# balcilar/gnn-matlang

Hardware: NVIDIA B200
Metric: GNNML3 train graphs/s (higher is better)
Workload: dtype f32

## Files before the change

### gnn_matlang_b200/_lib.py

```python
import ctypes
import os

import torch

_HERE = os.path.dirname(os.path.abspath(__file__))
LIB_PATH = os.environ.get("GNNML3_LIB", os.path.join(_HERE, "libgnnml3_b200.so"))

_p = ctypes.c_void_p
_i64 = ctypes.c_int64
_i = ctypes.c_int
_sz = ctypes.c_size_t

SIGNATURES = {
    "gnnml3_last_error": (ctypes.c_char_p, []),
    "gnnml3_version": (_i, []),
    "gnnml3_launch_count": (_i64, []),
    "gnnml3_csr_workspace_bytes": (_sz, [_i64, _i64]),
    "gnnml3_csr_build": (_i, [_p, _i64, _i64, _p, _p, _p, _p, _p, _p, _p, _p, _sz, _p]),
    "gnnml3_gather_rows": (_i, [_p, _p, _i64, _i, _p, _p]),
    "gnnml3_scatter_rows": (_i, [_p, _p, _i64, _i, _p, _p]),
    "gnnml3_spmm_k": (_i, [_p, _p, _p, _p, _p, _i64, _i64, _i, _i, _p, _i64, _p]),
    "gnnml3_spmm_projected": (_i, [_p, _p, _p, _p, _i, _p, _i64, _i64, _i, _p, _p, _i64, _p]),
    "gnnml3_sddmm_k": (_i, [_p, _p, _p, _p, _i64, _p, _i64, _i64, _i, _i, _p, _p]),
    "gnnml3_gemm_nn": (_i, [_p, _i64, _p, _i64, _p, _p, _i64, _i64, _i, _i, _i, _i, _p]),
    "gnnml3_gemm_tn_workspace_bytes": (_sz, [_i64, _i, _i]),
    "gnnml3_gemm_tn": (_i, [_p, _i64, _p, _i64, _p, _i64, _i64, _i, _i, _i, _p, _sz, _p]),
    "gnnml3_gemm_nn_tc_supported": (_i, [_i64, _i, _i]),
    "gnnml3_gemm_nn_tc_workspace_bytes": (_sz, [_i, _i]),
    "gnnml3_gemm_nn_tc": (_i, [_p, _i64, _p, _i64, _p, _p, _i64, _i64, _i, _i, _i, _i, _p, _sz, _p]),
    "gnnml3_colsum_workspace_bytes": (_sz, [_i64, _i]),
    "gnnml3_colsum": (_i, [_p, _i64, _i64, _i, _p, _p, _sz, _p]),
    "gnnml3_edge_mlp_supported": (_i, [_i, _i]),
    "gnnml3_collate_workspace_bytes": (_sz, [_i]),
    "gnnml3_collate": (_i, [_p, _p, _p, _p, _p, _p, _i, _p, _p, _i, _p, _i, _i64, _p, _i, _i, _i64, _i64, _p, _p, _p, _p, _p, _p, _sz, _p]),
    "gnnml3_collate_graphs_workspace_bytes": (_sz, [_i]),
    "gnnml3_collate_graphs": (_i, [_p, _p, _p, _p, _i, _p, _p, _i, _p, _p, _p, _i, _i64, _p, _i, _p, _p, _p, _i, _i64, _i, _i64, _i64, _i64,
                                   _p, _p, _p, _p, _p, _p, _p, _sz, _p]),
    "gnnml3_edge_mlp_set_tc": (_i, [_i]),
    "gnnml3_edge_mlp_path_counts": (_i, [_p, _i]),
    "gnnml3_edge_mlp_fwd": (_i, [_p, _p, _p, _p, _p, _p, _i64, _i, _i, _p, _p]),
    "gnnml3_edge_mlp_bwd_workspace_bytes": (_sz, [_i64, _i]),
    "gnnml3_edge_mlp_bwd": (_i, [_p, _p, _p, _p, _p, _p, _p, _i64, _i, _i, _p, _p, _p, _p, _p, _p, _sz, _p]),
    "gnnml3_ml3_act_fwd": (_i, [_p, _i64, _i64, _i, _i, _p, _i64, _p]),
    "gnnml3_ml3_act_bwd_workspace_bytes": (_sz, [_i64, _i, _i]),
    "gnnml3_ml3_act_bwd": (_i, [_p, _i64, _p, _i64, _i64, _i, _i, _p, _i64, _p, _i64, _p, _p, _sz, _p]),
    "gnnml3_ml3_act_bwd_y": (_i, [_p, _i64, _p, _i64, _p, _i64, _i64, _i, _i, _p, _i64, _p, _p, _sz, _p]),
    "gnnml3_fused_debug_counters": (_i, [_p, _i]),
    "gnnml3_fused_set_mode": (_i, [_i]),
    "gnnml3_fused_profile": (_i, [_i]),
    "gnnml3_fused_profile_fetch": (_i, [_p, _i]),
    "gnnml3_fused_supported": (_i, [_i, _i, _i, _i, _i, _i, _i]),
    "gnnml3_fused_workspace_bytes": (_sz, [_i, _i, _i, _i]),
    "gnnml3_fused_agg_proj": (_i, [_p, _p, _p, _p, _i, _i, _p, _i64, _i, _p, _i64, _i, _i, _p, _i64, _p, _i64, _i, _p, _p,
                                   _i64, _i, _p, _i64, _p, _i64, _i, _i, _p, _i64, _p, _p, _sz, _p]),
    "gnnml3_tile_rows": (_i, []),
    "gnnml3_tile_windows": (_i, [_p, _p, _i64, _p, _p]),
    "gnnml3_fused_ts_supported": (_i, [_i, _i, _i, _i, _i, _i, _i]),
    "gnnml3_fused_ts_workspace_bytes": (_sz, [_i, _i, _i]),
    "gnnml3_fused_set_ts": (_i, [_i]),
    "gnnml3_fused_path_counts": (_i, [_p, _i]),
    "gnnml3_fused_sddmm_supported": (_i, [_i, _i, _i]),
    "gnnml3_fused_sddmm_workspace_bytes": (_sz, [_i]),
    "gnnml3_fused_sddmm": (_i, [_p, _p, _p, _p, _i64, _i, _p, _i64, _i, _p, _i, _i64, _p, _p, _sz, _p]),
    "gnnml3_ml3layer_supported": (_i, [_i, _i, _i, _i, _i]),
    "gnnml3_ml3layer_workspace_bytes": (_sz, [_i64, _i64, _i, _i, _i, _i]),
    "gnnml3_ml3layer_forward": (_i, [_p, _p, _p, _i64, _i64, _p, _i64, _i, _p, _i, _p, _p, _p, _p, _p, _p, _i, _p, _p, _p, _p, _i, _p, _p,
                                     _i64, _p, _p, _i64, _p, _sz, _p]),
    "gnnml3_ml3layer_backward": (_i, [_p, _p, _p, _p, _p, _p, _p, _i64, _i64, _p, _i64, _i, _p, _p, _i, _p, _p, _p, _p, _p, _i, _p, _p, _i,
                                      _p, _i64, _p, _p, _i64, _i, _i, _p, _i64, _p, _p, _p, _p, _p, _p, _p, _p, _p, _p, _i64, _p, _sz, _p]),
    "gnnml3_ml1layer_supported": (_i, [_i, _i, _i]),
    "gnnml3_ml1layer_workspace_bytes": (_sz, [_i64, _i, _i, _i]),
    "gnnml3_ml1layer_forward": (_i, [_p, _p, _i64, _i64, _p, _i64, _i, _p, _p, _p, _p, _p, _p, _p, _p, _i, _i, _p, _i64, _p, _i64,
                                     _p, _i64, _p, _sz, _p]),
    "gnnml3_ml1layer_backward": (_i, [_p, _p, _i64, _i64, _p, _i64, _i, _p, _p, _p, _p, _i, _i, _p, _i64, _p, _i64, _p, _i64, _i,
                                      _p, _i64, _p, _p, _p, _p, _p, _p, _p, _p, _p, _sz, _p]),
    "gnnml3_ml1layer_forward_precision": (_i, [_p, _p, _i64, _i64, _p, _i64, _i, _p, _p, _p, _p, _p, _p, _p, _p, _i, _i, _p, _i64, _p,
                                               _i64, _p, _i64, _p, _sz, _p, _i]),
    "gnnml3_ml1layer_backward_precision": (_i, [_p, _p, _i64, _i64, _p, _i64, _i, _p, _p, _p, _p, _i, _i, _p, _i64, _p, _i64, _p, _i64,
                                                _i, _p, _i64, _p, _p, _p, _p, _p, _p, _p, _p, _p, _sz, _p, _i]),
    "gnnml3_segment_pool_fwd":(_i, [_p, _i64, _p, _i, _i, _i, _p, _p]),
    "gnnml3_segment_pool_bwd": (_i, [_p, _p, _i, _i, _i, _p, _i64, _p]),
    "gnnml3_segment_max_fwd": (_i, [_p, _i64, _p, _i, _i, _p, _p, _p]),
    "gnnml3_segment_max_bwd": (_i, [_p, _p, _p, _i, _i, _p, _i64, _p]),
    "gnnml3_spectral_max_nodes": (_i, [_i]),
    "gnnml3_spectral_count": (_i, [_p, _i64, _p, _p, _i, _i, _i, _p, _p]),
    "gnnml3_spectral_design": (_i, [_p, _i64, _p, _p, _i, _i, ctypes.c_double, _i, _i, _i, _i, ctypes.c_double, _i, _p, _i, _p,
                                    _i64, _p, _p, _p, _p]),
    "gnnml3_pairs_mark": (_i, [_p, _i64, _i64, _i, _p, _i64, ctypes.c_float, _p, _i64, _p]),
    "gnnml3_pairs_count": (_i, [_p, _i64, _i64, _i64, _p, _p]),
}

PREC_3XTF32 = 0
PREC_TF32 = 1
PREC_BF16 = 2
FUSED_FLAGS = {0: 0, 1: 0x100, 2: 0x200}
EPI_NONE = 0
EPI_RELU = 1

_lib = None


def load():
    global _lib
    if _lib is not None:
        return _lib
    if not os.path.exists(LIB_PATH):
        raise RuntimeError(
            "gnn_matlang_b200: %s not found -- build it with `python -c 'import __graft_entry__ as g; g.build()'` "
            "(or `make -C gnn_matlang_b200/csrc`).  There is no CPU / PyTorch fallback for the hot path." % LIB_PATH)
    lib = ctypes.CDLL(LIB_PATH)
    for name, (res, args) in SIGNATURES.items():
        fn = getattr(lib, name)
        fn.restype = res
        fn.argtypes = args
    _lib = lib
    return lib


def check(rc, what):
    if rc != 0:
        msg = load().gnnml3_last_error()
        raise RuntimeError("%s failed (code %d): %s" % (what, rc, msg.decode() if msg else "?"))


def stream_ptr():
    return torch._C._cuda_getCurrentRawStream(torch.cuda.current_device())


def ptr(t):
    if t is None:
        return None
    if not t.is_cuda:
        raise RuntimeError("gnn_matlang_b200: expected a CUDA tensor (the hot path has no CPU fallback)")
    return t.data_ptr()


def launch_count():
    return int(load().gnnml3_launch_count())
```

### gnn_matlang_b200/csrc/edge_mlp.cu

```cuda
#include "edge_mlp.cuh"

#include <stdlib.h>

#include <atomic>

namespace gnnml3 {

template <int K>
__global__ void __launch_bounds__(256)
k_edge_mlp_fwd(const float* __restrict__ ea, const int* __restrict__ eperm, const float* __restrict__ w1,
               const float* __restrict__ w2, const float* __restrict__ w3, const float* __restrict__ w4, int64_t E,
               float* __restrict__ out) {
    using C = EMC<K>;
    __shared__ __align__(16) float sw123[C::W123];
    __shared__ __align__(16) float sw4[C::W4];
    load_weights_smem<K>(sw123, sw4, w1, w2, w3, w4);
    __syncthreads();
    for (int64_t e = blockIdx.x * (int64_t)blockDim.x + threadIdx.x; e < E; e += (int64_t)gridDim.x * blockDim.x) {
        const int64_t src = eperm ? (int64_t)__ldg(eperm + e) : e;
        float in[C::KP];
        load_edge_row<K>(ea + src * K, in);
        float tmp[C::T];
#pragma unroll
        for (int j = 0; j < C::H; ++j) {
            const float a1 = dot_row<K>(sw123 + (0 * C::H + j) * C::KP, in);
            const float a2 = dot_row<K>(sw123 + (1 * C::H + j) * C::KP, in);
            const float a3 = dot_row<K>(sw123 + (2 * C::H + j) * C::KP, in);
            tmp[j] = fmaxf(a1, 0.f);
            tmp[C::H + j] = tanh_fast(a2) * tanh_fast(a3);
        }
        float o[K];
#pragma unroll
        for (int k = 0; k < K; ++k) {
            float a = 0.f;
#pragma unroll
            for (int j = 0; j < C::T; j += 4) {
                const float4 w = *reinterpret_cast<const float4*>(sw4 + k * C::T + j);
                a = fmaf(w.x, tmp[j], a);
                a = fmaf(w.y, tmp[j + 1], a);
                a = fmaf(w.z, tmp[j + 2], a);
                a = fmaf(w.w, tmp[j + 3], a);
            }
            o[k] = fmaxf(a, 0.f);
        }
        float* op = out + e * K;
#pragma unroll
        for (int k = 0; k < K; k += 2) *reinterpret_cast<float2*>(op + k) = make_float2(o[k], o[k + 1]);
    }
}

template <int K, bool DIN>
__global__ void __launch_bounds__(EMC<K>::THREADS)
k_edge_mlp_bwd(const float* __restrict__ ea, const int* __restrict__ eperm, const float* __restrict__ gout,
               const float* __restrict__ w1, const float* __restrict__ w2, const float* __restrict__ w3,
               const float* __restrict__ w4, int64_t E, float* __restrict__ dea, float* __restrict__ partial) {
    using C = EMC<K>;
    extern __shared__ __align__(16) float smem[];
    float* stage = smem;
    float* sw123 = smem + (size_t)C::TILE_E * C::S;
    float* sw4 = sw123 + C::W123;
    load_weights_smem<K>(sw123, sw4, w1, w2, w3, w4);

    const int tid = threadIdx.x;
    const int tile = tid % C::NT, group = tid / C::NT;
    const bool accum = group < C::GROUPS;
    int offA, offB;
    if (tile < C::NT1) {
        offA = C::OFF_D4 + 4 * (tile / (C::T / 4));
        offB = C::OFF_TMP + 4 * (tile % (C::T / 4));
    } else {
        const int t2 = tile - C::NT1;
        offA = C::OFF_D + 4 * (t2 / (C::KP / 4));
        offB = C::OFF_IN + 4 * (t2 % (C::KP / 4));
    }
    float acc[4][4];
#pragma unroll
    for (int r = 0; r < 4; ++r)
#pragma unroll
        for (int c = 0; c < 4; ++c) acc[r][c] = 0.f;
    __syncthreads();

    const int64_t ntiles = (E + C::TILE_E - 1) / C::TILE_E;
    for (int64_t tl = blockIdx.x; tl < ntiles; tl += gridDim.x) {
        const int64_t e = tl * C::TILE_E + tid;
        float* row = stage + (size_t)tid * C::S;
        if (e < E) {
            const int64_t src = eperm ? (int64_t)__ldg(eperm + e) : e;
            float in[C::KP];
            load_edge_row<K>(ea + src * K, in);
            float tmp[C::T];
            uint32_t mask1 = 0;
#pragma unroll
            for (int j0 = 0; j0 < C::H; j0 += 4) {
                float t2v[4], t3v[4];
#pragma unroll
                for (int jj = 0; jj < 4; ++jj) {
                    const int j = j0 + jj;
                    const float a1 = dot_row<K>(sw123 + (0 * C::H + j) * C::KP, in);
                    const float a2 = dot_row<K>(sw123 + (1 * C::H + j) * C::KP, in);
                    const float a3 = dot_row<K>(sw123 + (2 * C::H + j) * C::KP, in);
                    tmp[j] = fmaxf(a1, 0.f);
                    if (a1 > 0.f) mask1 |= (1u << j);
                    t2v[jj] = tanh_fast(a2);
                    t3v[jj] = tanh_fast(a3);
                    tmp[C::H + j] = t2v[jj] * t3v[jj];
                }
                *reinterpret_cast<float4*>(row + C::OFF_D + C::H + j0) = make_float4(t2v[0], t2v[1], t2v[2], t2v[3]);
                *reinterpret_cast<float4*>(row + C::OFF_D + 2 * C::H + j0) = make_float4(t3v[0], t3v[1], t3v[2], t3v[3]);
            }
#pragma unroll
            for (int j = 0; j < C::T; j += 4)
                *reinterpret_cast<float4*>(row + C::OFF_TMP + j) = make_float4(tmp[j], tmp[j + 1], tmp[j + 2], tmp[j + 3]);
#pragma unroll
            for (int i = 0; i < C::KP; i += 4)
                *reinterpret_cast<float4*>(row + C::OFF_IN + i) = make_float4(in[i], in[i + 1], in[i + 2], in[i + 3]);
            float d4[C::KP];
            {
                float go[C::KP];
                load_edge_row<K>(gout + e * K, go);
#pragma unroll
                for (int k = 0; k < K; ++k) {
                    float a = 0.f;
#pragma unroll
                    for (int j = 0; j < C::T; j += 4) {
                        const float4 w = *reinterpret_cast<const float4*>(sw4 + k * C::T + j);
                        a = fmaf(w.x, tmp[j], a);
                        a = fmaf(w.y, tmp[j + 1], a);
                        a = fmaf(w.z, tmp[j + 2], a);
                        a = fmaf(w.w, tmp[j + 3], a);
                    }
                    d4[k] = a > 0.f ? go[k] : 0.f;
                }
#pragma unroll
                for (int k = K; k < C::KP; ++k) d4[k] = 0.f;
            }
#pragma unroll
            for (int k = 0; k < C::KP; k += 4)
                *reinterpret_cast<float4*>(row + C::OFF_D4 + k) = make_float4(d4[k], d4[k + 1], d4[k + 2], d4[k + 3]);
            float din[DIN ? C::KP : 1];
#pragma unroll
            for (int i = 0; i < (DIN ? C::KP : 1); ++i) din[i] = 0.f;
#pragma unroll
            for (int j0 = 0; j0 < C::H; j0 += 4) {
                float dt1[4] = {0.f, 0.f, 0.f, 0.f}, dt2[4] = {0.f, 0.f, 0.f, 0.f};
#pragma unroll
                for (int k = 0; k < K; ++k) {
                    const float4 wa = *reinterpret_cast<const float4*>(sw4 + k * C::T + j0);
                    const float4 wb = *reinterpret_cast<const float4*>(sw4 + k * C::T + C::H + j0);
                    dt1[0] = fmaf(d4[k], wa.x, dt1[0]); dt1[1] = fmaf(d4[k], wa.y, dt1[1]);
                    dt1[2] = fmaf(d4[k], wa.z, dt1[2]); dt1[3] = fmaf(d4[k], wa.w, dt1[3]);
                    dt2[0] = fmaf(d4[k], wb.x, dt2[0]); dt2[1] = fmaf(d4[k], wb.y, dt2[1]);
                    dt2[2] = fmaf(d4[k], wb.z, dt2[2]); dt2[3] = fmaf(d4[k], wb.w, dt2[3]);
                }
                const float4 t2 = *reinterpret_cast<const float4*>(row + C::OFF_D + C::H + j0);
                const float4 t3 = *reinterpret_cast<const float4*>(row + C::OFF_D + 2 * C::H + j0);
                const float t2a[4] = {t2.x, t2.y, t2.z, t2.w}, t3a[4] = {t3.x, t3.y, t3.z, t3.w};
                float d1[4], d2[4], d3[4];
#pragma unroll
                for (int jj = 0; jj < 4; ++jj) {
                    d1[jj] = ((mask1 >> (j0 + jj)) & 1u) ? dt1[jj] : 0.f;
                    d2[jj] = dt2[jj] * t3a[jj] * (1.f - t2a[jj] * t2a[jj]);
                    d3[jj] = dt2[jj] * t2a[jj] * (1.f - t3a[jj] * t3a[jj]);
                }
                *reinterpret_cast<float4*>(row + C::OFF_D + j0) = make_float4(d1[0], d1[1], d1[2], d1[3]);
                *reinterpret_cast<float4*>(row + C::OFF_D + C::H + j0) = make_float4(d2[0], d2[1], d2[2], d2[3]);
                *reinterpret_cast<float4*>(row + C::OFF_D + 2 * C::H + j0) = make_float4(d3[0], d3[1], d3[2], d3[3]);
                if constexpr (DIN) {
#pragma unroll
                    for (int jj = 0; jj < 4; ++jj) {
                        const float* r1 = sw123 + (0 * C::H + j0 + jj) * C::KP;
                        const float* r2 = sw123 + (1 * C::H + j0 + jj) * C::KP;
                        const float* r3 = sw123 + (2 * C::H + j0 + jj) * C::KP;
#pragma unroll
                        for (int i = 0; i < C::KP; i += 4) {
                            const float4 a = *reinterpret_cast<const float4*>(r1 + i);
                            const float4 b = *reinterpret_cast<const float4*>(r2 + i);
                            const float4 c = *reinterpret_cast<const float4*>(r3 + i);
                            din[i] += d1[jj] * a.x + d2[jj] * b.x + d3[jj] * c.x;
                            din[i + 1] += d1[jj] * a.y + d2[jj] * b.y + d3[jj] * c.y;
                            din[i + 2] += d1[jj] * a.z + d2[jj] * b.z + d3[jj] * c.z;
                            din[i + 3] += d1[jj] * a.w + d2[jj] * b.w + d3[jj] * c.w;
                        }
                    }
                }
            }
            if constexpr (C::DP > C::D) {
#pragma unroll
                for (int i = C::D; i < C::DP; ++i) row[C::OFF_D + i] = 0.f;
            }
            if constexpr (DIN) {
                float* dp = dea + src * K;
#pragma unroll
                for (int i = 0; i < K; i += 2) *reinterpret_cast<float2*>(dp + i) = make_float2(din[i], din[i + 1]);
            }
        } else {
#pragma unroll
            for (int i = 0; i < C::ROW; i += 4) *reinterpret_cast<float4*>(row + i) = make_float4(0.f, 0.f, 0.f, 0.f);
        }
        __syncthreads();
        if (accum) {
#pragma unroll 4
            for (int r = group; r < C::TILE_E; r += C::GROUPS) {
                const float4 a = *reinterpret_cast<const float4*>(stage + (size_t)r * C::S + offA);
                const float4 b = *reinterpret_cast<const float4*>(stage + (size_t)r * C::S + offB);
                const float av[4] = {a.x, a.y, a.z, a.w}, bv[4] = {b.x, b.y, b.z, b.w};
#pragma unroll
                for (int i = 0; i < 4; ++i)
#pragma unroll
                    for (int j = 0; j < 4; ++j) acc[i][j] = fmaf(av[i], bv[j], acc[i][j]);
            }
        }
        __syncthreads();
    }
    float* red = stage;
    if (accum) {
#pragma unroll
        for (int i = 0; i < 4; ++i)
#pragma unroll
            for (int j = 0; j < 4; ++j) red[(size_t)group * C::NT * 16 + tile * 16 + i * 4 + j] = acc[i][j];
    }
    __syncthreads();
    for (int i = tid; i < C::NT * 16; i += blockDim.x) {
        float s = 0.f;
#pragma unroll
        for (int g = 0; g < C::GROUPS; ++g) s += red[(size_t)g * C::NT * 16 + i];
        partial[(size_t)blockIdx.x * C::NT * 16 + i] = s;
    }
}

static int bwd_blocks(int64_t E, int tile_e) {
    int64_t t = (E + tile_e - 1) / tile_e;
    int64_t cap = kNumSMs;
    return (int)(t < 1 ? 1 : (t > cap ? cap : t));
}

int edge_mlp_tc_fwd(const float* ea, const int32_t* eperm, const float* w1, const float* w2, const float* w3, const float* w4, int64_t E,
                    int K, float* out, cudaStream_t st);
size_t edge_mlp_tc_bwd_workspace_bytes(int K);
int edge_mlp_tc_bwd(const float* ea, const int32_t* eperm, const float* gout, const float* w1, const float* w2, const float* w3,
                    const float* w4, int64_t E, int K, float* dea, float* dw1, float* dw2, float* dw3, float* dw4, float* partial,
                    cudaStream_t st);

}

using namespace gnnml3;

static int g_edge_tc = [] {
    const char* e = getenv("GNNML3_EDGE_TC");
    return (e && e[0] == '0') ? 0 : 1;
}();
static std::atomic<long long> g_edge_paths[2];

extern "C" int gnnml3_edge_mlp_set_tc(int enable) {
    const int old = g_edge_tc;
    if (enable == 0 || enable == 1) g_edge_tc = enable;
    return old;
}
extern "C" int gnnml3_edge_mlp_path_counts(long long* out2_host, int reset) {
    out2_host[0] = reset ? g_edge_paths[0].exchange(0) : g_edge_paths[0].load();
    out2_host[1] = reset ? g_edge_paths[1].exchange(0) : g_edge_paths[1].load();
    return GNNML3_OK;
}

#define DISPATCH_EVEN_K(KV, ...)                                   \
    switch (KV) {                                                  \
        case 2: { constexpr int K_ = 2; __VA_ARGS__; } break;      \
        case 4: { constexpr int K_ = 4; __VA_ARGS__; } break;      \
        case 6: { constexpr int K_ = 6; __VA_ARGS__; } break;      \
        case 8: { constexpr int K_ = 8; __VA_ARGS__; } break;      \
        case 10: { constexpr int K_ = 10; __VA_ARGS__; } break;    \
        case 12: { constexpr int K_ = 12; __VA_ARGS__; } break;    \
        case 14: { constexpr int K_ = 14; __VA_ARGS__; } break;    \
        case 16: { constexpr int K_ = 16; __VA_ARGS__; } break;    \
        default: return set_err(GNNML3_ERR_INVALID, "edge_mlp: K=%d not instantiated (even K <= 16)", KV); \
    }

extern "C" int gnnml3_edge_mlp_supported(int K, int Kout) { return (K == Kout && K >= 2 && K <= 16 && K % 2 == 0) ? 1 : 0; }

extern "C" int gnnml3_edge_mlp_fwd(const float* ea, const int32_t* eperm, const float* w1, const float* w2, const float* w3,
                                   const float* w4, int64_t E, int K, int Kout, float* out, void* stream_) {
    GNNML3_REQUIRE(gnnml3_edge_mlp_supported(K, Kout), "edge_mlp_fwd: unsupported K=%d Kout=%d (even K <= 16, Kout == K)", K, Kout);
    GNNML3_REQUIRE(E >= 0, "edge_mlp_fwd: E < 0");
    if (E == 0) return GNNML3_OK;
    GNNML3_REQUIRE(ea && w1 && w2 && w3 && w4 && out, "edge_mlp_fwd: NULL pointer");
    GNNML3_REQUIRE((uintptr_t)ea % 16 == 0 && (uintptr_t)out % 16 == 0, "edge_mlp_fwd: ea/out must be 16-byte aligned");
    if (g_edge_tc) {
        ++g_edge_paths[0];
        return edge_mlp_tc_fwd(ea, eperm, w1, w2, w3, w4, E, K, out, (cudaStream_t)stream_);
    }
    ++g_edge_paths[1];
    int64_t nb = (E + 255) / 256;
    if (nb > (int64_t)kNumSMs * 8) nb = (int64_t)kNumSMs * 8;
    DISPATCH_EVEN_K(K, (k_edge_mlp_fwd<K_><<<(int)nb, 256, 0, (cudaStream_t)stream_>>>(ea, eperm, w1, w2, w3, w4, E, out)));
    GNNML3_LAUNCH_CHECK();
    return GNNML3_OK;
}

extern "C" size_t gnnml3_edge_mlp_bwd_workspace_bytes(int64_t E, int K) {
    const int KP = pad4(K), T = 4 * K, DP = pad4(6 * K);
    const size_t nt = (size_t)(KP / 4) * (T / 4) + (size_t)(DP / 4) * (KP / 4);
    const size_t cc = (size_t)bwd_blocks(E, 256) * nt * 16 * sizeof(float);
    const size_t tc = edge_mlp_tc_bwd_workspace_bytes(K);
    return align_up(cc > tc ? cc : tc, 256);
}

template <int K>
static int launch_edge_bwd(const float* ea, const int32_t* eperm, const float* gout, const float* w1, const float* w2,
                           const float* w3, const float* w4, int64_t E, float* dea, float* dw1, float* dw2, float* dw3,
                           float* dw4, float* partial, cudaStream_t st) {
    using C = EMC<K>;
    static bool configured[64] = {};
    if (auto once_ = first_use_on_device(configured)) {
        GNNML3_CUDA(cudaFuncSetAttribute(k_edge_mlp_bwd<K, true>, cudaFuncAttributeMaxDynamicSharedMemorySize, (int)C::bwd_smem));
        GNNML3_CUDA(cudaFuncSetAttribute(k_edge_mlp_bwd<K, false>, cudaFuncAttributeMaxDynamicSharedMemorySize, (int)C::bwd_smem));
    }
    const int nb = bwd_blocks(E, C::TILE_E);
    if (dea)
        k_edge_mlp_bwd<K, true><<<nb, C::THREADS, C::bwd_smem, st>>>(ea, eperm, gout, w1, w2, w3, w4, E, dea, partial);
    else
        k_edge_mlp_bwd<K, false><<<nb, C::THREADS, C::bwd_smem, st>>>(ea, eperm, gout, w1, w2, w3, w4, E, dea, partial);
    GNNML3_LAUNCH_CHECK();
    k_edge_mlp_bwd_reduce<K><<<cdiv(C::NOUT, 32), 256, 0, st>>>(partial, nb, dw1, dw2, dw3, dw4);
    GNNML3_LAUNCH_CHECK();
    return GNNML3_OK;
}

extern "C" int gnnml3_edge_mlp_bwd(const float* ea, const int32_t* eperm, const float* gout, const float* w1, const float* w2,
                                   const float* w3, const float* w4, int64_t E, int K, int Kout, float* dea, float* dw1,
                                   float* dw2, float* dw3, float* dw4, void* workspace, size_t workspace_bytes,
                                   void* stream_) {
    GNNML3_REQUIRE(gnnml3_edge_mlp_supported(K, Kout), "edge_mlp_bwd: unsupported K=%d Kout=%d", K, Kout);
    GNNML3_REQUIRE(E >= 0 && w1 && w2 && w3 && w4 && dw1 && dw2 && dw3 && dw4, "edge_mlp_bwd: bad arguments");
    cudaStream_t st = (cudaStream_t)stream_;
    if (E == 0) {
        GNNML3_CUDA(cudaMemsetAsync(dw1, 0, sizeof(float) * 2 * K * K, st));
        GNNML3_CUDA(cudaMemsetAsync(dw2, 0, sizeof(float) * 2 * K * K, st));
        GNNML3_CUDA(cudaMemsetAsync(dw3, 0, sizeof(float) * 2 * K * K, st));
        GNNML3_CUDA(cudaMemsetAsync(dw4, 0, sizeof(float) * 4 * K * K, st));
        return GNNML3_OK;
    }
    GNNML3_REQUIRE(ea && gout && workspace, "edge_mlp_bwd: NULL pointer");
    GNNML3_REQUIRE((uintptr_t)ea % 16 == 0 && (uintptr_t)gout % 16 == 0 && (dea == nullptr || (uintptr_t)dea % 16 == 0),
                   "edge_mlp_bwd: ea/gout/dea must be 16-byte aligned");
    if (workspace_bytes < gnnml3_edge_mlp_bwd_workspace_bytes(E, K))
        return set_err(GNNML3_ERR_WORKSPACE, "edge_mlp_bwd: workspace too small");
    if (g_edge_tc) {
        ++g_edge_paths[0];
        return edge_mlp_tc_bwd(ea, eperm, gout, w1, w2, w3, w4, E, K, dea, dw1, dw2, dw3, dw4, (float*)workspace, st);
    }
    ++g_edge_paths[1];
    DISPATCH_EVEN_K(K, return launch_edge_bwd<K_>(ea, eperm, gout, w1, w2, w3, w4, E, dea, dw1, dw2, dw3, dw4,
                                                   (float*)workspace, st));
    return GNNML3_OK;
}
```

### gnn_matlang_b200/csrc/edge_mlp.cuh

```cuda
#pragma once
#include "common.cuh"

namespace gnnml3 {

constexpr int pad4(int x) { return (x + 3) / 4 * 4; }

template <int K>
struct EMC {
    static constexpr int KP = pad4(K);
    static constexpr int H = 2 * K;
    static constexpr int T = 4 * K;
    static constexpr int D = 6 * K;
    static constexpr int DP = pad4(D);
    static constexpr int OFF_D4 = 0, OFF_TMP = KP, OFF_D = KP + T, OFF_IN = KP + T + DP, ROW = KP + T + DP + KP;
    static constexpr int S = ((ROW / 4) % 2 == 1) ? ROW : ROW + 4;
    static constexpr int NT1 = (KP / 4) * (T / 4);
    static constexpr int NT2 = (DP / 4) * (KP / 4);
    static constexpr int NT = NT1 + NT2;
    static constexpr int THREADS = 256;
    static constexpr int GROUPS = (THREADS / NT) < 1 ? 1 : (THREADS / NT);
    static constexpr int TILE_E = THREADS;
    static constexpr int W123 = 3 * H * KP;
    static constexpr int W4 = K * T;
    static constexpr int NOUT = K * T + 3 * H * K;
    static constexpr size_t bwd_smem = sizeof(float) * ((size_t)TILE_E * S + W123 + W4);
};

template <int K>
__device__ __forceinline__ void load_weights_smem(float* sw123, float* sw4, const float* __restrict__ w1,
                                                  const float* __restrict__ w2, const float* __restrict__ w3,
                                                  const float* __restrict__ w4) {
    using C = EMC<K>;
    for (int i = threadIdx.x; i < C::W123; i += blockDim.x) {
        const int m = i / (C::H * C::KP), r = (i / C::KP) % C::H, c = i % C::KP;
        const float* w = m == 0 ? w1 : (m == 1 ? w2 : w3);
        sw123[i] = (c < K) ? __ldg(w + r * K + c) : 0.f;
    }
    for (int i = threadIdx.x; i < C::W4; i += blockDim.x) sw4[i] = __ldg(w4 + i);
}

template <int K>
__device__ __forceinline__ void load_edge_row(const float* __restrict__ p, float (&in)[EMC<K>::KP]) {
    if constexpr (K % 4 == 0) {
#pragma unroll
        for (int i = 0; i < K; i += 4) {
            float4 v = ldg4(p + i);
            in[i] = v.x; in[i + 1] = v.y; in[i + 2] = v.z; in[i + 3] = v.w;
        }
    } else {
#pragma unroll
        for (int i = 0; i < K; i += 2) {
            float2 v = ldg2(p + i);
            in[i] = v.x; in[i + 1] = v.y;
        }
#pragma unroll
        for (int i = K; i < EMC<K>::KP; ++i) in[i] = 0.f;
    }
}

template <int K>
__device__ __forceinline__ float dot_row(const float* __restrict__ wrow, const float (&in)[EMC<K>::KP]) {
    float a = 0.f;
#pragma unroll
    for (int i = 0; i < EMC<K>::KP; i += 4) {
        const float4 w = *reinterpret_cast<const float4*>(wrow + i);
        a = fmaf(w.x, in[i], a);
        a = fmaf(w.y, in[i + 1], a);
        a = fmaf(w.z, in[i + 2], a);
        a = fmaf(w.w, in[i + 3], a);
    }
    return a;
}

template <int K>
__global__ void __launch_bounds__(256)
k_edge_mlp_bwd_reduce(const float* __restrict__ partial, int nblocks, float* __restrict__ dw1, float* __restrict__ dw2,
                      float* __restrict__ dw3, float* __restrict__ dw4) {
    using C = EMC<K>;
    __shared__ float red[8][33];
    const int tx = threadIdx.x & 31, ty = threadIdx.x >> 5;
    const int i = blockIdx.x * 32 + tx;
    int idx = 0;
    float* dst = nullptr;
    if (i < C::NOUT) {
        int r, c;
        if (i < K * C::T) {
            r = i / C::T;
            c = i % C::T;
            idx = ((r / 4) * (C::T / 4) + c / 4) * 16 + (r % 4) * 4 + (c % 4);
            dst = dw4 + i;
        } else {
            const int q = i - K * C::T;
            const int m = q / (C::H * K), jj = (q / K) % C::H;
            c = q % K;
            r = m * C::H + jj;
            idx = (C::NT1 + (r / 4) * (C::KP / 4) + c / 4) * 16 + (r % 4) * 4 + (c % 4);
            dst = (m == 0 ? dw1 : (m == 1 ? dw2 : dw3)) + jj * K + c;
        }
    }
    float s = 0.f;
    if (dst) {
        float s1 = 0.f, s2 = 0.f, s3 = 0.f;
        int b = ty;
        for (; b + 24 < nblocks; b += 32) {
            s += __ldg(partial + (size_t)b * C::NT * 16 + idx);
            s1 += __ldg(partial + (size_t)(b + 8) * C::NT * 16 + idx);
            s2 += __ldg(partial + (size_t)(b + 16) * C::NT * 16 + idx);
            s3 += __ldg(partial + (size_t)(b + 24) * C::NT * 16 + idx);
        }
        for (; b < nblocks; b += 8) s += __ldg(partial + (size_t)b * C::NT * 16 + idx);
        s = (s + s1) + (s2 + s3);
    }
    red[ty][tx] = s;
    __syncthreads();
    if (ty == 0 && dst) {
        float v = 0.f;
#pragma unroll
        for (int y = 0; y < 8; ++y) v += red[y][tx];
        *dst = v;
    }
}


}
```

### gnn_matlang_b200/csrc/edge_mlp_tc.cu

```cuda
#include "edge_mlp.cuh"
#include "tc_common.cuh"

namespace gnnml3 {

#ifndef EMT_MAXWG
#define EMT_MAXWG 4
#endif

template <int K>
struct EMT {
    using C = EMC<K>;
    static constexpr int P = (K + 7) / 8 * 8;
    static constexpr int HP = 2 * P, TP = 4 * P, DPP = 6 * P;
    static constexpr int N1 = 6 * P;
    static constexpr int N2 = 16;
    static constexpr int N3 = TP;
    static constexpr int TB = TP / 32;
    static constexpr int DB = (DPP + 31) / 32;
    static constexpr int B1_BYTES = 2 * N1 * 128, B2_BYTES = TB * 32 * 128, B3_BYTES = 2 * N3 * 128, B4_BYTES = DB * 32 * 128;
    __host__ __device__ static constexpr int xc(int mode) { return mode > 1 ? 12 * P : 8 * P; }
    static constexpr int YC = 2 * P;
    __host__ __device__ static constexpr int slot(int mode) { return xc(mode) + YC; }
    __host__ __device__ static constexpr int plane_bytes(int mode) { return B1_BYTES + B2_BYTES + (mode > 0 ? B3_BYTES : 0) + (mode > 1 ? B4_BYTES : 0); }
    static constexpr int stage_bytes = 128 * C::S * 4;
    static constexpr int SMEM_MAX = 227 * 1024 - 1024;
    __host__ __device__ static constexpr int nwg(int mode) {
        int n = 512 / slot(mode);
        if (mode > 0) {
            const int m = (SMEM_MAX - plane_bytes(mode) - 64) / stage_bytes;
            n = m < n ? m : n;
        }
        return n < 1 ? 1 : (n > EMT_MAXWG ? EMT_MAXWG : n);
    }
    __host__ __device__ static constexpr int smem_bytes(int mode) { return 1024 + plane_bytes(mode) + 64 + (mode > 0 ? nwg(mode) * stage_bytes : 0); }
    static constexpr int NT = C::NT;
    static constexpr int TPT = (NT + 127) / 128;
    static constexpr int GROUPS = NT >= 128 ? 1 : 128 / NT;
};

#ifdef EMT_PROFILE
__device__ unsigned long long g_emt_dbg[16];
#define EMT_T(i) do { if (prof) { const long long now_ = clock64(); tacc[i] += now_ - tlast; tlast = now_; } } while (0)
#else
#define EMT_T(i) do { } while (0)
#endif

struct EMTParams {
    const float* ea;
    const int* eperm;
    const float* gout;
    const float *w1, *w2, *w3, *w4;
    int64_t E;
    float* out;
    float* dea;
    float* partial;
};

__device__ __forceinline__ float emt_lo(float v) { return v - __uint_as_float(__float_as_uint(v) & 0xFFFFE000u); }

__device__ __forceinline__ void emt_st8(uint32_t ta, const float* v) {
    asm volatile("tcgen05.st.sync.aligned.32x32b.x8.b32 [%0], {%1,%2,%3,%4,%5,%6,%7,%8};" ::"r"(ta), "f"(v[0]), "f"(v[1]), "f"(v[2]),
                 "f"(v[3]), "f"(v[4]), "f"(v[5]), "f"(v[6]), "f"(v[7])
                 : "memory");
}
__device__ __forceinline__ void emt_st16(uint32_t ta, const float* v) {
    asm volatile("tcgen05.st.sync.aligned.32x32b.x16.b32 [%0], {%1,%2,%3,%4,%5,%6,%7,%8,%9,%10,%11,%12,%13,%14,%15,%16};" ::"r"(ta),
                 "f"(v[0]), "f"(v[1]), "f"(v[2]), "f"(v[3]), "f"(v[4]), "f"(v[5]), "f"(v[6]), "f"(v[7]), "f"(v[8]), "f"(v[9]), "f"(v[10]),
                 "f"(v[11]), "f"(v[12]), "f"(v[13]), "f"(v[14]), "f"(v[15])
                 : "memory");
}
__device__ __forceinline__ void emt_st_wait() { asm volatile("tcgen05.wait::st.sync.aligned;" ::: "memory"); }
__device__ __forceinline__ void emt_ld16(uint32_t ta, float (&v)[16]) {
    asm volatile(
        "tcgen05.ld.sync.aligned.32x32b.x16.b32 {%0,%1,%2,%3,%4,%5,%6,%7,%8,%9,%10,%11,%12,%13,%14,%15}, [%16];"
        : "=f"(v[0]), "=f"(v[1]), "=f"(v[2]), "=f"(v[3]), "=f"(v[4]), "=f"(v[5]), "=f"(v[6]), "=f"(v[7]), "=f"(v[8]), "=f"(v[9]), "=f"(v[10]),
          "=f"(v[11]), "=f"(v[12]), "=f"(v[13]), "=f"(v[14]), "=f"(v[15])
        : "r"(ta)
        : "memory");
}
__device__ __forceinline__ void emt_ld_wait() { asm volatile("tcgen05.wait::ld.sync.aligned;" ::: "memory"); }

__device__ __forceinline__ void emt_mma(uint32_t tmem_d, uint32_t tmem_a, uint64_t bdesc, uint32_t idesc, uint32_t accumulate) {
    asm volatile(
        "{\n\t"
        ".reg .pred p;\n\t"
        "setp.ne.b32 p, %4, 0;\n\t"
        "tcgen05.mma.cta_group::1.kind::tf32 [%0], [%1], %2, %3, p;\n\t"
        "}\n" ::"r"(tmem_d), "r"(tmem_a), "l"(bdesc), "r"(idesc), "r"(accumulate)
        : "memory");
}
__device__ __forceinline__ bool emt_elect() {
    uint32_t pred;
    asm volatile(
        "{\n\t"
        ".reg .pred p;\n\t"
        "elect.sync _|p, 0xffffffff;\n\t"
        "selp.u32 %0, 1, 0, p;\n\t"
        "}\n"
        : "=r"(pred));
    return pred != 0;
}
__device__ __forceinline__ void emt_group_sync(int id) { asm volatile("bar.sync %0, 128;" ::"r"(id) : "memory"); }

__device__ __forceinline__ uint32_t emt_sw128(int n, int c) { return (uint32_t)n * 128u + ((uint32_t)(((c >> 2) ^ (n & 7)) << 4) | (uint32_t)((c & 3) << 2)); }

__device__ __forceinline__ void emt_put(uint8_t* plane, int n, int c, float v, bool lo) {
    const float h = tf32_rn(v);
    *reinterpret_cast<float*>(plane + emt_sw128(n, c)) = lo ? v - h : h;
}

template <typename F>
__device__ __forceinline__ void emt_round(int barid, int warp_in_wg, uint64_t* bar, uint32_t& ph, F issue) {
    emt_st_wait();
    tc_fence_before();
    emt_group_sync(barid);
    if (warp_in_wg == 0) {
        if (emt_elect()) {
            tc_fence_after();
            issue();
            umma_commit(bar);
        }
        __syncwarp();
    }
    mbar_wait(bar, ph);
    ph ^= 1;
    tc_fence_after();
}

template <int K, int MODE>
__global__ void __launch_bounds__(EMT<K>::nwg(MODE) * 128, 1) k_edge_mlp_tc(const EMTParams p) {
    using T = EMT<K>;
    using C = EMC<K>;
    constexpr int P = T::P, HP = T::HP, TP = T::TP, H = C::H;
    constexpr int NWG = T::nwg(MODE);
    extern __shared__ uint8_t smem_raw[];
    uint8_t* smem = smem_raw + ((1024u - (smem_u32(smem_raw) & 1023u)) & 1023u);
    uint8_t* b1 = smem;
    uint8_t* b2 = b1 + T::B1_BYTES;
    uint8_t* b3 = b2 + T::B2_BYTES;
    uint8_t* b4 = b3 + T::B3_BYTES;
    uint8_t* tail = smem + T::plane_bytes(MODE);
    uint64_t* bars = reinterpret_cast<uint64_t*>(tail);
    uint32_t* tmem_slot = reinterpret_cast<uint32_t*>(tail + 48);
    float* stage_all = reinterpret_cast<float*>(tail + 64);

    const int wg = threadIdx.x >> 7, t = threadIdx.x & 127, warp_in_wg = t >> 5;

    for (int i = threadIdx.x; i < 2 * T::N1 * P; i += blockDim.x) {
        const int n = i / P, c = i % P;
        const bool lo = n >= T::N1;
        const int nn = lo ? n - T::N1 : n, b = nn / HP, j = nn % HP;
        const float* w = b == 0 ? p.w1 : (b == 1 ? p.w2 : p.w3);
        emt_put(b1, n, c, (j < H && c < K) ? __ldg(w + j * K + c) : 0.f, lo);
    }
    for (int i = threadIdx.x; i < T::TB * 32 * 32; i += blockDim.x) {
        const int tb = i / 1024, n = (i / 32) % 32, c = i % 32;
        const bool lo = n >= 16;
        const int k = n & 15, q = tb * 32 + c, part = q / HP, j = q % HP;
        emt_put(b2 + tb * 4096, n, c, (k < K && j < H) ? __ldg(p.w4 + k * C::T + part * H + j) : 0.f, lo);
    }
    if constexpr (MODE > 0) {
        for (int i = threadIdx.x; i < 2 * T::N3 * P; i += blockDim.x) {
            const int n = i / P, c = i % P;
            const bool lo = n >= T::N3;
            const int q = lo ? n - T::N3 : n, part = q / HP, j = q % HP;
            emt_put(b3, n, c, (c < K && j < H) ? __ldg(p.w4 + c * C::T + part * H + j) : 0.f, lo);
        }
    }
    if constexpr (MODE > 1) {
        for (int i = threadIdx.x; i < T::DB * 32 * 32; i += blockDim.x) {
            const int db = i / 1024, n = (i / 32) % 32, c = i % 32;
            const bool lo = n >= 16;
            const int ii = n & 15, q = db * 32 + c, b = q / HP, j = q % HP;
            const float* w = b == 0 ? p.w1 : (b == 1 ? p.w2 : p.w3);
            emt_put(b4 + db * 4096, n, c, (ii < K && q < T::DPP && j < H) ? __ldg(w + j * K + ii) : 0.f, lo);
        }
    }
    fence_proxy_async_smem();
    if (threadIdx.x == 0) {
        for (int g = 0; g < NWG; ++g) mbar_init(bars + g, 1);
        asm volatile("fence.mbarrier_init.release.cluster;" ::: "memory");
    }
    if (threadIdx.x < 32) tmem_alloc(tmem_slot, 512);
    tc_fence_before();
    __syncthreads();
    tc_fence_after();
    const uint32_t tmem_base = *tmem_slot;

    const uint32_t Xm = tmem_base + (uint32_t)wg * T::slot(MODE), Ym = Xm + T::xc(MODE);
    const uint32_t lane_sel = (uint32_t)(warp_in_wg * 32) << 16;
    const uint32_t X = Xm + lane_sel, Y = Ym + lane_sel;
    uint64_t* bar = bars + wg;
    uint32_t ph = 0;
    const int barid = 1 + wg;
    const uint64_t d1h = make_kmajor_sw128_desc(smem_u32(b1)), d1l = d1h + (uint64_t)((T::N1 * 128) >> 4);
    const uint64_t d2h = make_kmajor_sw128_desc(smem_u32(b2)), d2l = d2h + (uint64_t)((16 * 128) >> 4);
    const uint64_t d3h = make_kmajor_sw128_desc(smem_u32(b3)), d3l = d3h + (uint64_t)((T::N3 * 128) >> 4);
    const uint64_t d4h = make_kmajor_sw128_desc(smem_u32(b4)), d4l = d4h + (uint64_t)((16 * 128) >> 4);
    constexpr uint32_t ID1 = make_idesc_tf32_mn(128, T::N1), ID2 = make_idesc_tf32_mn(128, T::N2), ID3 = make_idesc_tf32_mn(128, T::N3);
    auto mma3 = [&](uint32_t d, uint32_t a_raw, uint32_t a_lo, uint64_t bh, uint64_t bl, uint32_t idesc, bool first) {
        emt_mma(d, a_raw, bh, idesc, first ? 0u : 1u);
        emt_mma(d, a_raw, bl, idesc, 1u);
        emt_mma(d, a_lo, bh, idesc, 1u);
    };

    float* stage = stage_all + (size_t)wg * 128 * C::S;
    float* row = stage + (size_t)t * C::S;

    int offA[T::TPT], offB[T::TPT];
    bool accum[T::TPT];
    float acc[T::TPT][4][4];
    const int group = T::TPT == 1 ? t / T::NT : 0;
    if constexpr (MODE > 0) {
#pragma unroll
        for (int u = 0; u < T::TPT; ++u) {
            const int tl = T::TPT == 1 ? t % T::NT : t + 128 * u;
            accum[u] = T::TPT == 1 ? group < T::GROUPS : tl < T::NT;
            if (tl < C::NT1) {
                offA[u] = C::OFF_D4 + 4 * (tl / (C::T / 4));
                offB[u] = C::OFF_TMP + 4 * (tl % (C::T / 4));
            } else {
                const int t2 = (tl < T::NT ? tl : C::NT1) - C::NT1;
                offA[u] = C::OFF_D + 4 * (t2 / (C::KP / 4));
                offB[u] = C::OFF_IN + 4 * (t2 % (C::KP / 4));
            }
#pragma unroll
            for (int r = 0; r < 4; ++r)
#pragma unroll
                for (int c = 0; c < 4; ++c) acc[u][r][c] = 0.f;
        }
    }

    const int64_t ntiles = (p.E + 127) / 128;
    const int64_t tstride = (int64_t)gridDim.x * NWG;
    float in_n[C::KP];
    int64_t src_n = 0;
    auto fetch = [&](int64_t tile) {
        const int64_t e = tile * 128 + t;
#pragma unroll
        for (int i = 0; i < C::KP; ++i) in_n[i] = 0.f;
        src_n = 0;
        if (tile < ntiles && e < p.E) {
            src_n = p.eperm ? (int64_t)__ldg(p.eperm + e) : e;
            load_edge_row<K>(p.ea + src_n * K, in_n);
        }
    };
    fetch((int64_t)blockIdx.x * NWG + wg);
#ifdef EMT_PROFILE
    const bool prof = t == 0;
    long long tacc[10] = {0, 0, 0, 0, 0, 0, 0, 0, 0, 0}, tlast = clock64();
    const long long tbegin = tlast;
#endif
    for (int64_t tile = (int64_t)blockIdx.x * NWG + wg; tile < ntiles; tile += tstride) {
        const int64_t e = tile * 128 + t;
        const bool live = e < p.E;
        const int64_t src = src_n;
        float in[P];
#pragma unroll
        for (int i = 0; i < P; ++i) in[i] = i < C::KP ? in_n[i < C::KP ? i : 0] : 0.f;
        {
            float lo[P];
#pragma unroll
            for (int i = 0; i < P; ++i) lo[i] = emt_lo(in[i]);
            if constexpr (P == 8) {
                emt_st8(Y, in);
                emt_st8(Y + 8, lo);
            } else {
                emt_st16(Y, in);
                emt_st16(Y + 16, lo);
            }
        }
        if constexpr (MODE > 0) {
#pragma unroll
            for (int i = 0; i < C::KP; i += 4) *reinterpret_cast<float4*>(row + C::OFF_IN + i) = make_float4(in[i], in[i + 1], in[i + 2], in[i + 3]);
        }
        float go[C::KP];
#pragma unroll
        for (int i = 0; i < C::KP; ++i) go[i] = 0.f;
        if constexpr (MODE > 0) {
            if (live) load_edge_row<K>(p.gout + e * K, go);
        }
        fetch(tile + tstride);
        EMT_T(0);
        emt_round(barid, warp_in_wg, bar, ph, [&] {
#pragma unroll
            for (int s = 0; s < P / 8; ++s) mma3(Xm, Ym + 8 * s, Ym + P + 8 * s, d1h + (uint64_t)(2 * s), d1l + (uint64_t)(2 * s), ID1, s == 0);
        });
        EMT_T(1);
        uint32_t mask1 = 0;
#pragma unroll
        for (int c = 0; c < HP / 16; ++c) {
            float r[16], a2[16], a3[16];
            emt_ld16(X + 16 * c, r);
            emt_ld16(X + 2 * P + 16 * c, a2);
            emt_ld16(X + 4 * P + 16 * c, a3);
            emt_ld_wait();
            float pr[16];
#pragma unroll
            for (int i = 0; i < 16; ++i) {
                if (MODE > 0 && r[i] > 0.f) mask1 |= 1u << (16 * c + i);
                r[i] = fmaxf(r[i], 0.f);
                a2[i] = tanh_fast5(a2[i]);
                a3[i] = tanh_fast5(a3[i]);
                pr[i] = a2[i] * a3[i];
            }
            emt_st16(X + 16 * c, r);
            emt_st16(X + 2 * P + 16 * c, pr);
            if constexpr (MODE > 0) {
#pragma unroll
                for (int i = 0; i < 16; i += 4) {
                    const int j0 = 16 * c + i;
                    if (j0 < H) {
                        *reinterpret_cast<float4*>(row + C::OFF_TMP + j0) = make_float4(r[i], r[i + 1], r[i + 2], r[i + 3]);
                        *reinterpret_cast<float4*>(row + C::OFF_TMP + H + j0) = make_float4(pr[i], pr[i + 1], pr[i + 2], pr[i + 3]);
                        *reinterpret_cast<float4*>(row + C::OFF_D + H + j0) = make_float4(a2[i], a2[i + 1], a2[i + 2], a2[i + 3]);
                        *reinterpret_cast<float4*>(row + C::OFF_D + 2 * H + j0) = make_float4(a3[i], a3[i + 1], a3[i + 2], a3[i + 3]);
                    }
                }
            }
#pragma unroll
            for (int i = 0; i < 16; ++i) {
                r[i] = emt_lo(r[i]);
                pr[i] = emt_lo(pr[i]);
            }
            emt_st16(X + 4 * P + 16 * c, r);
            emt_st16(X + 6 * P + 16 * c, pr);
        }
        EMT_T(2);
        emt_round(barid, warp_in_wg, bar, ph, [&] {
#pragma unroll
            for (int s = 0; s < TP / 8; ++s) {
                const uint64_t adv = (uint64_t)((s / 4) * (4096 >> 4) + 2 * (s % 4));
                mma3(Ym, Xm + 8 * s, Xm + TP + 8 * s, d2h + adv, d2l + adv, ID2, s == 0);
            }
        });
        EMT_T(3);
        float pre4[16];
        emt_ld16(Y, pre4);
        emt_ld_wait();
        if constexpr (MODE == 0) {
            if (live) {
                float* op = p.out + e * K;
#pragma unroll
                for (int k = 0; k < K; k += 2) *reinterpret_cast<float2*>(op + k) = make_float2(fmaxf(pre4[k], 0.f), fmaxf(pre4[k + 1], 0.f));
            }
        } else {
            float dp4[P];
#pragma unroll
            for (int k = 0; k < P; ++k) dp4[k] = (k < K && pre4[k] > 0.f) ? go[k < C::KP ? k : 0] : 0.f;
#pragma unroll
            for (int k = 0; k < C::KP; k += 4) *reinterpret_cast<float4*>(row + C::OFF_D4 + k) = make_float4(dp4[k], dp4[k + 1], dp4[k + 2], dp4[k + 3]);
            {
                float lo[P];
#pragma unroll
                for (int i = 0; i < P; ++i) lo[i] = emt_lo(dp4[i]);
                if constexpr (P == 8) {
                    emt_st8(Y, dp4);
                    emt_st8(Y + 8, lo);
                } else {
                    emt_st16(Y, dp4);
                    emt_st16(Y + 16, lo);
                }
            }
            emt_round(barid, warp_in_wg, bar, ph, [&] {
#pragma unroll
                for (int s = 0; s < P / 8; ++s) mma3(Xm, Ym + 8 * s, Ym + P + 8 * s, d3h + (uint64_t)(2 * s), d3l + (uint64_t)(2 * s), ID3, s == 0);
            });
            EMT_T(4);
#pragma unroll
            for (int c = 0; c < HP / 16; ++c) {
                float dt1[16], dt2[16];
                emt_ld16(X + 16 * c, dt1);
                emt_ld16(X + 2 * P + 16 * c, dt2);
                emt_ld_wait();
                float g1[16], g2[16], g3[16];
#pragma unroll
                for (int i = 0; i < 16; i += 4) {
                    const int j0 = 16 * c + i;
                    float4 t2 = make_float4(0.f, 0.f, 0.f, 0.f), t3 = t2;
                    if (j0 < H) {
                        t2 = *reinterpret_cast<const float4*>(row + C::OFF_D + H + j0);
                        t3 = *reinterpret_cast<const float4*>(row + C::OFF_D + 2 * H + j0);
                    }
                    const float t2a[4] = {t2.x, t2.y, t2.z, t2.w}, t3a[4] = {t3.x, t3.y, t3.z, t3.w};
#pragma unroll
                    for (int jj = 0; jj < 4; ++jj) {
                        g1[i + jj] = ((mask1 >> (j0 + jj)) & 1u) ? dt1[i + jj] : 0.f;
                        g2[i + jj] = dt2[i + jj] * t3a[jj] * (1.f - t2a[jj] * t2a[jj]);
                        g3[i + jj] = dt2[i + jj] * t2a[jj] * (1.f - t3a[jj] * t3a[jj]);
                    }
                    if (j0 < H) {
                        *reinterpret_cast<float4*>(row + C::OFF_D + j0) = make_float4(g1[i], g1[i + 1], g1[i + 2], g1[i + 3]);
                        *reinterpret_cast<float4*>(row + C::OFF_D + H + j0) = make_float4(g2[i], g2[i + 1], g2[i + 2], g2[i + 3]);
                        *reinterpret_cast<float4*>(row + C::OFF_D + 2 * H + j0) = make_float4(g3[i], g3[i + 1], g3[i + 2], g3[i + 3]);
                    }
                }
                if constexpr (MODE > 1) {
                    emt_st16(X + 16 * c, g1);
                    emt_st16(X + 2 * P + 16 * c, g2);
                    emt_st16(X + 4 * P + 16 * c, g3);
#pragma unroll
                    for (int i = 0; i < 16; ++i) {
                        g1[i] = emt_lo(g1[i]);
                        g2[i] = emt_lo(g2[i]);
                        g3[i] = emt_lo(g3[i]);
                    }
                    emt_st16(X + 6 * P + 16 * c, g1);
                    emt_st16(X + 8 * P + 16 * c, g2);
                    emt_st16(X + 10 * P + 16 * c, g3);
                }
            }
            if constexpr (C::DP > C::D) {
#pragma unroll
                for (int i = C::D; i < C::DP; ++i) row[C::OFF_D + i] = 0.f;
            }
            if constexpr (MODE > 1) {
                emt_round(barid, warp_in_wg, bar, ph, [&] {
#pragma unroll
                    for (int s = 0; s < T::DPP / 8; ++s) {
                        const uint64_t adv = (uint64_t)((s / 4) * (4096 >> 4) + 2 * (s % 4));
                        mma3(Ym, Xm + 8 * s, Xm + T::DPP + 8 * s, d4h + adv, d4l + adv, ID2, s == 0);
                    }
                });
                float din[16];
                emt_ld16(Y, din);
                emt_ld_wait();
                if (live) {
                    float* dp = p.dea + src * K;
#pragma unroll
                    for (int i = 0; i < K; i += 2) *reinterpret_cast<float2*>(dp + i) = make_float2(din[i], din[i + 1]);
                }
            }
            EMT_T(5);
            emt_group_sync(barid);
            EMT_T(6);
#pragma unroll
            for (int u = 0; u < T::TPT; ++u) {
                if (accum[u]) {
                    const float* pa = stage + (size_t)group * C::S + offA[u];
                    const float* pb = stage + (size_t)group * C::S + offB[u];
#pragma unroll 4
                    for (int r = group; r < 128; r += T::GROUPS) {
                        const float4 a = *reinterpret_cast<const float4*>(pa);
                        const float4 b = *reinterpret_cast<const float4*>(pb);
                        pa += T::GROUPS * C::S;
                        pb += T::GROUPS * C::S;
                        const float av[4] = {a.x, a.y, a.z, a.w}, bv[4] = {b.x, b.y, b.z, b.w};
#pragma unroll
                        for (int i = 0; i < 4; ++i)
#pragma unroll
                            for (int j = 0; j < 4; ++j) acc[u][i][j] = fmaf(av[i], bv[j], acc[u][i][j]);
                    }
                }
            }
            emt_group_sync(barid);
            EMT_T(7);
        }
        EMT_T(8);
    }
#ifdef EMT_PROFILE
    if (prof && wg == 0) {
        for (int i = 0; i < 9; ++i) atomicAdd(&g_emt_dbg[i], (unsigned long long)tacc[i]);
        atomicAdd(&g_emt_dbg[9], (unsigned long long)(clock64() - tbegin));
        atomicAdd(&g_emt_dbg[10], 1ull);
    }
#endif
    if constexpr (MODE > 0) {
        float* red = stage;
#pragma unroll
        for (int u = 0; u < T::TPT; ++u) {
            if (accum[u]) {
                const int tl = T::TPT == 1 ? t % T::NT : t + 128 * u;
#pragma unroll
                for (int i = 0; i < 4; ++i)
#pragma unroll
                    for (int j = 0; j < 4; ++j) red[(size_t)group * T::NT * 16 + tl * 16 + i * 4 + j] = acc[u][i][j];
            }
        }
        emt_group_sync(barid);
        for (int i = t; i < T::NT * 16; i += 128) {
            float s = 0.f;
#pragma unroll
            for (int g = 0; g < T::GROUPS; ++g) s += red[(size_t)g * T::NT * 16 + i];
            red[i] = s;
        }
        __syncthreads();
        float* dst = p.partial + (size_t)blockIdx.x * T::NT * 16;
        for (int i = threadIdx.x; i < T::NT * 16; i += NWG * 128) {
            float s = 0.f;
#pragma unroll
            for (int g = 0; g < NWG; ++g) s += stage_all[(size_t)g * 128 * C::S + i];
            dst[i] = s;
        }
    }
    tc_fence_before();
    __syncthreads();
    if (threadIdx.x < 32) tmem_dealloc(tmem_base, 512);
}

template <int K, int MODE>
static int emt_launch(const EMTParams& p, int* nparts, cudaStream_t st) {
    using T = EMT<K>;
    static bool configured[64] = {};
    if (auto once_ = first_use_on_device(configured))
        GNNML3_CUDA(cudaFuncSetAttribute(k_edge_mlp_tc<K, MODE>, cudaFuncAttributeMaxDynamicSharedMemorySize, T::smem_bytes(MODE)));
    constexpr int NWG = T::nwg(MODE);
    const int64_t ntiles = (p.E + 127) / 128;
    int64_t grid = (ntiles + NWG - 1) / NWG;
    if (grid > kNumSMs) grid = kNumSMs;
    k_edge_mlp_tc<K, MODE><<<(int)grid, NWG * 128, T::smem_bytes(MODE), st>>>(p);
    GNNML3_LAUNCH_CHECK();
    if (nparts) *nparts = (int)grid;
    return GNNML3_OK;
}

#define EMT_DISPATCH(KV, ...)                                      \
    switch (KV) {                                                  \
        case 2: { constexpr int K_ = 2; __VA_ARGS__; } break;      \
        case 4: { constexpr int K_ = 4; __VA_ARGS__; } break;      \
        case 6: { constexpr int K_ = 6; __VA_ARGS__; } break;      \
        case 8: { constexpr int K_ = 8; __VA_ARGS__; } break;      \
        case 10: { constexpr int K_ = 10; __VA_ARGS__; } break;    \
        case 12: { constexpr int K_ = 12; __VA_ARGS__; } break;    \
        case 14: { constexpr int K_ = 14; __VA_ARGS__; } break;    \
        case 16: { constexpr int K_ = 16; __VA_ARGS__; } break;    \
        default: return set_err(GNNML3_ERR_INVALID, "edge_mlp_tc: K=%d not instantiated (even K <= 16)", KV); \
    }

int edge_mlp_tc_fwd(const float* ea, const int32_t* eperm, const float* w1, const float* w2, const float* w3, const float* w4, int64_t E,
                    int K, float* out, cudaStream_t st) {
    EMTParams p;
    p.ea = ea; p.eperm = eperm; p.gout = nullptr; p.w1 = w1; p.w2 = w2; p.w3 = w3; p.w4 = w4; p.E = E; p.out = out; p.dea = nullptr;
    p.partial = nullptr;
    EMT_DISPATCH(K, return (emt_launch<K_, 0>(p, nullptr, st)));
    return GNNML3_OK;
}

size_t edge_mlp_tc_bwd_workspace_bytes(int K) {
    const int KP = pad4(K), T = 4 * K, DP = pad4(6 * K);
    const size_t nt = (size_t)(KP / 4) * (T / 4) + (size_t)(DP / 4) * (KP / 4);
    return (size_t)kNumSMs * nt * 16 * sizeof(float);
}

int edge_mlp_tc_bwd(const float* ea, const int32_t* eperm, const float* gout, const float* w1, const float* w2, const float* w3,
                    const float* w4, int64_t E, int K, float* dea, float* dw1, float* dw2, float* dw3, float* dw4, float* partial,
                    cudaStream_t st) {
    EMTParams p;
    p.ea = ea; p.eperm = eperm; p.gout = gout; p.w1 = w1; p.w2 = w2; p.w3 = w3; p.w4 = w4; p.E = E; p.out = nullptr; p.dea = dea;
    p.partial = partial;
    int nparts = 0, rc;
    if (dea) {
        EMT_DISPATCH(K, rc = (emt_launch<K_, 2>(p, &nparts, st)));
    } else {
        EMT_DISPATCH(K, rc = (emt_launch<K_, 1>(p, &nparts, st)));
    }
    if (rc) return rc;
    EMT_DISPATCH(K, (k_edge_mlp_bwd_reduce<K_><<<cdiv(EMC<K_>::NOUT, 32), 256, 0, st>>>(partial, nparts, dw1, dw2, dw3, dw4)));
    GNNML3_LAUNCH_CHECK();
    return GNNML3_OK;
}

}

#ifdef EMT_PROFILE
extern "C" __attribute__((visibility("default"))) int gnnml3_emt_debug_fetch(unsigned long long* host16, int reset) {
    cudaDeviceSynchronize();
    cudaMemcpyFromSymbol(host16, gnnml3::g_emt_dbg, sizeof(unsigned long long) * 16);
    if (reset) {
        unsigned long long z[16] = {};
        cudaMemcpyToSymbol(gnnml3::g_emt_dbg, z, sizeof(z));
    }
    return 0;
}
#endif
```

### gnn_matlang_b200/libs/spect_conv.py

```python
import math
import os

import torch
import torch.nn as nn
from torch.nn import Parameter

from .. import _lib, ops
from ..graph import get_plan, sorted_edge_attr

_PRECISIONS = {"fp32": _lib.PREC_3XTF32, "3xtf32": _lib.PREC_3XTF32, "tf32": _lib.PREC_TF32, "bf16": _lib.PREC_BF16}
USE_FUSED = os.environ.get("GNNML3_NO_FUSED", "0") != "1"
USE_LAYER_API = os.environ.get("GNNML3_NO_LAYER_API", "0") != "1"
KEEP_FIRST_LAYER_AGGREGATE = os.environ.get("GNNML3_KEEP_AGGREGATE", "1") != "0"


def _use_fused(precision):
    return USE_FUSED


def _fused_ok(precision, K, Kstride, F, Nc, Fs=0, self_mode=0, Ns=0):
    if precision == _lib.PREC_3XTF32:
        return ops.fused_supported(K, Kstride, F, Nc, Fs, self_mode, Ns)
    return ops.fused_ts_supported(K, Kstride, F, Nc, Fs, self_mode, Ns)


def glorot(tensor):
    if tensor is not None:
        stdv = math.sqrt(6.0 / (tensor.size(-2) + tensor.size(-1)))
        tensor.data.uniform_(-stdv, stdv)


def zeros(tensor):
    if tensor is not None:
        tensor.data.fill_(0)


def _aggregate(plan, ea_s, x, width_blocks, transposed=False):
    N, F = x.shape
    K = ea_s.size(1)
    out = torch.empty(N, width_blocks * F, dtype=torch.float32, device=x.device)
    if plan.E == 0:
        out[:, :K * F].zero_()
    elif transposed:
        ops.spmm_k(plan.rowptrT, plan.colT, plan.permT, ea_s, x, out=out)
    else:
        ops.spmm_k(plan.rowptr, plan.col, None, ea_s, x, out=out)
    return out


class _SpectConvFn(torch.autograd.Function):

    @staticmethod
    def forward(ctx, x, ea_s, weight, bias, plan, selfconn, precision):
        if x.stride(1) != 1:
            x = x.contiguous()
        ea_s = ea_s.contiguous()
        weight = weight.contiguous()
        N, Fi = x.shape
        Kw, _, Fo = weight.shape
        K = ea_s.size(1)
        fused = (_use_fused(precision) and N > 0 and plan.E > 0 and (not selfconn or Fi <= 32)
                 and _fused_ok(precision, K, K, Fi, Fo, Fi if selfconn else 0, 2 if selfconn else 0, 0))
        ctx.plan, ctx.selfconn, ctx.precision, ctx.has_bias = plan, selfconn, precision, bias is not None
        ctx.fused = fused
        if fused:
            x = ops.aligned_rows(x)
            out, _ = ops.fused_agg_proj(plan.rowptr, plan.col, None, ea_s, x, weight[:K].reshape(K * Fi, Fo), bias=bias,
                                        S=x if selfconn else None, self_mode=2 if selfconn else 0,
                                        Bself=weight[K] if selfconn else None, epilogue=0, win=plan.win, precision=precision)
        else:
            H = _aggregate(plan, ea_s, x, Kw)
            if selfconn:
                H[:, K * Fi:] = x
            out = ops.gemm_nn(H, weight.view(Kw * Fi, Fo), bias, precision=precision)
        ctx.save_for_backward(x, ea_s, weight)
        return out

    @staticmethod
    def backward(ctx, gout):
        x, ea_s, weight = ctx.saved_tensors
        plan, prec = ctx.plan, ctx.precision
        N, Fi = x.shape
        Kw, _, Fo = weight.shape
        K = ea_s.size(1)
        need_x, need_ea, need_w, need_b = ctx.needs_input_grad[:4]
        dx = dea = dw = db = None
        if N == 0:
            return (torch.zeros_like(x) if need_x else None, torch.zeros_like(ea_s) if need_ea else None,
                    torch.zeros_like(weight) if need_w else None,
                    torch.zeros(Fo, device=x.device) if (need_b and ctx.has_bias) else None, None, None, None)
        gout = ops.aligned_rows(gout) if ctx.fused else gout.contiguous()
        fused_dx = (ctx.fused and need_x and (not ctx.selfconn or Fo <= 32)
                    and _fused_ok(prec, K, K, Fo, Fi, Fo if ctx.selfconn else 0, 2 if ctx.selfconn else 0, 0))
        G = None
        if fused_dx:
            Fp = (Fo + 31) // 32 * 32
            side = need_w and ops.fused_side_output_ok()
            if side:
                G = torch.empty(N, (K + (1 if ctx.selfconn else 0)) * Fp, dtype=torch.float32, device=x.device)
            dx, _ = ops.fused_agg_proj(plan.rowptrT, plan.colT, plan.permT, ea_s, gout,
                                       weight[:K].transpose(1, 2).reshape(K * Fo, Fi).contiguous(),
                                       S=gout if ctx.selfconn else None, self_mode=2 if ctx.selfconn else 0,
                                       Bself=weight[K].t().contiguous() if ctx.selfconn else None, epilogue=0, hout=G,
                                       win=plan.winT, precision=prec)
            if side:
                dcat = ops.gemm_tn(x, G, precision=prec)
                dw = dcat.view(Fi, Kw, Fp)[:, :, :Fo].permute(1, 0, 2).contiguous()
                need_w = False
        if need_w or (need_x and not fused_dx):
            G = _aggregate(plan, ea_s, gout, Kw, transposed=True)
            if ctx.selfconn:
                G[:, K * Fo:] = gout
            if need_x and not fused_dx:
                dx = ops.gemm_nn(G, weight.transpose(1, 2).contiguous().view(Kw * Fo, Fi), precision=prec)
            if need_w:
                dw = ops.gemm_tn(x, G, precision=prec).view(Fi, Kw, Fo).permute(1, 0, 2).contiguous()
        if need_b and ctx.has_bias:
            db = ops.colsum(gout)
        if need_ea:
            if plan.E == 0:
                dea = torch.zeros_like(ea_s)
            elif ctx.fused and ops.fused_sddmm_supported(K, Fi, Fo):
                dea = ops.fused_sddmm(plan.rowptr, plan.col, x, gout, weight[:K].contiguous(), plan.E, win=plan.win)
            else:
                wp = weight[:K].permute(2, 0, 1).reshape(Fo, K * Fi).contiguous()
                dH = ops.gemm_nn(gout, wp, precision=prec)
                dea = ops.sddmm_k(plan.rowptr, plan.col, None, x, dH, K, plan.E)
        return dx, dea, dw, db, None, None, None


class _SpectConvProjectFirstFn(torch.autograd.Function):

    @staticmethod
    def forward(ctx, x, ea_s, weight, bias, plan, precision):
        x, ea_s = x.contiguous(), ea_s.contiguous()
        K, Fi, Fo = weight.shape
        wcat = weight.permute(1, 0, 2).reshape(Fi, K * Fo).contiguous()
        Y = ops.gemm_nn(x, wcat, precision=precision)
        if plan.E == 0:
            out = torch.zeros(x.size(0), Fo, device=x.device) + (bias if bias is not None else 0)
        else:
            out = ops.spmm_projected(plan.rowptr, plan.col, None, ea_s, Y, Fo, bias)
        ctx.save_for_backward(x, ea_s, wcat, Y)
        ctx.plan, ctx.precision, ctx.has_bias, ctx.shape = plan, precision, bias is not None, (K, Fi, Fo)
        return out

    @staticmethod
    def backward(ctx, gout):
        x, ea_s, wcat, Y = ctx.saved_tensors
        plan, prec = ctx.plan, ctx.precision
        K, Fi, Fo = ctx.shape
        gout = gout.contiguous()
        dY = _aggregate(plan, ea_s, gout, K, transposed=True)
        dx = ops.gemm_nn(dY, wcat.t().contiguous(), precision=prec) if ctx.needs_input_grad[0] else None
        dw = None
        if ctx.needs_input_grad[2]:
            dw = ops.gemm_tn(x, dY, precision=prec).view(Fi, K, Fo).permute(1, 0, 2).contiguous()
        dea = None
        if ctx.needs_input_grad[1]:
            dea = (torch.zeros_like(ea_s) if plan.E == 0 else
                   ops.sddmm_k(plan.rowptrT, plan.colT, plan.permT, gout, Y, K, plan.E))
        db = ops.colsum(gout) if (ctx.has_bias and ctx.needs_input_grad[3]) else None
        return dx, dea, dw, db, None, None


def project_first_pays(N, E, K, Fi, Fo):
    return K * Fo * (E + 2 * N) < Fi * (E + 2 * N * K)


class _AggregateFn(torch.autograd.Function):

    @staticmethod
    def forward(ctx, x, ea_s, plan):
        x, ea_s = x.contiguous(), ea_s.contiguous()
        ctx.save_for_backward(x, ea_s)
        ctx.plan = plan
        return _aggregate(plan, ea_s, x, ea_s.size(1))

    @staticmethod
    def backward(ctx, dH):
        x, ea_s = ctx.saved_tensors
        plan = ctx.plan
        dH = dH.contiguous()
        K, F = ea_s.size(1), x.size(1)
        if plan.E == 0:
            return torch.zeros_like(x), torch.zeros_like(ea_s), None
        dx = ops.spmm_projected(plan.rowptrT, plan.colT, plan.permT, ea_s, dH, F) if ctx.needs_input_grad[0] else None
        dea = ops.sddmm_k(plan.rowptr, plan.col, None, x, dH, K, plan.E) if ctx.needs_input_grad[1] else None
        return dx, dea, None


class _DepthwiseAggFn(torch.autograd.Function):

    @staticmethod
    def forward(ctx, x, ea_s, scale, plan):
        x, ea_s, scale = x.contiguous(), ea_s.contiguous(), scale.contiguous()
        N, F = x.shape
        K = ea_s.size(1)
        H = _aggregate(plan, ea_s, x, K)
        ctx.save_for_backward(x, ea_s, scale, H)
        ctx.plan = plan
        return (H.view(N, K, F) * scale.unsqueeze(0)).sum(1)

    @staticmethod
    def backward(ctx, dZ):
        x, ea_s, scale, H = ctx.saved_tensors
        plan = ctx.plan
        dZ = dZ.contiguous()
        N, F = x.shape
        K = ea_s.size(1)
        G = _aggregate(plan, ea_s, dZ, K, transposed=True)
        dx = (G.view(N, K, F) * scale.unsqueeze(0)).sum(1)
        dscale = (H.view(N, K, F) * dZ.unsqueeze(1)).sum(0)
        if plan.E == 0:
            dea = torch.zeros_like(ea_s)
        else:
            g = (dZ.unsqueeze(1) * scale.unsqueeze(0)).reshape(N, K * F).contiguous()
            dea = ops.sddmm_k(plan.rowptr, plan.col, None, x, g, K, plan.E)
        return dx, dea, dscale, None


class _LinearFn(torch.autograd.Function):

    @staticmethod
    def forward(ctx, x, wt, bias, precision):
        x, wt = x.contiguous(), wt.contiguous()
        ctx.save_for_backward(x, wt)
        ctx.precision, ctx.has_bias = precision, bias is not None
        return ops.gemm_nn(x, wt, bias, precision=precision)

    @staticmethod
    def backward(ctx, g):
        x, wt = ctx.saved_tensors
        g = g.contiguous()
        dx = dw = db = None
        if x.size(0) == 0:
            return torch.zeros_like(x), torch.zeros_like(wt), (torch.zeros(wt.size(1), device=x.device) if ctx.has_bias else None), None
        if ctx.needs_input_grad[0]:
            dx = ops.gemm_nn(g, wt.t().contiguous(), precision=ctx.precision)
        if ctx.needs_input_grad[1]:
            dw = ops.gemm_tn(x, g, precision=ctx.precision)
        if ctx.has_bias and ctx.needs_input_grad[2]:
            db = ops.colsum(g)
        return dx, dw, db, None


class _ML3LayerFn(torch.autograd.Function):

    @staticmethod
    def forward(ctx, x, ea_s, w1, w2, w3, w4, wconv, bconv, w11, b11, w12, b12, plan, fused_edge, precision, save=True):
        if x.stride(1) != 1:
            x = x.contiguous()
        ea_s = ea_s.contiguous()
        wconv = wconv.contiguous()
        N, Fi = x.shape
        K, _, Fo = wconv.shape
        G = 0 if w11 is None else w11.size(0)
        ctx.composite = False
        if (_use_fused(precision) and precision == _lib.PREC_3XTF32 and USE_LAYER_API and N > 0 and plan.E > 0
                and (fused_edge or w1 is None) and ops.ml3layer_supported(K, Fi, Fo, G, fused_edge)):
            xa = ops.aligned_rows(x)
            ws4 = tuple(w.contiguous() for w in (w1, w2, w3, w4)) if fused_edge else None
            gates = (w11.contiguous(), b11.contiguous(), w12.contiguous(), b12.contiguous()) if G > 0 else None
            keep = (not ctx.needs_input_grad[0]) and ctx.needs_input_grad[6] and Fi <= 32 and KEEP_FIRST_LAYER_AGGREGATE
            if save:
                y, aux, ea2, hside = ops.ml3layer_forward(plan, xa, ea_s, ws4, wconv, bconv.contiguous() if bconv is not None else None,
                                                          gates, keep_aggregate=keep)
            else:
                y, aux, ea2, hside = ops.ml3layer_forward(plan, xa, ea_s, ws4, wconv, bconv.contiguous() if bconv is not None else None,
                                                          gates, keep_aggregate=False, aux=False)
            ctx.plan, ctx.fused_edge, ctx.precision, ctx.G = plan, fused_edge, precision, G
            ctx.has_bias, ctx.fused, ctx.composite = bconv is not None, True, True
            if save:
                ctx.save_for_backward(xa, ea_s, ea2, y, aux, w1, w2, w3, w4, wconv, w11, w12, hside)
            return y
        if fused_edge:
            w1, w2, w3, w4 = w1.contiguous(), w2.contiguous(), w3.contiguous(), w4.contiguous()
            ea2 = ops.edge_mlp_fwd(ea_s, None, w1, w2, w3, w4)
        else:
            ea2 = ea_s
        fused = (_use_fused(precision) and N > 0 and plan.E > 0 and (G == 0 or Fi <= 32)
                 and _fused_ok(precision, K, K, Fi, Fo, Fi if G else 0, 1 if G else 0, 2 * G)
                 and _fused_ok(precision, K, K, Fo, Fi, 2 * G, 2 if G else 0, 0))
        ctx.plan, ctx.fused_edge, ctx.precision, ctx.G = plan, fused_edge, precision, G
        ctx.has_bias = bconv is not None
        ctx.fused = fused
        if fused:
            xa = ops.aligned_rows(x)
            wg = torch.cat([w11.t(), w12.t()], 1).contiguous() if G > 0 else None
            bg = torch.cat([b11, b12]) if G > 0 else None
            if save:
                y, aux = ops.fused_agg_proj(plan.rowptr, plan.col, None, ea2, xa, wconv.view(K * Fi, Fo), bias=bconv,
                                            S=xa if G > 0 else None, self_mode=1 if G > 0 else 0, Bself=wg, bias_s=bg, G=G,
                                            epilogue=1, win=plan.win, precision=precision)
                ctx.save_for_backward(xa, ea_s, ea2 if fused_edge else None, y, aux, w1, w2, w3, w4, wconv, w11, w12, None)
            else:
                y, _ = ops.fused_agg_proj(plan.rowptr, plan.col, None, ea2, xa, wconv.view(K * Fi, Fo), bias=bconv,
                                          S=xa if G > 0 else None, self_mode=1 if G > 0 else 0, Bself=wg, bias_s=bg, G=G,
                                          epilogue=1, win=plan.win, precision=precision, aux=False)
            return y
        H = _aggregate(plan, ea2, x, K)
        pre = torch.empty(N, (Fo + 2 * G + 3) // 4 * 4, dtype=torch.float32, device=x.device)[:, :Fo + 2 * G]
        if N > 0:
            ops.gemm_nn(H, wconv.view(K * Fi, Fo), bconv, precision=precision, out=pre[:, :Fo])
            if G > 0:
                wg = torch.cat([w11.t(), w12.t()], 1).contiguous()
                ops.gemm_nn(x, wg, torch.cat([b11, b12]), precision=precision, out=pre[:, Fo:])
        y = ops.ml3_act_fwd(pre, Fo, G)
        if save:
            ctx.save_for_backward(x, ea_s, ea2 if fused_edge else None, pre, None, w1, w2, w3, w4, wconv, w11, w12, None)
        return y

    @staticmethod
    def backward(ctx, gy):
        x, ea_s, ea2, pre, aux, w1, w2, w3, w4, wconv, w11, w12, hside = ctx.saved_tensors
        plan, prec, G = ctx.plan, ctx.precision, ctx.G
        if ea2 is None:
            ea2 = ea_s
        N, Fi = x.shape
        K, _, Fo = wconv.shape
        need = ctx.needs_input_grad
        if ctx.composite and N > 0:
            gy = gy if gy.stride(1) == 1 else gy.contiguous()
            ws4 = (w1, w2, w3, w4) if ctx.fused_edge else None
            dx, dea, dws, dwc, dbc, dw11, db11, dw12, db12 = ops.ml3layer_backward(
                plan, x, ea_s, ea2, ws4, wconv, (w11, w12) if G > 0 else None, pre, aux, gy, need[0], need[1], ctx.has_bias, hside=hside)
            return (dx, dea, dws[0], dws[1], dws[2], dws[3], dwc, dbc, dw11, db11, dw12, db12, None, None, None, None)
        gy = gy.contiguous()
        Gp = torch.empty(N, K * Fo + 2 * G, dtype=torch.float32, device=x.device)
        if ctx.fused:
            Fo4 = (Fo + 3) // 4 * 4
            gpre, dball = ops.ml3_act_bwd_y(pre, aux, gy, Fo, G)
            if G > 0:
                Gp[:, K * Fo:] = gpre[:, Fo4:Fo4 + 2 * G]
        else:
            gpre, dball = ops.ml3_act_bwd(pre, gy, Fo, G, gate_out=Gp[:, K * Fo:] if G > 0 else None)
        gc = gpre[:, :Fo]
        dx = dea = None
        dws = [None, None, None, None]
        dwc = dbc = dw11 = db11 = dw12 = db12 = None
        if N == 0:
            z = torch.zeros_like
            return (z(x), z(ea_s), *(z(w) if w is not None else None for w in (w1, w2, w3, w4)), z(wconv),
                    torch.zeros(Fo, device=x.device) if ctx.has_bias else None,
                    z(w11) if G else None, torch.zeros(G, device=x.device) if G else None,
                    z(w12) if G else None, torch.zeros(G, device=x.device) if G else None, None, None, None, None)
        if plan.E == 0:
            Gp[:, :K * Fo].zero_()
        else:
            ops.spmm_k(plan.rowptrT, plan.colT, plan.permT, ea2, gc, out=Gp)
        if need[0] and ctx.fused:
            dx, _ = ops.fused_agg_proj(plan.rowptrT, plan.colT, plan.permT, ea2, gpre[:, :Fo],
                                       wconv.transpose(1, 2).reshape(K * Fo, Fi).contiguous(),
                                       S=gpre[:, Fo4:Fo4 + 2 * G] if G > 0 else None, self_mode=2 if G > 0 else 0,
                                       Bself=torch.cat([w11, w12], 0).contiguous() if G > 0 else None, epilogue=0,
                                       win=plan.winT, precision=prec)
        elif need[0]:
            blocks = [wconv.transpose(1, 2).reshape(K * Fo, Fi)]
            if G > 0:
                blocks += [w11, w12]
            dx = ops.gemm_nn(Gp, torch.cat(blocks, 0).contiguous(), precision=prec)
        dcat = ops.gemm_tn(x, Gp, precision=prec)
        dwc = dcat[:, :K * Fo].reshape(Fi, K, Fo).permute(1, 0, 2).contiguous()
        if ctx.has_bias:
            dbc = dball[:Fo].contiguous()
        if G > 0:
            dw11 = dcat[:, K * Fo:K * Fo + G].t().contiguous()
            dw12 = dcat[:, K * Fo + G:].t().contiguous()
            db11 = dball[Fo:Fo + G].contiguous()
            db12 = dball[Fo + G:].contiguous()
        if ctx.fused_edge or need[1]:
            if plan.E == 0:
                dea2 = torch.zeros_like(ea2)
            elif ctx.fused and ops.fused_sddmm_supported(K, Fi, Fo):
                dea2 = ops.fused_sddmm(plan.rowptr, plan.col, x, gc, wconv, plan.E, win=plan.win)
            else:
                wp = wconv.permute(2, 0, 1).reshape(Fo, K * Fi).contiguous()
                dH = ops.gemm_nn(gc, wp, precision=prec)
                dea2 = ops.sddmm_k(plan.rowptr, plan.col, None, x, dH, K, plan.E)
            if ctx.fused_edge:
                dea, dws = ops.edge_mlp_bwd(ea_s, None, dea2, w1, w2, w3, w4, need_dea=need[1])
            else:
                dea = dea2
        return (dx, dea, dws[0], dws[1], dws[2], dws[3], dwc, dbc, dw11, db11, dw12, db12, None, None, None, None)


def _needs_save(*tensors):
    return torch.is_grad_enabled() and any(t is not None and t.requires_grad for t in tensors)


def _check_inputs(x, edge_index, edge_attr):
    if not (x.is_cuda and edge_index.is_cuda and edge_attr.is_cuda):
        raise RuntimeError("gnn_matlang_b200: x, edge_index and edge_attr must be CUDA tensors "
                           "(the B200 hot path has no CPU fallback)")
    if x.dim() != 2 or x.dtype != torch.float32 or edge_attr.dtype != torch.float32:
        raise RuntimeError("gnn_matlang_b200: x [N,F] and edge_attr [E,K] must be float32")


class SpectConv(nn.Module):

    def __init__(self, in_channels, out_channels, K=1, selfconn=True, depthwise=False, bias=True, **kwargs):
        kwargs.setdefault('aggr', 'add')
        if kwargs.pop('aggr') != 'add':
            raise ValueError("SpectConv only implements aggr='add' (the reference's default, :27)")
        self.precision = kwargs.pop('precision', 'fp32')
        if self.precision not in _PRECISIONS:
            raise ValueError("precision must be one of %s" % sorted(_PRECISIONS))
        self.order = kwargs.pop('order', 'auto')
        if self.order not in ('auto', 'aggregate_first', 'project_first'):
            raise ValueError("order must be 'auto', 'aggregate_first' or 'project_first'")
        super(SpectConv, self).__init__()
        assert K > 0
        self.in_channels = in_channels
        self.out_channels = out_channels
        self.depthwise = depthwise
        self.selfconn = selfconn
        if self.selfconn:
            K = K + 1
        if self.depthwise:
            self.DSweight = Parameter(torch.Tensor(K, in_channels))
            self.nsup = K
            K = 1
        self.weight = Parameter(torch.Tensor(K, in_channels, out_channels))
        if bias:
            self.bias = Parameter(torch.Tensor(out_channels))
        else:
            self.register_parameter('bias', None)
        self.reset_parameters()

    def reset_parameters(self):
        glorot(self.weight)
        zeros(self.bias)
        if self.depthwise:
            zeros(self.DSweight)

    def forward(self, x, edge_index, edge_attr, edge_weight=None, batch=None, lambda_max=None):
        _check_inputs(x, edge_index, edge_attr)
        plan = get_plan(edge_index, x.size(0))
        return self.forward_sorted(x, plan, sorted_edge_attr(edge_attr, plan))

    def forward_sorted(self, x, plan, ea_s):
        prec = _PRECISIONS[self.precision]
        if not self.depthwise:
            nk = self.weight.size(0) - (1 if self.selfconn else 0)
            if ea_s.size(1) < nk:
                raise RuntimeError("SpectConv: edge_attr has %d channels but the layer was built with K=%d"
                                   % (ea_s.size(1), nk))
            if ea_s.size(1) > nk:
                ea_s = ea_s[:, :nk]
            order = self.order
            if order == 'auto':
                Fi, Fo = self.in_channels, self.out_channels
                fused = _use_fused(prec) and _fused_ok(prec, nk, nk, Fi, Fo, Fi if self.selfconn else 0, 2 if self.selfconn else 0, 0)
                order = 'project_first' if (not fused and Fo <= 256 and project_first_pays(plan.N, plan.E, nk, Fi, Fo)) else 'aggregate_first'
            if order == 'project_first' and self.out_channels <= 256:
                out = _SpectConvProjectFirstFn.apply(x, ea_s, self.weight[:nk], None if self.selfconn else self.bias, plan, prec)
                if self.selfconn:
                    out = out + _LinearFn.apply(x, self.weight[nk], self.bias, prec)
                return out
            return _SpectConvFn.apply(x, ea_s, self.weight, self.bias, plan, self.selfconn, prec)
        nk = self.nsup - (1 if self.selfconn else 0)
        if ea_s.size(1) < nk:
            raise RuntimeError("SpectConv(depthwise): edge_attr has %d channels, need %d" % (ea_s.size(1), nk))
        scale = self.DSweight[:nk] + torch.cat([torch.ones(1, self.in_channels, device=x.device),
                                                torch.zeros(nk - 1, self.in_channels, device=x.device)], 0)
        z = _DepthwiseAggFn.apply(x, ea_s[:, :nk], scale, plan)
        if self.selfconn:
            z = z + x * self.DSweight[-1]
        return _LinearFn.apply(z, self.weight[0], self.bias, prec)

    def __repr__(self):
        return '{}({}, {}, K={})'.format(self.__class__.__name__, self.in_channels, self.out_channels,
                                         self.weight.size(0))


class SpectConCatConv(nn.Module):

    def __init__(self, in_channels, out_channels, K, selfconn=True, bias=True, **kwargs):
        kwargs.setdefault('aggr', 'add')
        if kwargs.pop('aggr') != 'add':
            raise ValueError("SpectConCatConv only implements aggr='add' (the reference's default, :109)")
        self.precision = kwargs.pop('precision', 'fp32')
        if self.precision not in _PRECISIONS:
            raise ValueError("precision must be one of %s" % sorted(_PRECISIONS))
        super(SpectConCatConv, self).__init__()
        assert K > 0
        self.in_channels = in_channels
        self.out_channels = out_channels
        self.selfconn = selfconn
        if self.selfconn:
            K = K + 1
        self.weight = Parameter(torch.Tensor(K, in_channels, out_channels))
        if bias:
            self.bias = Parameter(torch.Tensor(K * out_channels))
        else:
            self.register_parameter('bias', None)
        self.reset_parameters()

    def reset_parameters(self):
        glorot(self.weight)
        zeros(self.bias)

    def forward(self, x, edge_index, edge_attr, edge_weight=None, batch=None, lambda_max=None):
        _check_inputs(x, edge_index, edge_attr)
        plan = get_plan(edge_index, x.size(0))
        ea_s = sorted_edge_attr(edge_attr, plan)
        prec = _PRECISIONS[self.precision]
        nk = self.weight.size(0) - (1 if self.selfconn else 0)
        if ea_s.size(1) < nk:
            raise RuntimeError("SpectConCatConv: edge_attr has %d channels but the layer was built with K=%d" % (ea_s.size(1), nk))
        Fi = self.in_channels
        out = []
        if self.selfconn:
            out.append(_LinearFn.apply(x, self.weight[-1], None, prec))
        H = _AggregateFn.apply(x, ea_s[:, :nk], plan)
        for i in range(nk):
            out.append(_LinearFn.apply(H[:, i * Fi:(i + 1) * Fi], self.weight[i], None, prec))
        out = torch.cat(out, 1)
        if self.bias is not None:
            out = out + self.bias
        return out

    def __repr__(self):
        return '{}({}, {}, K={})'.format(self.__class__.__name__, self.in_channels, self.out_channels, self.weight.size(0))


class EdgeEncoder(torch.nn.Module):

    def __init__(self, emb_dim):
        super(EdgeEncoder, self).__init__()
        self.fc1 = torch.nn.Linear(emb_dim[0], emb_dim[1])
        self.fc2 = torch.nn.Linear(emb_dim[1], emb_dim[2])

    def forward(self, edge_attr):
        h = torch.relu(_LinearFn.apply(edge_attr, self.fc1.weight.t(), self.fc1.bias, _lib.PREC_3XTF32))
        return torch.relu(_LinearFn.apply(h, self.fc2.weight.t(), self.fc2.bias, _lib.PREC_3XTF32))


class ML3Layer(torch.nn.Module):

    def __init__(self, learnedge, nedgeinput, nedgeoutput, ninp, nout1, nout2, precision='fp32'):
        super(ML3Layer, self).__init__()
        self.learnedge = learnedge
        self.nout2 = nout2
        self.precision = precision
        if self.learnedge:
            self.fc1_1 = torch.nn.Linear(nedgeinput, 2 * nedgeinput, bias=False)
            self.fc1_2 = torch.nn.Linear(nedgeinput, 2 * nedgeinput, bias=False)
            self.fc1_3 = torch.nn.Linear(nedgeinput, 2 * nedgeinput, bias=False)
            self.fc1_4 = torch.nn.Linear(4 * nedgeinput, nedgeoutput, bias=False)
        else:
            nedgeoutput = nedgeinput
        self.conv1 = SpectConv(ninp, nout1, nedgeoutput, selfconn=False, precision=precision)
        if nout2 > 0:
            self.fc11 = torch.nn.Linear(ninp, nout2)
            self.fc12 = torch.nn.Linear(ninp, nout2)

    def forward(self, x, edge_index, edge_attr):
        _check_inputs(x, edge_index, edge_attr)
        plan = get_plan(edge_index, x.size(0))
        ea = sorted_edge_attr(edge_attr, plan)
        prec = _PRECISIONS[self.precision]
        c = self.conv1
        if not self.learnedge and ea.size(1) > c.weight.size(0):
            ea = ea[:, :c.weight.size(0)].contiguous()
        if ea.size(1) != (self.fc1_1.in_features if self.learnedge else c.weight.size(0)):
            raise RuntimeError("ML3Layer: edge_attr has %d channels, expected %d"
                               % (ea.size(1), self.fc1_1.in_features if self.learnedge else c.weight.size(0)))
        fused_edge = self.learnedge and ops.edge_mlp_supported(self.fc1_1.in_features, self.fc1_4.out_features)
        if self.learnedge and not fused_edge:
            tmp = torch.cat([torch.relu(_LinearFn.apply(ea, self.fc1_1.weight.t(), None, prec)),
                             torch.tanh(_LinearFn.apply(ea, self.fc1_2.weight.t(), None, prec)) *
                             torch.tanh(_LinearFn.apply(ea, self.fc1_3.weight.t(), None, prec))], 1)
            ea = torch.relu(_LinearFn.apply(tmp, self.fc1_4.weight.t(), None, prec))
        w = (self.fc1_1.weight, self.fc1_2.weight, self.fc1_3.weight, self.fc1_4.weight) if fused_edge else (None,) * 4
        g = (self.fc11.weight, self.fc11.bias, self.fc12.weight, self.fc12.bias) if self.nout2 > 0 else (None,) * 4
        return _ML3LayerFn.apply(x, ea, *w, c.weight, c.bias, *g, plan, fused_edge, prec, _needs_save(x, ea, *w, c.weight, c.bias, *g))


ML1_PATH_COUNTS = {"fused": 0, "composed": 0}


class _ML1LayerFn(torch.autograd.Function):

    @staticmethod
    def forward(ctx, x, wconv, bconv, wA, bA, wB, bB, wC, bC, plan, concat, precision=_lib.PREC_3XTF32, save=True):
        xa = ops.aligned_rows(x)
        ws = [w.contiguous() for w in (wconv, wA, wB, wC)]
        bs = [b.contiguous() if b is not None else None for b in (bconv, bA, bB, bC)]
        if save:
            y, aux, _ = ops.ml1layer_forward(plan, xa, ws[0], bs[0], ws[1], bs[1], ws[2], bs[2], ws[3], bs[3], concat=concat,
                                             precision=precision)
        else:
            y, aux, _ = ops.ml1layer_forward(plan, xa, ws[0], bs[0], ws[1], bs[1], ws[2], bs[2], ws[3], bs[3], concat=concat, aux=False,
                                             precision=precision)
        ctx.plan, ctx.concat, ctx.precision = plan, concat, precision
        ctx.has_bias = tuple(b is not None for b in (bconv, bA, bB, bC))
        if save:
            ctx.save_for_backward(xa, *ws, y, aux)
        return y

    @staticmethod
    def backward(ctx, gy):
        xa, wconv, wA, wB, wC, y, aux = ctx.saved_tensors
        need = ctx.needs_input_grad
        N, Fi = xa.shape
        if N == 0:
            z = torch.zeros_like
            bz = [torch.zeros(wconv.size(2), device=xa.device) if h else None for h in ctx.has_bias]
            return z(xa), z(wconv), bz[0], z(wA), bz[1], z(wB), bz[2], z(wC), bz[3], None, None, None, None
        gy = gy if gy.stride(1) == 1 else gy.contiguous()
        dx, dwc, dbc, dwA, dbA, dwB, dbB, dwC, dbC = ops.ml1layer_backward(ctx.plan, xa, wconv, wA, wB, wC, y, aux, gy, need[0],
                                                                          concat=ctx.concat, precision=ctx.precision)
        hb = ctx.has_bias
        return (dx, dwc, dbc if hb[0] else None, dwA, dbA if hb[1] else None, dwB, dbB if hb[2] else None, dwC,
                dbC if hb[3] else None, None, None, None, None)


class ML1Layer(torch.nn.Module):

    def __init__(self, ninp, nout, concat=False, precision="fp32"):
        super(ML1Layer, self).__init__()
        _check_precision(precision)
        self.concat = bool(concat)
        self.precision = precision
        self.conv1 = SpectConv(ninp, nout, 1, selfconn=False)
        self.fc11 = torch.nn.Linear(ninp, nout)
        self.fc12 = torch.nn.Linear(ninp, nout)
        self.fc13 = torch.nn.Linear(ninp, nout)

    @property
    def out_features(self):
        return self.conv1.out_channels * (3 if self.concat else 1)

    def forward(self, x, edge_index):
        return ml1_layer(x, edge_index, self.conv1, self.fc11, self.fc12, self.fc13, self.concat, self.precision)


def _check_precision(precision):
    if precision not in _PRECISIONS:
        raise ValueError("precision must be one of %s" % sorted(_PRECISIONS))


def ml1_layer(x, edge_index, conv, fcA, fcB, fcC, concat=False, precision="fp32"):
    _check_precision(precision)
    if not (x.is_cuda and edge_index.is_cuda):
        raise RuntimeError("gnn_matlang_b200: x and edge_index must be CUDA tensors (the B200 hot path has no CPU fallback)")
    if x.dim() != 2 or x.dtype != torch.float32:
        raise RuntimeError("gnn_matlang_b200: x [N, F] must be float32")
    plan = get_plan(edge_index, x.size(0))
    Fi, Fo = conv.in_channels, conv.out_channels
    prec = _PRECISIONS[precision]
    if ops.ml1layer_supported(Fi, Fo, concat):
        ML1_PATH_COUNTS["fused"] += 1
        ps = (conv.weight, conv.bias, fcA.weight, fcA.bias, fcB.weight, fcB.bias, fcC.weight, fcC.bias)
        return _ML1LayerFn.apply(x, *ps, plan, bool(concat), prec, _needs_save(x, *ps))
    ML1_PATH_COUNTS["composed"] += 1
    ones = torch.ones(plan.E, 1, dtype=torch.float32, device=x.device)
    ax = _AggregateFn.apply(x, ones, plan)
    pa = _LinearFn.apply(x, fcA.weight.t(), fcA.bias, prec)
    pc = _LinearFn.apply(ax, conv.weight[0], conv.bias, prec)
    pp = _LinearFn.apply(x, fcB.weight.t(), fcB.bias, prec) * _LinearFn.apply(x, fcC.weight.t(), fcC.bias, prec)
    if concat:
        return torch.cat([torch.relu(pa), torch.relu(pc), torch.relu(pp)], 1)
    return torch.relu(pa + pc + pp)
```

### gnn_matlang_b200/models.py

```python
import torch
import torch.nn as nn

from .libs.spect_conv import ML3Layer, SpectConv, _LinearFn, _PRECISIONS, _check_precision, ml1_layer
import torch.nn.functional as F

from .pool import global_add_pool, global_max_pool, global_mean_pool

MODEL_CONFIGS = {
    "graph8c": dict(nlayer=3, nout1=32, nout2=16, head=(10,), pool="add", final="tanh"),
    "zinc": dict(nlayer=4, nout1=30, nout2=2, head=(32, 1), pool="add", final=None),
    "exp": dict(nlayer=3, nout1=32, nout2=16, head=(10, 1), pool="mean", final=None),
    "counting": dict(nlayer=5, nout1=16, nout2=16, head=(32, 1), pool="add", final=None),
    "enzymes": dict(nlayer=4, nout1=64, nout2=0, head=(6,), pool="add_max", final="log_softmax", learnedge=False, dropout=0.1,
                    bn="readout", fc_name="fc2"),
    "mutag": dict(nlayer=3, nout1=24, nout2=24, head=(32, 1), pool="mean", final=None, learnedge=False, bn="layers"),
    "filtering": dict(nlayer=3, nout1=32, nout2=16, head=(1,), pool="none", final=None, learnedge=False, fc_name="fc2"),
}


class GNNML3(nn.Module):
    def __init__(self, config, ne, ninp, precision="fp32"):
        super().__init__()
        c = dict(MODEL_CONFIGS[config]) if isinstance(config, str) else dict(config)
        self.cfg = c
        self.precision = precision
        nin = c["nout1"] + c["nout2"]
        for l in range(c["nlayer"]):
            setattr(self, "conv%d" % (l + 1),
                    ML3Layer(learnedge=c.get("learnedge", True), nedgeinput=ne, nedgeoutput=ne, ninp=ninp if l == 0 else nin,
                             nout1=c["nout1"], nout2=c["nout2"], precision=precision))
        if c.get("bn") == "layers":
            for l in range(c["nlayer"]):
                setattr(self, "bn%d" % (l + 1), nn.BatchNorm1d(nin))
        npool = nin * (2 if "_" in c["pool"] else 1)
        if c.get("bn") == "readout":
            setattr(self, "bn%d" % c["nlayer"], nn.BatchNorm1d(npool))
        if len(c["head"]) == 1 and c.get("fc_name") == "fc2":
            self.fc2 = nn.Linear(npool, c["head"][0])
        else:
            self.fc1 = nn.Linear(npool, c["head"][0])
            if len(c["head"]) > 1:
                self.fc2 = nn.Linear(c["head"][0], c["head"][1])

    def forward(self, data):
        x = data.x
        edge_index = data.edge_index2
        edge_attr = data.edge_attr2
        c = self.cfg
        for l in range(c["nlayer"]):
            if c.get("dropout"):
                x = F.dropout(x, p=c["dropout"], training=self.training)
            x = getattr(self, "conv%d" % (l + 1))(x, edge_index, edge_attr)
            if c.get("bn") == "layers":
                x = getattr(self, "bn%d" % (l + 1))(x)
        B = getattr(data, "num_graphs", None)
        pools = {"add": global_add_pool, "mean": global_mean_pool, "max": global_max_pool}
        if c["pool"] != "none":
            x = torch.cat([pools[k](x, data.batch, B) for k in c["pool"].split("_")], 1)
        if c.get("bn") == "readout":
            x = getattr(self, "bn%d" % c["nlayer"])(x)
        prec = _PRECISIONS[self.precision]
        if len(c["head"]) == 1:
            fc = self.fc2 if c.get("fc_name") == "fc2" else self.fc1
            x = _LinearFn.apply(x, fc.weight.t(), fc.bias, prec)
            if c["final"] == "tanh":
                return torch.tanh(x)
            return F.log_softmax(x, dim=1) if c["final"] == "log_softmax" else x
        x = _LinearFn.apply(x, self.fc1.weight.t(), self.fc1.bias, prec)
        return _LinearFn.apply(torch.relu(x), self.fc2.weight.t(), self.fc2.bias, prec)


GNNML1_PRESETS = ("graph8c", "zinc", "exp", "counting")


class GNNML1(nn.Module):

    def __init__(self, config, ninp, nlayer=3, nout=64, concat=False, precision="fp32"):
        super().__init__()
        if isinstance(config, str) and config not in GNNML1_PRESETS:
            raise ValueError("GNNML1 presets: %s" % (GNNML1_PRESETS,))
        _check_precision(precision)
        c = dict(MODEL_CONFIGS[config]) if isinstance(config, str) else dict(config)
        self.cfg = c
        self.precision = precision
        self.nlayer, self.concat = int(nlayer), bool(concat)
        width = nout * (3 if concat else 1)
        for l in range(1, self.nlayer + 1):
            nin = ninp if l == 1 else width
            setattr(self, "conv%d1" % l, SpectConv(nin, nout, 1, selfconn=False))
            setattr(self, "fc%d1" % l, nn.Linear(nin, nout))
            setattr(self, "fc%d2" % l, nn.Linear(nin, nout))
            setattr(self, "fc%d3" % l, nn.Linear(nin, nout))
        self.fc1 = nn.Linear(width, c["head"][0])
        if len(c["head"]) > 1:
            self.fc2 = nn.Linear(c["head"][0], c["head"][1])

    def forward(self, data):
        x = data.x
        edge_index = data.edge_index
        for l in range(1, self.nlayer + 1):
            x = ml1_layer(x, edge_index, getattr(self, "conv%d1" % l), getattr(self, "fc%d1" % l), getattr(self, "fc%d2" % l),
                          getattr(self, "fc%d3" % l), self.concat, self.precision)
        c = self.cfg
        B = getattr(data, "num_graphs", None)
        pool = {"add": global_add_pool, "mean": global_mean_pool}[c["pool"]]
        x = pool(x, data.batch, B)
        prec = _PRECISIONS[self.precision]
        x = _LinearFn.apply(x, self.fc1.weight.t(), self.fc1.bias, prec)
        if len(c["head"]) == 1:
            return torch.tanh(x) if c["final"] == "tanh" else x
        return _LinearFn.apply(torch.relu(x), self.fc2.weight.t(), self.fc2.bias, prec)
```

### gnn_matlang_b200/ops.py

```python
import os

import torch

from . import _lib

_workspaces = {}


class _NullCtx(object):
    def __enter__(self):
        return None

    def __exit__(self, *a):
        return False


_NULL = _NullCtx()


def _on(device):
    idx = device.index
    if idx is None or idx == torch.cuda.current_device():
        return _NULL
    return torch.cuda.device(device)


def _ws(device, nbytes, tag="main"):
    idx = device.index if device.index is not None else torch.cuda.current_device()
    key = (idx, torch._C._cuda_getCurrentRawStream(idx), tag)
    buf = _workspaces.get(key)
    if buf is None or buf.numel() < nbytes:
        buf = torch.empty(max(int(nbytes), 1 << 20), dtype=torch.uint8, device=device)
        _workspaces[key] = buf
    return buf


def _f32c(t, name):
    if t.dtype != torch.float32:
        raise RuntimeError("%s must be float32 (got %s)" % (name, t.dtype))
    if not t.is_cuda:
        raise RuntimeError("%s must be a CUDA tensor: gnn_matlang_b200 has no CPU fallback" % name)
    return t if t.is_contiguous() else t.contiguous()


def _rows(t, name):
    if t.dtype != torch.float32:
        raise RuntimeError("%s must be float32 (got %s)" % (name, t.dtype))
    if not t.is_cuda:
        raise RuntimeError("%s must be a CUDA tensor: gnn_matlang_b200 has no CPU fallback" % name)
    if t.dim() == 2 and (t.size(1) == 1 or t.stride(1) == 1) and (t.size(0) <= 1 or t.stride(0) >= t.size(1)):
        return t
    return t if t.is_contiguous() else t.contiguous()


def _ld(t):
    return t.stride(0) if t.size(0) > 1 else max(t.size(1), 1)


def csr_build(edge_index, num_nodes, check_range=True):
    lib = _lib.load()
    if edge_index.dtype != torch.int64 or edge_index.dim() != 2 or edge_index.size(0) != 2:
        raise RuntimeError("edge_index must be an int64 tensor of shape [2, E]")
    if not edge_index.is_cuda:
        raise RuntimeError("edge_index must be a CUDA tensor: gnn_matlang_b200 has no CPU fallback")
    ei = edge_index.contiguous()
    E, N = ei.size(1), int(num_nodes)
    dev = ei.device
    i32 = dict(dtype=torch.int32, device=dev)
    out = dict(rowptr=torch.empty(N + 1, **i32), col=torch.empty(E, **i32), perm=torch.empty(E, **i32),
               rowptrT=torch.empty(N + 1, **i32), colT=torch.empty(E, **i32), permT=torch.empty(E, **i32))
    flag = torch.zeros(1, **i32)
    nbytes = lib.gnnml3_csr_workspace_bytes(E, N)
    ws = _ws(dev, nbytes)
    with _on(dev):
        rc = lib.gnnml3_csr_build(_lib.ptr(ei), E, N, _lib.ptr(out["rowptr"]), _lib.ptr(out["col"]), _lib.ptr(out["perm"]),
                                  _lib.ptr(out["rowptrT"]), _lib.ptr(out["colT"]), _lib.ptr(out["permT"]),
                                  _lib.ptr(flag), _lib.ptr(ws), ws.numel(), _lib.stream_ptr())
    _lib.check(rc, "gnnml3_csr_build")
    if check_range and int(flag.item()) != 0:
        raise RuntimeError("edge_index contains node ids outside [0, %d)" % N)
    if E > 0:
        nt = (N + lib.gnnml3_tile_rows() - 1) // lib.gnnml3_tile_rows()
        out["win"] = torch.empty(nt, 2, **i32)
        out["winT"] = torch.empty(nt, 2, **i32)
        with _on(dev):
            _lib.check(lib.gnnml3_tile_windows(_lib.ptr(out["rowptr"]), _lib.ptr(out["col"]), N, _lib.ptr(out["win"]),
                                               _lib.stream_ptr()), "gnnml3_tile_windows")
            _lib.check(lib.gnnml3_tile_windows(_lib.ptr(out["rowptrT"]), _lib.ptr(out["colT"]), N, _lib.ptr(out["winT"]),
                                               _lib.stream_ptr()), "gnnml3_tile_windows")
    else:
        out["win"] = out["winT"] = None
    return out


def tile_windows(rowptr, col):
    lib = _lib.load()
    N = rowptr.numel() - 1
    nt = (N + lib.gnnml3_tile_rows() - 1) // lib.gnnml3_tile_rows()
    win = torch.empty(nt, 2, dtype=torch.int32, device=rowptr.device)
    with _on(rowptr.device):
        _lib.check(lib.gnnml3_tile_windows(_lib.ptr(rowptr), _lib.ptr(col), N, _lib.ptr(win), _lib.stream_ptr()),
                   "gnnml3_tile_windows")
    return win


def gather_rows(src, perm):
    lib = _lib.load()
    src = _f32c(src, "src")
    rows, width = perm.numel(), src.size(1)
    out = torch.empty(rows, width, dtype=torch.float32, device=src.device)
    with _on(src.device):
        _lib.check(lib.gnnml3_gather_rows(_lib.ptr(src), _lib.ptr(perm), rows, width, _lib.ptr(out), _lib.stream_ptr()),
                   "gnnml3_gather_rows")
    return out


def scatter_rows(src, perm):
    lib = _lib.load()
    src = _f32c(src, "src")
    rows, width = perm.numel(), src.size(1)
    out = torch.empty(rows, width, dtype=torch.float32, device=src.device)
    with _on(src.device):
        _lib.check(lib.gnnml3_scatter_rows(_lib.ptr(src), _lib.ptr(perm), rows, width, _lib.ptr(out), _lib.stream_ptr()),
                   "gnnml3_scatter_rows")
    return out


def spmm_k(rowptr, col, eperm, ea, x, out=None):
    lib = _lib.load()
    x = _rows(x, "x")
    ea = _f32c(ea, "edge_attr")
    N, F = x.shape
    K = ea.size(1)
    if out is None:
        out = torch.empty(N, K * F, dtype=torch.float32, device=x.device)
    if N == 0:
        return out
    with _on(x.device):
        _lib.check(lib.gnnml3_spmm_k(_lib.ptr(rowptr), _lib.ptr(col), _lib.ptr(eperm), _lib.ptr(ea), _lib.ptr(x), _ld(x),
                                     N, K, F, _lib.ptr(out), _ld(out), _lib.stream_ptr()), "gnnml3_spmm_k")
    return out


def spmm_projected(rowptr, col, eperm, ea, Y, Fo, bias=None):
    lib = _lib.load()
    Y = _rows(Y, "Y")
    ea = _f32c(ea, "edge_attr")
    N, K = Y.size(0), ea.size(1)
    out = torch.empty(N, Fo, dtype=torch.float32, device=Y.device)
    if N == 0:
        return out
    if bias is not None:
        bias = _f32c(bias, "bias")
    with _on(Y.device):
        _lib.check(lib.gnnml3_spmm_projected(_lib.ptr(rowptr), _lib.ptr(col), _lib.ptr(eperm), _lib.ptr(ea), K, _lib.ptr(Y), _ld(Y), N, Fo,
                                             _lib.ptr(bias), _lib.ptr(out), _ld(out), _lib.stream_ptr()), "gnnml3_spmm_projected")
    return out


def sddmm_k(rowptr, col, eperm, x, g, K, E):
    lib = _lib.load()
    x = _rows(x, "x")
    g = _rows(g, "g")
    N, F = x.shape
    dea = torch.empty(E, K, dtype=torch.float32, device=x.device)
    if N == 0 or E == 0:
        return dea
    with _on(x.device):
        _lib.check(lib.gnnml3_sddmm_k(_lib.ptr(rowptr), _lib.ptr(col), _lib.ptr(eperm), _lib.ptr(x), _ld(x), _lib.ptr(g),
                                      _ld(g), N, K, F, _lib.ptr(dea), _lib.stream_ptr()), "gnnml3_sddmm_k")
    return dea


USE_TCGEN05 = os.environ.get("GNNML3_NO_TCGEN05", "0") != "1"
TC_MIN_ROWS = 1024


def gemm_nn_tc(A, B, bias=None, epilogue=_lib.EPI_NONE, out=None, chunk_kblocks=0):
    lib = _lib.load()
    A = _rows(A, "A")
    B = _f32c(B, "B")
    M, Kc = A.shape
    Nc = B.size(1)
    if B.size(0) != Kc:
        raise RuntimeError("gemm_nn_tc: inner dimensions differ (%d vs %d)" % (Kc, B.size(0)))
    if out is None:
        out = torch.empty(M, Nc, dtype=torch.float32, device=A.device)
    if M == 0:
        return out
    if bias is not None:
        bias = _f32c(bias, "bias")
    ws = _ws(A.device, lib.gnnml3_gemm_nn_tc_workspace_bytes(Nc, Kc), tag="tc")
    with _on(A.device):
        _lib.check(lib.gnnml3_gemm_nn_tc(_lib.ptr(A), _ld(A), _lib.ptr(B), _ld(B), _lib.ptr(bias), _lib.ptr(out), _ld(out),
                                         M, Nc, Kc, epilogue, chunk_kblocks, _lib.ptr(ws), ws.numel(), _lib.stream_ptr()),
                   "gnnml3_gemm_nn_tc")
    return out


def gemm_nn(A, B, bias=None, precision=_lib.PREC_3XTF32, epilogue=_lib.EPI_NONE, out=None):
    lib = _lib.load()
    precision = min(int(precision), _lib.PREC_TF32)
    A = _rows(A, "A")
    B = _f32c(B, "B")
    M, Kc = A.shape
    Nc = B.size(1)
    if B.size(0) != Kc:
        raise RuntimeError("gemm_nn: inner dimensions differ (%d vs %d)" % (Kc, B.size(0)))
    if (USE_TCGEN05 and precision == _lib.PREC_3XTF32 and M >= TC_MIN_ROWS and _ld(A) % 4 == 0 and A.data_ptr() % 16 == 0
            and lib.gnnml3_gemm_nn_tc_supported(_ld(A), Nc, Kc)):
        return gemm_nn_tc(A, B, bias, epilogue, out)
    if out is None:
        out = torch.empty(M, Nc, dtype=torch.float32, device=A.device)
    if M == 0:
        return out
    if bias is not None:
        bias = _f32c(bias, "bias")
    with _on(A.device):
        _lib.check(lib.gnnml3_gemm_nn(_lib.ptr(A), _ld(A), _lib.ptr(B), _ld(B), _lib.ptr(bias), _lib.ptr(out),
                                      _ld(out), M, Nc, Kc, precision, epilogue, _lib.stream_ptr()), "gnnml3_gemm_nn")
    return out


def gemm_tn(A, B, precision=_lib.PREC_3XTF32):
    lib = _lib.load()
    precision = min(int(precision), _lib.PREC_TF32)
    A = _rows(A, "A")
    B = _rows(B, "B")
    M, Ka = A.shape
    Nb = B.size(1)
    out = torch.empty(Ka, Nb, dtype=torch.float32, device=A.device)
    if M == 0:
        return out.zero_()
    nbytes = lib.gnnml3_gemm_tn_workspace_bytes(M, Ka, Nb)
    ws = _ws(A.device, nbytes)
    with _on(A.device):
        _lib.check(lib.gnnml3_gemm_tn(_lib.ptr(A), _ld(A), _lib.ptr(B), _ld(B), _lib.ptr(out), _ld(out), M, Ka,
                                      Nb, precision, _lib.ptr(ws), ws.numel(), _lib.stream_ptr()), "gnnml3_gemm_tn")
    return out


def colsum(A):
    lib = _lib.load()
    A = _rows(A, "A")
    M, Nc = A.shape
    out = torch.empty(Nc, dtype=torch.float32, device=A.device)
    if M == 0:
        return out.zero_()
    nbytes = lib.gnnml3_colsum_workspace_bytes(M, Nc)
    ws = _ws(A.device, nbytes)
    with _on(A.device):
        _lib.check(lib.gnnml3_colsum(_lib.ptr(A), _ld(A), M, Nc, _lib.ptr(out), _lib.ptr(ws), ws.numel(),
                                     _lib.stream_ptr()), "gnnml3_colsum")
    return out


def edge_mlp_supported(K, Kout):
    return bool(_lib.load().gnnml3_edge_mlp_supported(int(K), int(Kout)))


def edge_mlp_fwd(ea, eperm, w1, w2, w3, w4):
    lib = _lib.load()
    ea = _f32c(ea, "edge_attr")
    w1, w2, w3, w4 = (_f32c(w, "w") for w in (w1, w2, w3, w4))
    E, K = ea.shape
    Kout = w4.size(0)
    out = torch.empty(E, Kout, dtype=torch.float32, device=ea.device)
    with _on(ea.device):
        _lib.check(lib.gnnml3_edge_mlp_fwd(_lib.ptr(ea), _lib.ptr(eperm), _lib.ptr(w1), _lib.ptr(w2), _lib.ptr(w3), _lib.ptr(w4),
                                           E, K, Kout, _lib.ptr(out), _lib.stream_ptr()), "gnnml3_edge_mlp_fwd")
    return out


def edge_mlp_bwd(ea, eperm, gout, w1, w2, w3, w4, need_dea):
    lib = _lib.load()
    ea = _f32c(ea, "edge_attr")
    gout = _f32c(gout, "gout")
    w1, w2, w3, w4 = (_f32c(w, "w") for w in (w1, w2, w3, w4))
    E, K = ea.shape
    Kout = w4.size(0)
    dev = ea.device
    dea = torch.empty_like(ea) if need_dea else None
    dw = [torch.empty_like(w) for w in (w1, w2, w3, w4)]
    nbytes = lib.gnnml3_edge_mlp_bwd_workspace_bytes(E, K)
    ws = _ws(dev, nbytes)
    with _on(dev):
        _lib.check(lib.gnnml3_edge_mlp_bwd(_lib.ptr(ea), _lib.ptr(eperm), _lib.ptr(gout), _lib.ptr(w1), _lib.ptr(w2), _lib.ptr(w3),
                                           _lib.ptr(w4), E, K, Kout, _lib.ptr(dea), _lib.ptr(dw[0]), _lib.ptr(dw[1]),
                                           _lib.ptr(dw[2]), _lib.ptr(dw[3]), _lib.ptr(ws), ws.numel(), _lib.stream_ptr()),
                   "gnnml3_edge_mlp_bwd")
    return dea, dw


def ml3_act_fwd(pre, Fo, G):
    lib = _lib.load()
    N = pre.size(0)
    y = torch.empty(N, Fo + G, dtype=torch.float32, device=pre.device)
    with _on(pre.device):
        _lib.check(lib.gnnml3_ml3_act_fwd(_lib.ptr(pre), _ld(pre), N, Fo, G, _lib.ptr(y), _ld(y), _lib.stream_ptr()),
                   "gnnml3_ml3_act_fwd")
    return y


def ml3_act_bwd(pre, gy, Fo, G, gate_out=None):
    lib = _lib.load()
    gy = _f32c(gy, "gy")
    N = pre.size(0)
    ld4 = (Fo + 2 * G + 3) // 4 * 4
    gpre = torch.empty(N, ld4, dtype=torch.float32, device=pre.device)[:, :Fo + 2 * G]
    csum = torch.empty(Fo + 2 * G, dtype=torch.float32, device=pre.device)
    ws = _ws(pre.device, lib.gnnml3_ml3_act_bwd_workspace_bytes(N, Fo, G))
    with _on(pre.device):
        _lib.check(lib.gnnml3_ml3_act_bwd(_lib.ptr(pre), _ld(pre), _lib.ptr(gy), _ld(gy), N, Fo, G, _lib.ptr(gpre),
                                          _ld(gpre), _lib.ptr(gate_out) if gate_out is not None else None,
                                          _ld(gate_out) if gate_out is not None else 0, _lib.ptr(csum), _lib.ptr(ws),
                                          ws.numel(), _lib.stream_ptr()),
                   "gnnml3_ml3_act_bwd")
    return gpre, csum


def _padded_rows(N, W, device):
    ld = (W + 3) // 4 * 4
    buf = torch.empty(N, ld, dtype=torch.float32, device=device)
    if ld != W:
        buf[:, W:].zero_()
        buf._gnnml3_zero_pad = True
        return buf[:, :W]
    return buf


def aligned_rows(t):
    if t.dtype != torch.float32 or not t.is_cuda:
        raise RuntimeError("expected a float32 CUDA tensor: gnn_matlang_b200 has no CPU fallback")
    if t.dim() == 2 and t.stride(1) == 1 and t.stride(0) % 4 == 0 and t.data_ptr() % 16 == 0 and t.stride(0) >= t.size(1):
        if t.size(1) % 4 == 0 or getattr(t._base, "_gnnml3_zero_pad", False):
            return t
    N, F = t.shape
    buf = torch.zeros(N, (F + 3) // 4 * 4, dtype=torch.float32, device=t.device)
    buf[:, :F] = t
    return buf[:, :F]


def fused_supported(K, Kstride, F, Nc, Fs=0, self_mode=0, Ns=0):
    return bool(_lib.load().gnnml3_fused_supported(int(K), int(Kstride), int(F), int(Nc), int(Fs), int(self_mode), int(Ns)))


def fused_ts_supported(K, Kstride, F, Nc, Fs=0, self_mode=0, Ns=0):
    return bool(_lib.load().gnnml3_fused_ts_supported(int(K), int(Kstride), int(F), int(Nc), int(Fs), int(self_mode), int(Ns)))


def fused_agg_proj(rowptr, col, eperm, ea, x, Bmain, bias=None, S=None, self_mode=0, Bself=None, bias_s=None, G=0,
                   epilogue=0, hout=None, win=None, precision=_lib.PREC_3XTF32, aux=True):
    lib = _lib.load()
    ea = _f32c(ea, "edge_attr")
    Bmain = _f32c(Bmain, "Bmain")
    N = rowptr.numel() - 1
    F, K = x.size(1), ea.size(1)
    Nc = Bmain.size(1)
    if Bmain.size(0) != K * F:
        raise RuntimeError("fused_agg_proj: Bmain must be [K*F, Nc] = [%d, %d], got %s" % (K * F, Nc, tuple(Bmain.shape)))
    Fs = Ns = 0
    if self_mode:
        Bself = _f32c(Bself, "Bself")
        Fs, Ns = S.size(1), Bself.size(1)
        if Bself.size(0) != Fs:
            raise RuntimeError("fused_agg_proj: Bself must have %d rows" % Fs)
    dev = x.device
    W = Nc + (G if self_mode == 1 else 0)
    out = _padded_rows(N, W, dev)
    save_aux = self_mode == 1 and aux
    aux = torch.empty(N, 2 * G, dtype=torch.float32, device=dev) if save_aux else None
    if bias is not None:
        bias = _f32c(bias, "bias")
    if bias_s is not None:
        bias_s = _f32c(bias_s, "bias_s")
    E = ea.size(0)
    _prof["last_bytes"] = 4.0 * (N * F + (N * Fs if (self_mode and S.data_ptr() != x.data_ptr()) else 0) + E * K + E * (2 if eperm is not None else 1)
                                 + (N + 1) + K * F * Nc + Fs * Ns + Nc + N * W + (N * 2 * G if save_aux else 0))
    ws = _ws(dev, lib.gnnml3_fused_workspace_bytes(K, F, Nc, self_mode), tag="fused")
    with _on(dev):
        _lib.check(lib.gnnml3_fused_agg_proj(
            _lib.ptr(rowptr), _lib.ptr(col), _lib.ptr(eperm), _lib.ptr(ea), K, K, _lib.ptr(x), _ld(x), F,
            _lib.ptr(S) if self_mode else None, _ld(S) if self_mode else 0, Fs, self_mode, _lib.ptr(Bmain), _ld(Bmain),
            _lib.ptr(Bself) if self_mode else None, _ld(Bself) if self_mode else 0, Ns, _lib.ptr(bias), _lib.ptr(bias_s),
            N, Nc, _lib.ptr(out), (W + 3) // 4 * 4, _lib.ptr(aux), 2 * G, G, epilogue | _lib.FUSED_FLAGS[precision], _lib.ptr(hout), _ld(hout) if hout is not None else 0,
            _lib.ptr(win), _lib.ptr(ws), ws.numel(), _lib.stream_ptr()),
            "gnnml3_fused_agg_proj")
    return out, aux


def ml3_act_bwd_y(y, aux, gy, Fo, G):
    lib = _lib.load()
    gy = _rows(gy, "gy")
    N = y.size(0)
    Fo4 = (Fo + 3) // 4 * 4
    ldg = (Fo4 + 2 * G + 3) // 4 * 4
    gpre = torch.empty(N, ldg, dtype=torch.float32, device=y.device)
    csum = torch.empty(Fo + 2 * G, dtype=torch.float32, device=y.device)
    ws = _ws(y.device, lib.gnnml3_ml3_act_bwd_workspace_bytes(N, Fo, G))
    with _on(y.device):
        _lib.check(lib.gnnml3_ml3_act_bwd_y(_lib.ptr(y), _ld(y), _lib.ptr(aux), 2 * G, _lib.ptr(gy), _ld(gy), N, Fo, G,
                                            _lib.ptr(gpre), ldg, _lib.ptr(csum), _lib.ptr(ws), ws.numel(), _lib.stream_ptr()),
                   "gnnml3_ml3_act_bwd_y")
    return gpre, csum


def fused_path_counts(reset=False):
    import ctypes
    buf = (ctypes.c_longlong * 2)()
    _lib.load().gnnml3_fused_path_counts(buf, int(bool(reset)))
    return int(buf[0]), int(buf[1])


def edge_mlp_path_counts(reset=False):
    import ctypes
    buf = (ctypes.c_longlong * 2)()
    _lib.load().gnnml3_edge_mlp_path_counts(buf, int(bool(reset)))
    return int(buf[0]), int(buf[1])


def edge_mlp_set_tc(enable):
    return bool(_lib.load().gnnml3_edge_mlp_set_tc(int(bool(enable))))


def fused_side_output_ok():
    return _lib.load().gnnml3_fused_set_mode(-1) == 0


def fused_sddmm_supported(K, Fi, Fo):
    return bool(_lib.load().gnnml3_fused_sddmm_supported(int(K), int(Fi), int(Fo)))


def fused_sddmm(rowptr, col, x, gc, W, E, win=None):
    lib = _lib.load()
    W = _f32c(W, "W")
    K, Fi, Fo = W.shape
    N = rowptr.numel() - 1
    dea = torch.empty(E, K, dtype=torch.float32, device=x.device)
    ws = _ws(x.device, lib.gnnml3_fused_sddmm_workspace_bytes(K), tag="fused_sddmm")
    with _on(x.device):
        _lib.check(lib.gnnml3_fused_sddmm(_lib.ptr(rowptr), _lib.ptr(col), _lib.ptr(win), _lib.ptr(x), _ld(x), Fi, _lib.ptr(gc), _ld(gc), Fo,
                                          _lib.ptr(W), K, N, _lib.ptr(dea), _lib.ptr(ws), ws.numel(), _lib.stream_ptr()),
                   "gnnml3_fused_sddmm")
    return dea


def ml3layer_supported(K, Fi, Fo, G, learnedge):
    return bool(_lib.load().gnnml3_ml3layer_supported(int(K), int(Fi), int(Fo), int(G), int(bool(learnedge))))


def ml3layer_forward(plan, x, ea_s, ws4, wconv, bconv, gates, keep_aggregate=False, aux=True):
    lib = _lib.load()
    N, Fi = x.shape
    E, K = ea_s.shape
    Fo = wconv.size(2)
    G = gates[0].size(0) if gates is not None else 0
    dev = x.device
    W = Fo + G
    y = _padded_rows(N, W, dev)
    ldy = (W + 3) // 4 * 4
    aux = torch.empty(N, 2 * G, dtype=torch.float32, device=dev) if (G > 0 and aux) else None
    ea2 = torch.empty(E, K, dtype=torch.float32, device=dev) if ws4 is not None else None
    ldh = (K + (1 if G > 0 else 0)) * 32
    hside = torch.empty(N, ldh, dtype=torch.float32, device=dev) if (keep_aggregate and Fi <= 32) else None
    ws = _ws(dev, lib.gnnml3_ml3layer_workspace_bytes(N, E, K, Fi, Fo, G), tag="layer")
    p = _lib.ptr
    w = ws4 if ws4 is not None else (None,) * 4
    g = gates if gates is not None else (None,) * 4
    with _on(dev):
        _lib.check(lib.gnnml3_ml3layer_forward(p(plan.rowptr), p(plan.col), p(plan.win), N, E, p(x), _ld(x), Fi, p(ea_s), K, p(w[0]), p(w[1]), p(w[2]),
                                               p(w[3]), p(wconv), p(bconv), Fo, p(g[0]), p(g[1]), p(g[2]), p(g[3]), G, p(ea2), p(y), ldy,
                                               p(aux), p(hside), ldh, p(ws), ws.numel(), _lib.stream_ptr()), "gnnml3_ml3layer_forward")
    return y, aux, ea2, hside


def ml3layer_backward(plan, x, ea_s, ea2, ws4, wconv, gates_w, y, aux, gy, need_dx, need_dea, has_bias, hside=None):
    lib = _lib.load()
    N, Fi = x.shape
    E, K = ea_s.shape
    Fo = wconv.size(2)
    G = gates_w[0].size(0) if gates_w is not None else 0
    dev = x.device
    f32 = dict(dtype=torch.float32, device=dev)
    lddx = (Fi + 3) // 4 * 4
    dx = torch.empty(N, lddx, **f32) if need_dx else None
    dea = torch.empty(E, K, **f32) if need_dea else None
    dws = [torch.empty_like(t) for t in ws4] if ws4 is not None else [None] * 4
    dwc = torch.empty_like(wconv)
    dbias = torch.empty(Fo + 2 * G, **f32)
    dw11 = torch.empty(G, Fi, **f32) if G > 0 else None
    dw12 = torch.empty(G, Fi, **f32) if G > 0 else None
    ws = _ws(dev, lib.gnnml3_ml3layer_workspace_bytes(N, E, K, Fi, Fo, G), tag="layer")
    p = _lib.ptr
    w = ws4 if ws4 is not None else (None,) * 4
    gw = gates_w if gates_w is not None else (None, None)
    with _on(dev):
        _lib.check(lib.gnnml3_ml3layer_backward(
            p(plan.rowptr), p(plan.col), p(plan.win), p(plan.rowptrT), p(plan.colT), p(plan.permT), p(plan.winT), N, E, p(x), _ld(x), Fi, p(ea_s), p(ea2), K,
            p(w[0]), p(w[1]), p(w[2]), p(w[3]), p(wconv), Fo, p(gw[0]), p(gw[1]), G, p(y), _ld(y), p(aux), p(gy), _ld(gy),
            int(need_dx), int(need_dea), p(dx), lddx, p(dea), p(dws[0]), p(dws[1]), p(dws[2]), p(dws[3]), p(dwc), p(dbias), p(dw11),
            p(dw12), p(hside), _ld(hside) if hside is not None else 0, p(ws), ws.numel(), _lib.stream_ptr()), "gnnml3_ml3layer_backward")
    dbc = dbias[:Fo] if has_bias else None
    db11 = dbias[Fo:Fo + G] if G > 0 else None
    db12 = dbias[Fo + G:] if G > 0 else None
    return (dx[:, :Fi] if need_dx else None), dea, dws, dwc, dbc, dw11, db11, dw12, db12


def ml1layer_supported(Fi, Fo, concat=False):
    return bool(_lib.load().gnnml3_ml1layer_supported(int(Fi), int(Fo), int(bool(concat))))


def ml1layer_forward(plan, x, wconv, bconv, wA, bA, wB, bB, wC, bC, concat=False, keep_aggregate=False, aux=True,
                     precision=_lib.PREC_3XTF32):
    lib = _lib.load()
    N, Fi = x.shape
    Fo = wconv.size(2)
    dev = x.device
    W = 3 * Fo if concat else Fo
    y = _padded_rows(N, W, dev)
    aux = torch.empty(N, 2 * Fo, dtype=torch.float32, device=dev) if aux else None
    hside = _padded_rows(N, Fi, dev) if keep_aggregate else None
    ws = _ws(dev, lib.gnnml3_ml1layer_workspace_bytes(N, Fi, Fo, int(bool(concat))), tag="ml1")
    p = _lib.ptr
    args = (p(plan.rowptr), p(plan.col), N, plan.E, p(x), _ld(x), Fi, p(wconv), p(bconv), p(wA), p(bA), p(wB), p(bB), p(wC), p(bC), Fo,
            int(bool(concat)), p(y), _ld(y) if N > 1 else (W + 3) // 4 * 4, p(aux), 2 * Fo, p(hside), (Fi + 3) // 4 * 4, p(ws), ws.numel(),
            _lib.stream_ptr())
    with _on(dev):
        if precision == _lib.PREC_3XTF32:
            _lib.check(lib.gnnml3_ml1layer_forward(*args), "gnnml3_ml1layer_forward")
        else:
            _lib.check(lib.gnnml3_ml1layer_forward_precision(*args, int(precision)), "gnnml3_ml1layer_forward_precision")
    return y, aux, hside


def ml1layer_backward(plan, x, wconv, wA, wB, wC, y, aux, gy, need_dx, concat=False, precision=_lib.PREC_3XTF32):
    lib = _lib.load()
    N, Fi = x.shape
    Fo = wconv.size(2)
    dev = x.device
    f32 = dict(dtype=torch.float32, device=dev)
    lddx = (Fi + 3) // 4 * 4
    dx = torch.empty(N, lddx, **f32) if need_dx else None
    dwc = torch.empty_like(wconv)
    dwA, dwB, dwC = torch.empty_like(wA), torch.empty_like(wB), torch.empty_like(wC)
    dbs = torch.empty(4, Fo, **f32)
    ws = _ws(dev, lib.gnnml3_ml1layer_workspace_bytes(N, Fi, Fo, int(bool(concat))), tag="ml1")
    p = _lib.ptr
    args = (p(plan.rowptrT), p(plan.colT), N, plan.E, p(x), _ld(x), Fi, p(wconv), p(wA), p(wB), p(wC), Fo, int(bool(concat)),
            p(y), _ld(y) if N > 1 else y.size(1), p(aux), 2 * Fo, p(gy), _ld(gy), int(bool(need_dx)), p(dx), lddx, p(dwc), p(dbs[0]),
            p(dwA), p(dbs[1]), p(dwB), p(dbs[2]), p(dwC), p(dbs[3]), p(ws), ws.numel(), _lib.stream_ptr())
    with _on(dev):
        if precision == _lib.PREC_3XTF32:
            _lib.check(lib.gnnml3_ml1layer_backward(*args), "gnnml3_ml1layer_backward")
        else:
            _lib.check(lib.gnnml3_ml1layer_backward_precision(*args, int(precision)), "gnnml3_ml1layer_backward_precision")
    return (dx[:, :Fi] if need_dx else None), dwc, dbs[0], dwA, dbs[1], dwB, dbs[2], dwC, dbs[3]


def collate_device(n, e, el, ea, B, out, idx=None, node_off=None, edge_off=None, xc=None, widths=None, x=None, m=None, al=None,
                   adj_off=None):
    import ctypes
    lib = _lib.load()
    sup, adj = ea is not None, m is not None
    if not sup and not adj:
        raise RuntimeError("collate_device: the records carry neither supports (ea) nor a plain edge list (m, al)")
    dev = n.device
    if sup and el.is_cuda and not el.is_contiguous():
        el = el.contiguous()
    if adj and al is not None and al.is_cuda and not al.is_contiguous():
        al = al.contiguous()
    checks = [("n", n), ("out.x", out.x), ("out.batch", out.batch), ("out.graph_ptr", out.graph_ptr)]
    if sup:
        checks += [("e", e), ("el", el), ("ea", ea), ("out.edge_index2", out.edge_index2), ("out.edge_attr2", out.edge_attr2)]
    if adj:
        if al is None or getattr(out, "edge_index", None) is None:
            raise RuntimeError("collate_device: the plain edge list needs m, al and out.edge_index")
        checks += [("m", m), ("al", al), ("out.edge_index", out.edge_index)]
    for name, t in checks:
        if not t.is_cuda or not t.is_contiguous():
            raise RuntimeError("collate_device: %s must be a contiguous CUDA tensor (no CPU fallback)" % name)
    if n.dtype != torch.int32 or out.batch.dtype != torch.int64 or out.graph_ptr.dtype != torch.int32 or out.x.dtype != torch.float32 \
            or (sup and (e.dtype != torch.int32 or out.edge_index2.dtype != torch.int64 or ea.dtype != torch.float32)) \
            or (adj and (m.dtype != torch.int32 or out.edge_index.dtype != torch.int64)):
        raise RuntimeError("collate_device: unexpected dtype")
    for t in ((el,) if sup else ()) + ((al,) if adj else ()):
        if t.dtype not in (torch.uint8, torch.int16, torch.int32, torch.int64) or t.dim() != 2 or t.size(0) != 2:
            raise RuntimeError("collate_device: el / al must be [2, *] uint8 / int16 / int32 / int64")
    Np, F = out.x.shape
    Ep, K = out.edge_attr2.shape if sup else (0, 0)
    Mp = out.edge_index.size(1) if adj else 0
    if (sup and (out.edge_index2.size(1) != Ep or ea.size(1) != K)) or (adj and out.edge_index.size(0) != 2) \
            or out.batch.numel() != Np or out.graph_ptr.numel() < B + 1:
        raise RuntimeError("collate_device: output shapes do not match")
    wh = None
    C = 0
    if xc is not None:
        C = xc.size(1)
        wh = (ctypes.c_int32 * C)(*[int(w) for w in widths])
        if xc.dtype != torch.uint8 or not xc.is_contiguous():
            raise RuntimeError("collate_device: xc must be a contiguous uint8 tensor")
    elif x is None or x.dtype != torch.float32 or not x.is_contiguous() or x.size(1) != F:
        raise RuntimeError("collate_device: x [*, F] float32 or xc + widths must be given")
    for t in (idx, node_off, edge_off, adj_off):
        if t is not None and (t.dtype != torch.int64 or not t.is_cuda or not t.is_contiguous()):
            raise RuntimeError("collate_device: idx / node_off / edge_off / adj_off must be contiguous int64 CUDA tensors")
    P = _lib.ptr
    if sup and not adj:
        ws = _ws(dev, lib.gnnml3_collate_workspace_bytes(int(B)), tag="collate")
        with _on(dev):
            _lib.check(lib.gnnml3_collate(P(idx), P(n), P(e), P(node_off), P(edge_off), P(xc), C, wh, P(x), F, P(el),
                                          el.element_size(), el.size(1), P(ea), K, int(B), Np, Ep, P(out.x), P(out.edge_index2),
                                          P(out.edge_attr2), P(out.batch), P(out.graph_ptr), P(ws), ws.numel(), _lib.stream_ptr()),
                       "gnnml3_collate")
        return out
    ws = _ws(dev, lib.gnnml3_collate_graphs_workspace_bytes(int(B)), tag="collate")
    with _on(dev):
        _lib.check(lib.gnnml3_collate_graphs(
            P(idx), P(n), P(node_off), P(xc), C, wh, P(x), F, P(e) if sup else None, P(edge_off) if sup else None,
            P(el) if sup else None, el.element_size() if sup else 0, el.size(1) if sup else 0, P(ea), K, P(m),
            P(adj_off) if adj else None, P(al) if adj else None, al.element_size() if adj else 0, al.size(1) if adj else 0, int(B),
            Np, Ep, Mp, P(out.x), P(out.edge_index2) if sup else None, P(out.edge_attr2) if sup else None,
            P(out.edge_index) if adj else None, P(out.batch), P(out.graph_ptr), P(ws), ws.numel(), _lib.stream_ptr()),
            "gnnml3_collate_graphs")
    return out


def segment_pool_fwd(x, graph_ptr, mean):
    lib = _lib.load()
    x = _f32c(x, "x")
    B, F = graph_ptr.numel() - 1, x.size(1)
    out = torch.empty(B, F, dtype=torch.float32, device=x.device)
    with _on(x.device):
        _lib.check(lib.gnnml3_segment_pool_fwd(_lib.ptr(x), _ld(x), _lib.ptr(graph_ptr), B, F, int(mean), _lib.ptr(out),
                                               _lib.stream_ptr()), "gnnml3_segment_pool_fwd")
    return out


def segment_pool_bwd(gout, graph_ptr, mean, N):
    lib = _lib.load()
    gout = _f32c(gout, "gout")
    B, F = gout.shape
    gx = torch.empty(N, F, dtype=torch.float32, device=gout.device)
    with _on(gout.device):
        _lib.check(lib.gnnml3_segment_pool_bwd(_lib.ptr(gout), _lib.ptr(graph_ptr), B, F, int(mean), _lib.ptr(gx), _ld(gx),
                                               _lib.stream_ptr()), "gnnml3_segment_pool_bwd")
    return gx


def segment_max_fwd(x, graph_ptr):
    lib = _lib.load()
    x = _f32c(x, "x")
    B, F = graph_ptr.numel() - 1, x.size(1)
    out = torch.empty(B, F, dtype=torch.float32, device=x.device)
    arg = torch.empty(B, F, dtype=torch.int32, device=x.device)
    with _on(x.device):
        _lib.check(lib.gnnml3_segment_max_fwd(_lib.ptr(x), _ld(x), _lib.ptr(graph_ptr), B, F, _lib.ptr(out), _lib.ptr(arg),
                                              _lib.stream_ptr()), "gnnml3_segment_max_fwd")
    return out, arg


def segment_max_bwd(gout, arg, graph_ptr, N):
    lib = _lib.load()
    gout = _f32c(gout, "gout")
    B, F = gout.shape
    gx = torch.empty(N, F, dtype=torch.float32, device=gout.device)
    with _on(gout.device):
        _lib.check(lib.gnnml3_segment_max_bwd(_lib.ptr(gout), _lib.ptr(arg), _lib.ptr(graph_ptr), B, F, _lib.ptr(gx), _ld(gx),
                                              _lib.stream_ptr()), "gnnml3_segment_max_bwd")
    return gx


def pairs_mark(emb, bits, wpr, threshold, pairs=None):
    lib = _lib.load()
    emb = _rows(emb, "emb")
    n, d = emb.shape
    P = 0 if pairs is None else pairs.size(0)
    with _on(emb.device):
        _lib.check(lib.gnnml3_pairs_mark(_lib.ptr(emb), _ld(emb), n, d, _lib.ptr(pairs), P, float(threshold), _lib.ptr(bits), wpr,
                                         _lib.stream_ptr()), "gnnml3_pairs_mark")


def pairs_count(bits, n, wpr, P, out):
    lib = _lib.load()
    with _on(bits.device):
        _lib.check(lib.gnnml3_pairs_count(_lib.ptr(bits), n, wpr, P, _lib.ptr(out), _lib.stream_ptr()), "gnnml3_pairs_count")
    return out


_prof = {"enabled": False, "names": None, "records": [], "last_bytes": None}


def profile_start(names=None):
    _prof["enabled"], _prof["names"], _prof["records"] = True, (set(names) if names else None), []


def profile_stop():
    _prof["enabled"] = False
    torch.cuda.synchronize()
    out = [(n, s.elapsed_time(e), shp) for n, s, e, shp in _prof["records"]]
    _prof["records"] = []
    return out


def _instrument(name, fn):
    def wrapped(*a, **k):
        if not _prof["enabled"] or (_prof["names"] is not None and name not in _prof["names"]):
            return fn(*a, **k)
        s, e = torch.cuda.Event(enable_timing=True), torch.cuda.Event(enable_timing=True)
        s.record()
        out = fn(*a, **k)
        e.record()
        shapes = tuple(tuple(t.shape) for t in a if isinstance(t, torch.Tensor))
        if name == "fused_agg_proj":
            shapes = ("algorithmic_bytes", _prof["last_bytes"])
        _prof["records"].append((name, s, e, shapes))
        return out
    wrapped.__name__ = fn.__name__
    wrapped.__doc__ = fn.__doc__
    return wrapped


for _n in ("csr_build", "gather_rows", "scatter_rows", "spmm_k", "spmm_projected", "sddmm_k", "gemm_nn_tc", "gemm_nn", "gemm_tn", "colsum", "edge_mlp_fwd",
           "edge_mlp_bwd", "ml3_act_fwd", "ml3_act_bwd", "ml3_act_bwd_y", "fused_agg_proj", "fused_sddmm", "ml3layer_forward", "ml3layer_backward", "segment_pool_fwd",
           "segment_pool_bwd"):
    globals()[_n] = _instrument(_n, globals()[_n])
```

### include/gnnml3_b200.h

```cpp
#ifndef GNNML3_B200_H_
#define GNNML3_B200_H_

#include <stddef.h>
#include <stdint.h>

#ifdef __cplusplus
extern "C" {
#endif

#if defined(__GNUC__)
#define GNNML3_API __attribute__((visibility("default")))
#else
#define GNNML3_API
#endif

#define GNNML3_OK 0
#define GNNML3_ERR_INVALID 1
#define GNNML3_ERR_CUDA 2
#define GNNML3_ERR_WORKSPACE 3

#define GNNML3_PREC_3XTF32 0
#define GNNML3_PREC_TF32 1
#define GNNML3_PREC_BF16 2

#define GNNML3_FUSED_TF32 0x100
#define GNNML3_FUSED_BF16 0x200

#define GNNML3_EPI_NONE 0
#define GNNML3_EPI_RELU 1

GNNML3_API const char* gnnml3_last_error(void);
GNNML3_API int gnnml3_version(void);
GNNML3_API int64_t gnnml3_launch_count(void);

GNNML3_API size_t gnnml3_csr_workspace_bytes(int64_t E, int64_t N);
GNNML3_API int gnnml3_csr_build(const int64_t* edge_index, int64_t E, int64_t N,
                     int32_t* rowptr, int32_t* col, int32_t* perm,
                     int32_t* rowptrT, int32_t* colT, int32_t* permT,
                     int32_t* err_flag, void* workspace, size_t workspace_bytes, void* stream);

GNNML3_API int gnnml3_gather_rows(const float* in, const int32_t* perm, int64_t rows, int width, float* out, void* stream);
GNNML3_API int gnnml3_scatter_rows(const float* in, const int32_t* perm, int64_t rows, int width, float* out, void* stream);

GNNML3_API int gnnml3_spmm_k(const int32_t* rowptr, const int32_t* col, const int32_t* eperm, const float* ea,
                  const float* x, int64_t ldx, int64_t N, int K, int F, float* out, int64_t ldo, void* stream);

GNNML3_API int gnnml3_spmm_projected(const int32_t* rowptr, const int32_t* col, const int32_t* eperm, const float* ea, int K,
                          const float* Y, int64_t ldy, int64_t N, int Fo, const float* bias, float* out, int64_t ldo, void* stream);

GNNML3_API int gnnml3_sddmm_k(const int32_t* rowptr, const int32_t* col, const int32_t* eperm, const float* x, int64_t ldx,
                   const float* g, int64_t ldg, int64_t N, int K, int F, float* dea, void* stream);

GNNML3_API int gnnml3_gemm_nn(const float* A, int64_t lda, const float* B, int64_t ldb, const float* bias,
                   float* C, int64_t ldc, int64_t M, int Nc, int Kc, int precision, int epilogue, void* stream);
GNNML3_API size_t gnnml3_gemm_tn_workspace_bytes(int64_t M, int Ka, int Nb);
GNNML3_API int gnnml3_gemm_tn(const float* A, int64_t lda, const float* B, int64_t ldb, float* C, int64_t ldc,
                   int64_t M, int Ka, int Nb, int precision, void* workspace, size_t workspace_bytes, void* stream);
GNNML3_API size_t gnnml3_colsum_workspace_bytes(int64_t M, int Nc);
GNNML3_API int gnnml3_colsum(const float* A, int64_t lda, int64_t M, int Nc, float* out, void* workspace,
                  size_t workspace_bytes, void* stream);

GNNML3_API int gnnml3_edge_mlp_supported(int K, int Kout);
GNNML3_API int gnnml3_edge_mlp_set_tc(int enable);
GNNML3_API int gnnml3_edge_mlp_path_counts(long long* out2_host, int reset);
GNNML3_API int gnnml3_edge_mlp_fwd(const float* ea, const int32_t* eperm, const float* w1, const float* w2, const float* w3,
                        const float* w4, int64_t E, int K, int Kout, float* out, void* stream);
GNNML3_API size_t gnnml3_edge_mlp_bwd_workspace_bytes(int64_t E, int K);
GNNML3_API int gnnml3_edge_mlp_bwd(const float* ea, const int32_t* eperm, const float* gout, const float* w1, const float* w2,
                        const float* w3, const float* w4, int64_t E, int K, int Kout, float* dea, float* dw1,
                        float* dw2, float* dw3, float* dw4, void* workspace, size_t workspace_bytes, void* stream);

GNNML3_API int gnnml3_ml3_act_fwd(const float* pre, int64_t ldp, int64_t N, int Fo, int G, float* y, int64_t ldy, void* stream);
GNNML3_API size_t gnnml3_ml3_act_bwd_workspace_bytes(int64_t N, int Fo, int G);
GNNML3_API int gnnml3_ml3_act_bwd(const float* pre, int64_t ldp, const float* gy, int64_t ldy, int64_t N, int Fo, int G,
                       float* gpre, int64_t ldg, float* gate_out, int64_t ldgate, float* colsum,
                       void* workspace, size_t workspace_bytes, void* stream);

GNNML3_API int gnnml3_ml3_act_bwd_y(const float* y, int64_t ldy, const float* aux, int64_t ldaux, const float* gy, int64_t ldgy,
                         int64_t N, int Fo, int G, float* gpre, int64_t ldg, float* colsum,
                         void* workspace, size_t workspace_bytes, void* stream);

GNNML3_API int gnnml3_fused_debug_counters(unsigned long long* out8_host, int reset);
GNNML3_API int gnnml3_fused_set_mode(int slot_mode);
GNNML3_API int gnnml3_fused_profile(int enable);
GNNML3_API int gnnml3_fused_profile_fetch(double* out, int max_records);
GNNML3_API int gnnml3_fused_supported(int K, int Kstride, int F, int Nc, int Fs, int self_mode, int Ns);
GNNML3_API size_t gnnml3_fused_workspace_bytes(int K, int F, int Nc, int self_mode);
GNNML3_API int gnnml3_fused_agg_proj(const int32_t* rowptr, const int32_t* col, const int32_t* eperm, const float* ea,
                          int Kstride, int K, const float* X, int64_t ldx, int F, const float* S, int64_t lds,
                          int Fs, int self_mode, const float* Bmain, int64_t ldb, const float* Bself,
                          int64_t ldbs, int Ns, const float* bias, const float* bias_s, int64_t N, int Nc,
                          float* out, int64_t ldo, float* aux, int64_t ldaux, int G, int epilogue,
                          float* hout, int64_t ldh, const int32_t* tilewin, void* workspace, size_t workspace_bytes,
                          void* stream);
GNNML3_API int gnnml3_tile_rows(void);
GNNML3_API int gnnml3_tile_windows(const int32_t* rowptr, const int32_t* col, int64_t N, int32_t* win, void* stream);
GNNML3_API int gnnml3_fused_ts_supported(int K, int Kstride, int F, int Nc, int Fs, int self_mode, int Ns);
GNNML3_API size_t gnnml3_fused_ts_workspace_bytes(int K, int Nc, int self_mode);
GNNML3_API int gnnml3_fused_set_ts(int enable);
GNNML3_API int gnnml3_fused_path_counts(long long* out2_host, int reset);

GNNML3_API int gnnml3_fused_sddmm_supported(int K, int Fi, int Fo);
GNNML3_API size_t gnnml3_fused_sddmm_workspace_bytes(int K);
GNNML3_API int gnnml3_fused_sddmm(const int32_t* rowptr, const int32_t* col, const int32_t* win, const float* X, int64_t ldx, int Fi,
                       const float* GC, int64_t ldg, int Fo, const float* W, int K, int64_t N, float* dea, void* workspace,
                       size_t workspace_bytes, void* stream);

GNNML3_API int gnnml3_ml3layer_supported(int K, int Fi, int Fo, int G, int learnedge);
GNNML3_API size_t gnnml3_ml3layer_workspace_bytes(int64_t N, int64_t E, int K, int Fi, int Fo, int G);
GNNML3_API int gnnml3_ml3layer_forward(const int32_t* rowptr, const int32_t* col, const int32_t* win, int64_t N, int64_t E, const float* x, int64_t ldx,
                            int Fi, const float* ea_s, int K, const float* w1, const float* w2, const float* w3,
                            const float* w4, const float* wconv, const float* bconv, int Fo, const float* w11,
                            const float* b11, const float* w12, const float* b12, int G, float* ea2, float* y,
                            int64_t ldy, float* aux, float* hside, int64_t ldh, void* workspace, size_t workspace_bytes, void* stream);
GNNML3_API int gnnml3_ml3layer_backward(const int32_t* rowptr, const int32_t* col, const int32_t* win, const int32_t* rowptrT,
                             const int32_t* colT, const int32_t* permT, const int32_t* winT, int64_t N, int64_t E, const float* x, int64_t ldx, int Fi,
                             const float* ea_s, const float* ea2, int K, const float* w1, const float* w2, const float* w3,
                             const float* w4, const float* wconv, int Fo, const float* w11, const float* w12, int G,
                             const float* y, int64_t ldy, const float* aux, const float* gy, int64_t ldgy, int need_dx,
                             int need_dea, float* dx, int64_t lddx, float* dea, float* dw1, float* dw2, float* dw3,
                             float* dw4, float* dwconv, float* dbias, float* dw11, float* dw12, const float* hside, int64_t ldh,
                             void* workspace, size_t workspace_bytes, void* stream);

GNNML3_API int gnnml3_ml1layer_supported(int Fi, int Fo, int concat);
GNNML3_API size_t gnnml3_ml1layer_workspace_bytes(int64_t N, int Fi, int Fo, int concat);
GNNML3_API int gnnml3_ml1layer_forward(const int32_t* rowptr, const int32_t* col, int64_t N, int64_t E, const float* x, int64_t ldx,
                            int Fi, const float* wconv, const float* bconv, const float* wA, const float* bA, const float* wB,
                            const float* bB, const float* wC, const float* bC, int Fo, int concat, float* y, int64_t ldy,
                            float* aux, int64_t ldaux, float* hside, int64_t ldh, void* workspace, size_t workspace_bytes,
                            void* stream);
GNNML3_API int gnnml3_ml1layer_backward(const int32_t* rowptrT, const int32_t* colT, int64_t N, int64_t E, const float* x, int64_t ldx,
                             int Fi, const float* wconv, const float* wA, const float* wB, const float* wC, int Fo, int concat,
                             const float* y, int64_t ldy, const float* aux, int64_t ldaux, const float* gy, int64_t ldgy,
                             int need_dx, float* dx, int64_t lddx, float* dwconv, float* dbconv, float* dwA, float* dbA,
                             float* dwB, float* dbB, float* dwC, float* dbC, void* workspace, size_t workspace_bytes,
                             void* stream);
GNNML3_API int gnnml3_ml1layer_forward_precision(const int32_t* rowptr, const int32_t* col, int64_t N, int64_t E, const float* x,
                            int64_t ldx, int Fi, const float* wconv, const float* bconv, const float* wA, const float* bA,
                            const float* wB, const float* bB, const float* wC, const float* bC, int Fo, int concat, float* y,
                            int64_t ldy, float* aux, int64_t ldaux, float* hside, int64_t ldh, void* workspace,
                            size_t workspace_bytes, void* stream, int precision);
GNNML3_API int gnnml3_ml1layer_backward_precision(const int32_t* rowptrT, const int32_t* colT, int64_t N, int64_t E, const float* x,
                             int64_t ldx, int Fi, const float* wconv, const float* wA, const float* wB, const float* wC, int Fo,
                             int concat, const float* y, int64_t ldy, const float* aux, int64_t ldaux, const float* gy,
                             int64_t ldgy, int need_dx, float* dx, int64_t lddx, float* dwconv, float* dbconv, float* dwA,
                             float* dbA, float* dwB, float* dbB, float* dwC, float* dbC, void* workspace, size_t workspace_bytes,
                             void* stream, int precision);

GNNML3_API int gnnml3_segment_pool_fwd(const float* x, int64_t ldx, const int32_t* graph_ptr, int B, int F, int mean,
                            float* out, void* stream);
GNNML3_API int gnnml3_segment_pool_bwd(const float* gout, const int32_t* graph_ptr, int B, int F, int mean, float* gx,
                            int64_t ldx, void* stream);
GNNML3_API int gnnml3_segment_max_fwd(const float* x, int64_t ldx, const int32_t* graph_ptr, int B, int F, float* out, int32_t* arg,
                           void* stream);
GNNML3_API int gnnml3_segment_max_bwd(const float* gout, const int32_t* arg, const int32_t* graph_ptr, int B, int F, float* gx,
                           int64_t ldx, void* stream);

GNNML3_API int gnnml3_spectral_max_nodes(int nfreq);
GNNML3_API int gnnml3_spectral_count(const int64_t* edge_index, int64_t Etot, const int32_t* edge_ptr, const int32_t* node_ptr,
                          int B, int recfield, int nmax, int32_t* counts, void* stream);
GNNML3_API int gnnml3_spectral_design(const int64_t* edge_index, int64_t Etot, const int32_t* edge_ptr, const int32_t* node_ptr,
                           int B, int recfield, double dv, int nfreq, int laplacien, int addadj, int has_vmax,
                           double vmax, int nmax, const int64_t* out_ptr, int global_ids, int64_t* edge_index2,
                           int64_t E2, float* edge_attr2, float* lmax, float* degree, void* stream);

GNNML3_API int gnnml3_gemm_nn_tc_supported(int64_t lda, int Nc, int Kc);
GNNML3_API size_t gnnml3_gemm_nn_tc_workspace_bytes(int Nc, int Kc);
GNNML3_API int gnnml3_gemm_nn_tc(const float* A, int64_t lda, const float* B, int64_t ldb, const float* bias, float* C,
                      int64_t ldc, int64_t M, int Nc, int Kc, int epilogue, int chunk_kblocks, void* workspace,
                      size_t workspace_bytes, void* stream);

GNNML3_API size_t gnnml3_collate_workspace_bytes(int B);
GNNML3_API int gnnml3_collate(const int64_t* idx, const int32_t* n, const int32_t* e, const int64_t* node_off, const int64_t* edge_off,
                   const uint8_t* xc, int C, const int32_t* widths_host, const float* x, int F, const void* el, int el_bytes,
                   int64_t el_stride, const float* ea, int K, int B, int64_t Np, int64_t Ep, float* out_x,
                   int64_t* out_edge_index, float* out_edge_attr, int64_t* out_batch, int32_t* out_graph_ptr,
                   void* workspace, size_t workspace_bytes, void* stream);

GNNML3_API size_t gnnml3_collate_graphs_workspace_bytes(int B);
GNNML3_API int gnnml3_collate_graphs(const int64_t* idx, const int32_t* n, const int64_t* node_off, const uint8_t* xc, int C,
                   const int32_t* widths_host, const float* x, int F, const int32_t* e, const int64_t* edge_off, const void* el,
                   int el_bytes, int64_t el_stride, const float* ea, int K, const int32_t* m, const int64_t* adj_off, const void* al,
                   int al_bytes, int64_t al_stride, int B, int64_t Np, int64_t Ep, int64_t Mp, float* out_x,
                   int64_t* out_edge_index2, float* out_edge_attr2, int64_t* out_edge_index, int64_t* out_batch,
                   int32_t* out_graph_ptr, void* workspace, size_t workspace_bytes, void* stream);

GNNML3_API int gnnml3_pairs_mark(const float* emb, int64_t ld, int64_t n, int d, const int64_t* pairs, int64_t P,
                                 float threshold, uint32_t* bits, int64_t wpr, void* stream);
GNNML3_API int gnnml3_pairs_count(const uint32_t* bits, int64_t n, int64_t wpr, int64_t P, int64_t* out, void* stream);

#ifdef __cplusplus
}
#endif
#endif
```

Before: 3.651 million.

## Batch edge MLP across all layers into single multi-layer TC kernels

Adds multi-layer variants of the tensor-core edge MLP forward and backward that compute every layer's edge-attribute transform in one launch. They reuse the shared edge-attribute loads and keep one set of weight planes per layer in shared memory, or loop passes over the edges in backward modes. The model precomputes all layers' edge outputs up front when inputs permit, and each layer consumes its precomputed edge features instead of running its own fused edge path. This cuts launch count and repeated edge-attribute reads, at the cost of losing the per-layer fusion of the edge MLP into the aggregation kernel and more shared memory per block.

```diff
diff --git a/gnn_matlang_b200/_lib.py b/gnn_matlang_b200/_lib.py
--- a/gnn_matlang_b200/_lib.py
+++ b/gnn_matlang_b200/_lib.py
@@ -41,6 +41,9 @@
     "gnnml3_edge_mlp_fwd": (_i, [_p, _p, _p, _p, _p, _p, _i64, _i, _i, _p, _p]),
     "gnnml3_edge_mlp_bwd_workspace_bytes": (_sz, [_i64, _i]),
     "gnnml3_edge_mlp_bwd": (_i, [_p, _p, _p, _p, _p, _p, _p, _i64, _i, _i, _p, _p, _p, _p, _p, _p, _sz, _p]),
+    "gnnml3_edge_mlp_fwd_layers": (_i, [_p, _p, _p, _p, _p, _p, _i, _i64, _i, _i, _p, _p]),
+    "gnnml3_edge_mlp_bwd_layers_workspace_bytes": (_sz, [_i64, _i, _i]),
+    "gnnml3_edge_mlp_bwd_layers": (_i, [_p, _p, _p, _p, _p, _p, _p, _i, _i64, _i, _i, _p, _p, _p, _p, _p, _sz, _p]),
     "gnnml3_ml3_act_fwd": (_i, [_p, _i64, _i64, _i, _i, _p, _i64, _p]),
     "gnnml3_ml3_act_bwd_workspace_bytes": (_sz, [_i64, _i, _i]),
     "gnnml3_ml3_act_bwd": (_i, [_p, _i64, _p, _i64, _i64, _i, _i, _p, _i64, _p, _i64, _p, _p, _sz, _p]),
diff --git a/gnn_matlang_b200/csrc/edge_mlp.cu b/gnn_matlang_b200/csrc/edge_mlp.cu
--- a/gnn_matlang_b200/csrc/edge_mlp.cu
+++ b/gnn_matlang_b200/csrc/edge_mlp.cu
@@ -234,12 +234,12 @@
     return (int)(t < 1 ? 1 : (t > cap ? cap : t));
 }
 
-int edge_mlp_tc_fwd(const float* ea, const int32_t* eperm, const float* w1, const float* w2, const float* w3, const float* w4, int64_t E,
-                    int K, float* out, cudaStream_t st);
+int edge_mlp_tc_fwd(const float* ea, const int32_t* eperm, const float* const* w1, const float* const* w2, const float* const* w3,
+                    const float* const* w4, int L, int64_t E, int K, float* const* out, cudaStream_t st);
 size_t edge_mlp_tc_bwd_workspace_bytes(int K);
-int edge_mlp_tc_bwd(const float* ea, const int32_t* eperm, const float* gout, const float* w1, const float* w2, const float* w3,
-                    const float* w4, int64_t E, int K, float* dea, float* dw1, float* dw2, float* dw3, float* dw4, float* partial,
-                    cudaStream_t st);
+int edge_mlp_tc_bwd(const float* ea, const int32_t* eperm, const float* const* gout, const float* const* w1, const float* const* w2,
+                    const float* const* w3, const float* const* w4, int L, int64_t E, int K, float* dea, float* const* dw1,
+                    float* const* dw2, float* const* dw3, float* const* dw4, float* partial, cudaStream_t st);
 
 }
 
@@ -286,7 +286,7 @@
     GNNML3_REQUIRE((uintptr_t)ea % 16 == 0 && (uintptr_t)out % 16 == 0, "edge_mlp_fwd: ea/out must be 16-byte aligned");
     if (g_edge_tc) {
         ++g_edge_paths[0];
-        return edge_mlp_tc_fwd(ea, eperm, w1, w2, w3, w4, E, K, out, (cudaStream_t)stream_);
+        return edge_mlp_tc_fwd(ea, eperm, &w1, &w2, &w3, &w4, 1, E, K, &out, (cudaStream_t)stream_);
     }
     ++g_edge_paths[1];
     int64_t nb = (E + 255) / 256;
@@ -320,7 +320,9 @@
     else
         k_edge_mlp_bwd<K, false><<<nb, C::THREADS, C::bwd_smem, st>>>(ea, eperm, gout, w1, w2, w3, w4, E, dea, partial);
     GNNML3_LAUNCH_CHECK();
-    k_edge_mlp_bwd_reduce<K><<<cdiv(C::NOUT, 32), 256, 0, st>>>(partial, nb, dw1, dw2, dw3, dw4);
+    EMReduceOut d = {};
+    d.dw1[0] = dw1; d.dw2[0] = dw2; d.dw3[0] = dw3; d.dw4[0] = dw4;
+    k_edge_mlp_bwd_reduce<K><<<cdiv(C::NOUT, 32), 256, 0, st>>>(partial, nb, d);
     GNNML3_LAUNCH_CHECK();
     return GNNML3_OK;
 }
@@ -346,10 +348,80 @@
         return set_err(GNNML3_ERR_WORKSPACE, "edge_mlp_bwd: workspace too small");
     if (g_edge_tc) {
         ++g_edge_paths[0];
-        return edge_mlp_tc_bwd(ea, eperm, gout, w1, w2, w3, w4, E, K, dea, dw1, dw2, dw3, dw4, (float*)workspace, st);
+        return edge_mlp_tc_bwd(ea, eperm, &gout, &w1, &w2, &w3, &w4, 1, E, K, dea, &dw1, &dw2, &dw3, &dw4, (float*)workspace, st);
     }
     ++g_edge_paths[1];
     DISPATCH_EVEN_K(K, return launch_edge_bwd<K_>(ea, eperm, gout, w1, w2, w3, w4, E, dea, dw1, dw2, dw3, dw4,
                                                    (float*)workspace, st));
     return GNNML3_OK;
 }
+
+
+static int check_layers(const char* who, int L, const float* const* a, const float* const* b, const float* const* c,
+                        const float* const* d) {
+    GNNML3_REQUIRE(L >= 1, "%s: L=%d < 1", who, L);
+    GNNML3_REQUIRE(a && b && c && d, "%s: NULL pointer array", who);
+    for (int l = 0; l < L; ++l) GNNML3_REQUIRE(a[l] && b[l] && c[l] && d[l], "%s: NULL pointer for layer %d", who, l);
+    return GNNML3_OK;
+}
+
+extern "C" int gnnml3_edge_mlp_fwd_layers(const float* ea, const int32_t* eperm, const float* const* w1, const float* const* w2,
+                                          const float* const* w3, const float* const* w4, int L, int64_t E, int K, int Kout,
+                                          float* const* out, void* stream_) {
+    GNNML3_REQUIRE(gnnml3_edge_mlp_supported(K, Kout), "edge_mlp_fwd_layers: unsupported K=%d Kout=%d (even K <= 16, Kout == K)", K, Kout);
+    GNNML3_REQUIRE(E >= 0, "edge_mlp_fwd_layers: E < 0");
+    int rc;
+    if ((rc = check_layers("edge_mlp_fwd_layers", L, w1, w2, w3, w4))) return rc;
+    GNNML3_REQUIRE(out, "edge_mlp_fwd_layers: NULL output array");
+    for (int l = 0; l < L; ++l) {
+        GNNML3_REQUIRE(out[l], "edge_mlp_fwd_layers: NULL output for layer %d", l);
+        GNNML3_REQUIRE((uintptr_t)out[l] % 16 == 0, "edge_mlp_fwd_layers: outputs must be 16-byte aligned");
+    }
+    if (E == 0) return GNNML3_OK;
+    GNNML3_REQUIRE(ea && (uintptr_t)ea % 16 == 0, "edge_mlp_fwd_layers: ea must be a 16-byte aligned pointer");
+    if (g_edge_tc) {
+        ++g_edge_paths[0];
+        return edge_mlp_tc_fwd(ea, eperm, w1, w2, w3, w4, L, E, K, out, (cudaStream_t)stream_);
+    }
+    for (int l = 0; l < L; ++l)
+        if ((rc = gnnml3_edge_mlp_fwd(ea, eperm, w1[l], w2[l], w3[l], w4[l], E, K, Kout, out[l], stream_))) return rc;
+    return GNNML3_OK;
+}
+
+extern "C" size_t gnnml3_edge_mlp_bwd_layers_workspace_bytes(int64_t E, int K, int L) {
+    const size_t one = gnnml3_edge_mlp_bwd_workspace_bytes(E, K);
+    return one * (size_t)(L < 1 ? 1 : (L < EM_MAXL ? L : EM_MAXL));
+}
+
+extern "C" int gnnml3_edge_mlp_bwd_layers(const float* ea, const int32_t* eperm, const float* const* gout, const float* const* w1,
+                                          const float* const* w2, const float* const* w3, const float* const* w4, int L, int64_t E,
+                                          int K, int Kout, float* const* dw1, float* const* dw2, float* const* dw3,
+                                          float* const* dw4, void* workspace, size_t workspace_bytes, void* stream_) {
+    GNNML3_REQUIRE(gnnml3_edge_mlp_supported(K, Kout), "edge_mlp_bwd_layers: unsupported K=%d Kout=%d", K, Kout);
+    GNNML3_REQUIRE(E >= 0, "edge_mlp_bwd_layers: E < 0");
+    int rc;
+    if ((rc = check_layers("edge_mlp_bwd_layers", L, w1, w2, w3, w4))) return rc;
+    if ((rc = check_layers("edge_mlp_bwd_layers (weight gradients)", L, dw1, dw2, dw3, dw4))) return rc;
+    GNNML3_REQUIRE(gout, "edge_mlp_bwd_layers: NULL gradient array");
+    for (int l = 0; l < L; ++l) GNNML3_REQUIRE(gout[l], "edge_mlp_bwd_layers: NULL gradient for layer %d", l);
+    if (E == 0) {
+        for (int l = 0; l < L; ++l)
+            if ((rc = gnnml3_edge_mlp_bwd(ea, eperm, gout[l], w1[l], w2[l], w3[l], w4[l], 0, K, Kout, nullptr, dw1[l], dw2[l], dw3[l],
+                                          dw4[l], workspace, workspace_bytes, stream_))) return rc;
+        return GNNML3_OK;
+    }
+    GNNML3_REQUIRE(ea && workspace, "edge_mlp_bwd_layers: NULL pointer");
+    GNNML3_REQUIRE((uintptr_t)ea % 16 == 0, "edge_mlp_bwd_layers: ea must be 16-byte aligned");
+    for (int l = 0; l < L; ++l) GNNML3_REQUIRE((uintptr_t)gout[l] % 16 == 0, "edge_mlp_bwd_layers: gradients must be 16-byte aligned");
+    if (workspace_bytes < gnnml3_edge_mlp_bwd_layers_workspace_bytes(E, K, L))
+        return set_err(GNNML3_ERR_WORKSPACE, "edge_mlp_bwd_layers: workspace too small");
+    if (g_edge_tc) {
+        ++g_edge_paths[0];
+        return edge_mlp_tc_bwd(ea, eperm, gout, w1, w2, w3, w4, L, E, K, nullptr, dw1, dw2, dw3, dw4, (float*)workspace,
+                               (cudaStream_t)stream_);
+    }
+    for (int l = 0; l < L; ++l)
+        if ((rc = gnnml3_edge_mlp_bwd(ea, eperm, gout[l], w1[l], w2[l], w3[l], w4[l], E, K, Kout, nullptr, dw1[l], dw2[l], dw3[l],
+                                      dw4[l], workspace, workspace_bytes, stream_))) return rc;
+    return GNNML3_OK;
+}
diff --git a/gnn_matlang_b200/csrc/edge_mlp.cuh b/gnn_matlang_b200/csrc/edge_mlp.cuh
--- a/gnn_matlang_b200/csrc/edge_mlp.cuh
+++ b/gnn_matlang_b200/csrc/edge_mlp.cuh
@@ -72,11 +72,22 @@
     return a;
 }
 
+constexpr int EM_MAXL = 8;
+
+struct EMReduceOut {
+    float *dw1[EM_MAXL], *dw2[EM_MAXL], *dw3[EM_MAXL], *dw4[EM_MAXL];
+};
+
 template <int K>
 __global__ void __launch_bounds__(256)
-k_edge_mlp_bwd_reduce(const float* __restrict__ partial, int nblocks, float* __restrict__ dw1, float* __restrict__ dw2,
-                      float* __restrict__ dw3, float* __restrict__ dw4) {
+k_edge_mlp_bwd_reduce(const float* __restrict__ partial, int nblocks, const EMReduceOut out) {
     using C = EMC<K>;
+    const int layer = blockIdx.y;
+    partial += (size_t)layer * nblocks * C::NT * 16;
+    float* __restrict__ dw1 = out.dw1[layer];
+    float* __restrict__ dw2 = out.dw2[layer];
+    float* __restrict__ dw3 = out.dw3[layer];
+    float* __restrict__ dw4 = out.dw4[layer];
     __shared__ float red[8][33];
     const int tx = threadIdx.x & 31, ty = threadIdx.x >> 5;
     const int i = blockIdx.x * 32 + tx;
diff --git a/gnn_matlang_b200/csrc/edge_mlp_tc.cu b/gnn_matlang_b200/csrc/edge_mlp_tc.cu
--- a/gnn_matlang_b200/csrc/edge_mlp_tc.cu
+++ b/gnn_matlang_b200/csrc/edge_mlp_tc.cu
@@ -32,7 +32,10 @@
         }
         return n < 1 ? 1 : (n > EMT_MAXWG ? EMT_MAXWG : n);
     }
-    __host__ __device__ static constexpr int smem_bytes(int mode) { return 1024 + plane_bytes(mode) + 64 + (mode > 0 ? nwg(mode) * stage_bytes : 0); }
+    static constexpr int LC_FWD = (SMEM_MAX - 64) / plane_bytes(0) < EM_MAXL ? (SMEM_MAX - 64) / plane_bytes(0) : EM_MAXL;
+    __host__ __device__ static constexpr int smem_bytes(int mode, int L = 1) {
+        return 1024 + plane_bytes(mode) * (mode > 0 ? 1 : L) + 64 + (mode > 0 ? nwg(mode) * stage_bytes : 0);
+    }
     static constexpr int NT = C::NT;
     static constexpr int TPT = (NT + 127) / 128;
     static constexpr int GROUPS = NT >= 128 ? 1 : 128 / NT;
@@ -48,10 +51,11 @@
 struct EMTParams {
     const float* ea;
     const int* eperm;
-    const float* gout;
-    const float *w1, *w2, *w3, *w4;
+    const float* gout[EM_MAXL];
+    const float *w1[EM_MAXL], *w2[EM_MAXL], *w3[EM_MAXL], *w4[EM_MAXL];
     int64_t E;
-    float* out;
+    int L;
+    float* out[EM_MAXL];
     float* dea;
     float* partial;
 };
@@ -135,48 +139,58 @@
     constexpr int NWG = T::nwg(MODE);
     extern __shared__ uint8_t smem_raw[];
     uint8_t* smem = smem_raw + ((1024u - (smem_u32(smem_raw) & 1023u)) & 1023u);
+    constexpr int PB = T::plane_bytes(MODE);
     uint8_t* b1 = smem;
     uint8_t* b2 = b1 + T::B1_BYTES;
     uint8_t* b3 = b2 + T::B2_BYTES;
     uint8_t* b4 = b3 + T::B3_BYTES;
-    uint8_t* tail = smem + T::plane_bytes(MODE);
+    uint8_t* tail = smem + (MODE > 0 ? 1 : p.L) * PB;
     uint64_t* bars = reinterpret_cast<uint64_t*>(tail);
     uint32_t* tmem_slot = reinterpret_cast<uint32_t*>(tail + 48);
     float* stage_all = reinterpret_cast<float*>(tail + 64);
 
     const int wg = threadIdx.x >> 7, t = threadIdx.x & 127, warp_in_wg = t >> 5;
 
-    for (int i = threadIdx.x; i < 2 * T::N1 * P; i += blockDim.x) {
-        const int n = i / P, c = i % P;
-        const bool lo = n >= T::N1;
-        const int nn = lo ? n - T::N1 : n, b = nn / HP, j = nn % HP;
-        const float* w = b == 0 ? p.w1 : (b == 1 ? p.w2 : p.w3);
-        emt_put(b1, n, c, (j < H && c < K) ? __ldg(w + j * K + c) : 0.f, lo);
-    }
-    for (int i = threadIdx.x; i < T::TB * 32 * 32; i += blockDim.x) {
-        const int tb = i / 1024, n = (i / 32) % 32, c = i % 32;
-        const bool lo = n >= 16;
-        const int k = n & 15, q = tb * 32 + c, part = q / HP, j = q % HP;
-        emt_put(b2 + tb * 4096, n, c, (k < K && j < H) ? __ldg(p.w4 + k * C::T + part * H + j) : 0.f, lo);
-    }
-    if constexpr (MODE > 0) {
-        for (int i = threadIdx.x; i < 2 * T::N3 * P; i += blockDim.x) {
+    auto build_planes = [&](int l, uint8_t* base) {
+        const float *w1 = p.w1[l], *w2 = p.w2[l], *w3 = p.w3[l], *w4 = p.w4[l];
+        uint8_t *c1 = base, *c2 = base + (b2 - b1), *c3 = base + (b3 - b1), *c4 = base + (b4 - b1);
+        for (int i = threadIdx.x; i < 2 * T::N1 * P; i += blockDim.x) {
             const int n = i / P, c = i % P;
-            const bool lo = n >= T::N3;
-            const int q = lo ? n - T::N3 : n, part = q / HP, j = q % HP;
-            emt_put(b3, n, c, (c < K && j < H) ? __ldg(p.w4 + c * C::T + part * H + j) : 0.f, lo);
-        }
-    }
-    if constexpr (MODE > 1) {
-        for (int i = threadIdx.x; i < T::DB * 32 * 32; i += blockDim.x) {
-            const int db = i / 1024, n = (i / 32) % 32, c = i % 32;
+            const bool lo = n >= T::N1;
+            const int nn = lo ? n - T::N1 : n, b = nn / HP, j = nn % HP;
+            const float* w = b == 0 ? w1 : (b == 1 ? w2 : w3);
+            emt_put(c1, n, c, (j < H && c < K) ? __ldg(w + j * K + c) : 0.f, lo);
+        }
+        for (int i = threadIdx.x; i < T::TB * 32 * 32; i += blockDim.x) {
+            const int tb = i / 1024, n = (i / 32) % 32, c = i % 32;
             const bool lo = n >= 16;
-            const int ii = n & 15, q = db * 32 + c, b = q / HP, j = q % HP;
-            const float* w = b == 0 ? p.w1 : (b == 1 ? p.w2 : p.w3);
-            emt_put(b4 + db * 4096, n, c, (ii < K && q < T::DPP && j < H) ? __ldg(w + j * K + ii) : 0.f, lo);
-        }
-    }
-    fence_proxy_async_smem();
+            const int k = n & 15, q = tb * 32 + c, part = q / HP, j = q % HP;
+            emt_put(c2 + tb * 4096, n, c, (k < K && j < H) ? __ldg(w4 + k * C::T + part * H + j) : 0.f, lo);
+        }
+        if constexpr (MODE > 0) {
+            for (int i = threadIdx.x; i < 2 * T::N3 * P; i += blockDim.x) {
+                const int n = i / P, c = i % P;
+                const bool lo = n >= T::N3;
+                const int q = lo ? n - T::N3 : n, part = q / HP, j = q % HP;
+                emt_put(c3, n, c, (c < K && j < H) ? __ldg(w4 + c * C::T + part * H + j) : 0.f, lo);
+            }
+        }
+        if constexpr (MODE > 1) {
+            for (int i = threadIdx.x; i < T::DB * 32 * 32; i += blockDim.x) {
+                const int db = i / 1024, n = (i / 32) % 32, c = i % 32;
+                const bool lo = n >= 16;
+                const int ii = n & 15, q = db * 32 + c, b = q / HP, j = q % HP;
+                const float* w = b == 0 ? w1 : (b == 1 ? w2 : w3);
+                emt_put(c4 + db * 4096, n, c, (ii < K && q < T::DPP && j < H) ? __ldg(w + j * K + ii) : 0.f, lo);
+            }
+        }
+        fence_proxy_async_smem();
+    };
+    if constexpr (MODE == 0) {
+        for (int l = 0; l < p.L; ++l) build_planes(l, smem + l * PB);
+    } else {
+        build_planes(0, smem);
+    }
     if (threadIdx.x == 0) {
         for (int g = 0; g < NWG; ++g) mbar_init(bars + g, 1);
         asm volatile("fence.mbarrier_init.release.cluster;" ::: "memory");
@@ -224,10 +238,6 @@
                 offA[u] = C::OFF_D + 4 * (t2 / (C::KP / 4));
                 offB[u] = C::OFF_IN + 4 * (t2 % (C::KP / 4));
             }
-#pragma unroll
-            for (int r = 0; r < 4; ++r)
-#pragma unroll
-                for (int c = 0; c < 4; ++c) acc[u][r][c] = 0.f;
         }
     }
 
@@ -245,12 +255,27 @@
             load_edge_row<K>(p.ea + src_n * K, in_n);
         }
     };
-    fetch((int64_t)blockIdx.x * NWG + wg);
 #ifdef EMT_PROFILE
     const bool prof = t == 0;
     long long tacc[10] = {0, 0, 0, 0, 0, 0, 0, 0, 0, 0}, tlast = clock64();
     const long long tbegin = tlast;
 #endif
+    for (int pass = 0; pass < (MODE > 0 ? p.L : 1); ++pass) {
+    if constexpr (MODE > 0) {
+        if (pass > 0) {
+            build_planes(pass, smem);
+            tc_fence_before();
+            __syncthreads();
+            tc_fence_after();
+        }
+#pragma unroll
+        for (int u = 0; u < T::TPT; ++u)
+#pragma unroll
+            for (int r = 0; r < 4; ++r)
+#pragma unroll
+                for (int c = 0; c < 4; ++c) acc[u][r][c] = 0.f;
+    }
+    fetch((int64_t)blockIdx.x * NWG + wg);
     for (int64_t tile = (int64_t)blockIdx.x * NWG + wg; tile < ntiles; tile += tstride) {
         const int64_t e = tile * 128 + t;
         const bool live = e < p.E;
@@ -258,7 +283,7 @@
         float in[P];
 #pragma unroll
         for (int i = 0; i < P; ++i) in[i] = i < C::KP ? in_n[i < C::KP ? i : 0] : 0.f;
-        {
+        auto store_ea = [&] {
             float lo[P];
 #pragma unroll
             for (int i = 0; i < P; ++i) lo[i] = emt_lo(in[i]);
@@ -269,7 +294,8 @@
                 emt_st16(Y, in);
                 emt_st16(Y + 16, lo);
             }
-        }
+        };
+        store_ea();
         if constexpr (MODE > 0) {
 #pragma unroll
             for (int i = 0; i < C::KP; i += 4) *reinterpret_cast<float4*>(row + C::OFF_IN + i) = make_float4(in[i], in[i + 1], in[i + 2], in[i + 3]);
@@ -278,13 +304,18 @@
 #pragma unroll
         for (int i = 0; i < C::KP; ++i) go[i] = 0.f;
         if constexpr (MODE > 0) {
-            if (live) load_edge_row<K>(p.gout + e * K, go);
+            if (live) load_edge_row<K>(p.gout[pass] + e * K, go);
         }
         fetch(tile + tstride);
         EMT_T(0);
+#pragma unroll 1
+        for (int l = 0; l < (MODE > 0 ? 1 : p.L); ++l) {
+        if (l > 0) store_ea();
+        const uint64_t lp = (uint64_t)((l * PB) >> 4);
         emt_round(barid, warp_in_wg, bar, ph, [&] {
 #pragma unroll
-            for (int s = 0; s < P / 8; ++s) mma3(Xm, Ym + 8 * s, Ym + P + 8 * s, d1h + (uint64_t)(2 * s), d1l + (uint64_t)(2 * s), ID1, s == 0);
+            for (int s = 0; s < P / 8; ++s)
+                mma3(Xm, Ym + 8 * s, Ym + P + 8 * s, d1h + lp + (uint64_t)(2 * s), d1l + lp + (uint64_t)(2 * s), ID1, s == 0);
         });
         EMT_T(1);
         uint32_t mask1 = 0;
@@ -331,7 +362,7 @@
 #pragma unroll
             for (int s = 0; s < TP / 8; ++s) {
                 const uint64_t adv = (uint64_t)((s / 4) * (4096 >> 4) + 2 * (s % 4));
-                mma3(Ym, Xm + 8 * s, Xm + TP + 8 * s, d2h + adv, d2l + adv, ID2, s == 0);
+                mma3(Ym, Xm + 8 * s, Xm + TP + 8 * s, d2h + lp + adv, d2l + lp + adv, ID2, s == 0);
             }
         });
         EMT_T(3);
@@ -340,7 +371,7 @@
         emt_ld_wait();
         if constexpr (MODE == 0) {
             if (live) {
-                float* op = p.out + e * K;
+                float* op = p.out[l] + e * K;
 #pragma unroll
                 for (int k = 0; k < K; k += 2) *reinterpret_cast<float2*>(op + k) = make_float2(fmaxf(pre4[k], 0.f), fmaxf(pre4[k + 1], 0.f));
             }
@@ -456,7 +487,38 @@
             emt_group_sync(barid);
             EMT_T(7);
         }
+        }
         EMT_T(8);
+    }
+    if constexpr (MODE > 0) {
+        float* red = stage;
+#pragma unroll
+        for (int u = 0; u < T::TPT; ++u) {
+            if (accum[u]) {
+                const int tl = T::TPT == 1 ? t % T::NT : t + 128 * u;
+#pragma unroll
+                for (int i = 0; i < 4; ++i)
+#pragma unroll
+                    for (int j = 0; j < 4; ++j) red[(size_t)group * T::NT * 16 + tl * 16 + i * 4 + j] = acc[u][i][j];
+            }
+        }
+        emt_group_sync(barid);
+        for (int i = t; i < T::NT * 16; i += 128) {
+            float s = 0.f;
+#pragma unroll
+            for (int g = 0; g < T::GROUPS; ++g) s += red[(size_t)g * T::NT * 16 + i];
+            red[i] = s;
+        }
+        __syncthreads();
+        float* dst = p.partial + ((size_t)pass * gridDim.x + blockIdx.x) * T::NT * 16;
+        for (int i = threadIdx.x; i < T::NT * 16; i += NWG * 128) {
+            float s = 0.f;
+#pragma unroll
+            for (int g = 0; g < NWG; ++g) s += stage_all[(size_t)g * 128 * C::S + i];
+            dst[i] = s;
+        }
+        __syncthreads();
+    }
     }
 #ifdef EMT_PROFILE
     if (prof && wg == 0) {
@@ -465,34 +527,6 @@
         atomicAdd(&g_emt_dbg[10], 1ull);
     }
 #endif
-    if constexpr (MODE > 0) {
-        float* red = stage;
-#pragma unroll
-        for (int u = 0; u < T::TPT; ++u) {
-            if (accum[u]) {
-                const int tl = T::TPT == 1 ? t % T::NT : t + 128 * u;
-#pragma unroll
-                for (int i = 0; i < 4; ++i)
-#pragma unroll
-                    for (int j = 0; j < 4; ++j) red[(size_t)group * T::NT * 16 + tl * 16 + i * 4 + j] = acc[u][i][j];
-            }
-        }
-        emt_group_sync(barid);
-        for (int i = t; i < T::NT * 16; i += 128) {
-            float s = 0.f;
-#pragma unroll
-            for (int g = 0; g < T::GROUPS; ++g) s += red[(size_t)g * T::NT * 16 + i];
-            red[i] = s;
-        }
-        __syncthreads();
-        float* dst = p.partial + (size_t)blockIdx.x * T::NT * 16;
-        for (int i = threadIdx.x; i < T::NT * 16; i += NWG * 128) {
-            float s = 0.f;
-#pragma unroll
-            for (int g = 0; g < NWG; ++g) s += stage_all[(size_t)g * 128 * C::S + i];
-            dst[i] = s;
-        }
-    }
     tc_fence_before();
     __syncthreads();
     if (threadIdx.x < 32) tmem_dealloc(tmem_base, 512);
@@ -503,12 +537,13 @@
     using T = EMT<K>;
     static bool configured[64] = {};
     if (auto once_ = first_use_on_device(configured))
-        GNNML3_CUDA(cudaFuncSetAttribute(k_edge_mlp_tc<K, MODE>, cudaFuncAttributeMaxDynamicSharedMemorySize, T::smem_bytes(MODE)));
+        GNNML3_CUDA(cudaFuncSetAttribute(k_edge_mlp_tc<K, MODE>, cudaFuncAttributeMaxDynamicSharedMemorySize,
+                                         T::smem_bytes(MODE, MODE > 0 ? 1 : T::LC_FWD)));
     constexpr int NWG = T::nwg(MODE);
     const int64_t ntiles = (p.E + 127) / 128;
     int64_t grid = (ntiles + NWG - 1) / NWG;
     if (grid > kNumSMs) grid = kNumSMs;
-    k_edge_mlp_tc<K, MODE><<<(int)grid, NWG * 128, T::smem_bytes(MODE), st>>>(p);
+    k_edge_mlp_tc<K, MODE><<<(int)grid, NWG * 128, T::smem_bytes(MODE, MODE > 0 ? 1 : p.L), st>>>(p);
     GNNML3_LAUNCH_CHECK();
     if (nparts) *nparts = (int)grid;
     return GNNML3_OK;
@@ -527,12 +562,20 @@
         default: return set_err(GNNML3_ERR_INVALID, "edge_mlp_tc: K=%d not instantiated (even K <= 16)", KV); \
     }
 
-int edge_mlp_tc_fwd(const float* ea, const int32_t* eperm, const float* w1, const float* w2, const float* w3, const float* w4, int64_t E,
-                    int K, float* out, cudaStream_t st) {
-    EMTParams p;
-    p.ea = ea; p.eperm = eperm; p.gout = nullptr; p.w1 = w1; p.w2 = w2; p.w3 = w3; p.w4 = w4; p.E = E; p.out = out; p.dea = nullptr;
-    p.partial = nullptr;
-    EMT_DISPATCH(K, return (emt_launch<K_, 0>(p, nullptr, st)));
+int edge_mlp_tc_fwd(const float* ea, const int32_t* eperm, const float* const* w1, const float* const* w2, const float* const* w3,
+                    const float* const* w4, int L, int64_t E, int K, float* const* out, cudaStream_t st) {
+    int lc = 0;
+    EMT_DISPATCH(K, lc = EMT<K_>::LC_FWD);
+    for (int l0 = 0; l0 < L; l0 += lc) {
+        EMTParams p = {};
+        p.ea = ea; p.eperm = eperm; p.E = E; p.L = L - l0 < lc ? L - l0 : lc;
+        for (int l = 0; l < p.L; ++l) {
+            p.w1[l] = w1[l0 + l]; p.w2[l] = w2[l0 + l]; p.w3[l] = w3[l0 + l]; p.w4[l] = w4[l0 + l]; p.out[l] = out[l0 + l];
+        }
+        int rc = GNNML3_OK;
+        EMT_DISPATCH(K, rc = (emt_launch<K_, 0>(p, nullptr, st)));
+        if (rc) return rc;
+    }
     return GNNML3_OK;
 }
 
@@ -542,21 +585,28 @@
     return (size_t)kNumSMs * nt * 16 * sizeof(float);
 }
 
-int edge_mlp_tc_bwd(const float* ea, const int32_t* eperm, const float* gout, const float* w1, const float* w2, const float* w3,
-                    const float* w4, int64_t E, int K, float* dea, float* dw1, float* dw2, float* dw3, float* dw4, float* partial,
-                    cudaStream_t st) {
-    EMTParams p;
-    p.ea = ea; p.eperm = eperm; p.gout = gout; p.w1 = w1; p.w2 = w2; p.w3 = w3; p.w4 = w4; p.E = E; p.out = nullptr; p.dea = dea;
-    p.partial = partial;
-    int nparts = 0, rc;
-    if (dea) {
-        EMT_DISPATCH(K, rc = (emt_launch<K_, 2>(p, &nparts, st)));
-    } else {
-        EMT_DISPATCH(K, rc = (emt_launch<K_, 1>(p, &nparts, st)));
-    }
-    if (rc) return rc;
-    EMT_DISPATCH(K, (k_edge_mlp_bwd_reduce<K_><<<cdiv(EMC<K_>::NOUT, 32), 256, 0, st>>>(partial, nparts, dw1, dw2, dw3, dw4)));
-    GNNML3_LAUNCH_CHECK();
+int edge_mlp_tc_bwd(const float* ea, const int32_t* eperm, const float* const* gout, const float* const* w1, const float* const* w2,
+                    const float* const* w3, const float* const* w4, int L, int64_t E, int K, float* dea, float* const* dw1,
+                    float* const* dw2, float* const* dw3, float* const* dw4, float* partial, cudaStream_t st) {
+    for (int l0 = 0; l0 < L; l0 += EM_MAXL) {
+        EMTParams p = {};
+        p.ea = ea; p.eperm = eperm; p.E = E; p.L = L - l0 < EM_MAXL ? L - l0 : EM_MAXL; p.dea = dea; p.partial = partial;
+        EMReduceOut d = {};
+        for (int l = 0; l < p.L; ++l) {
+            p.gout[l] = gout[l0 + l];
+            p.w1[l] = w1[l0 + l]; p.w2[l] = w2[l0 + l]; p.w3[l] = w3[l0 + l]; p.w4[l] = w4[l0 + l];
+            d.dw1[l] = dw1[l0 + l]; d.dw2[l] = dw2[l0 + l]; d.dw3[l] = dw3[l0 + l]; d.dw4[l] = dw4[l0 + l];
+        }
+        int nparts = 0, rc;
+        if (dea) {
+            EMT_DISPATCH(K, rc = (emt_launch<K_, 2>(p, &nparts, st)));
+        } else {
+            EMT_DISPATCH(K, rc = (emt_launch<K_, 1>(p, &nparts, st)));
+        }
+        if (rc) return rc;
+        EMT_DISPATCH(K, (k_edge_mlp_bwd_reduce<K_><<<dim3(cdiv(EMC<K_>::NOUT, 32), p.L), 256, 0, st>>>(partial, nparts, d)));
+        GNNML3_LAUNCH_CHECK();
+    }
     return GNNML3_OK;
 }
 
diff --git a/gnn_matlang_b200/libs/spect_conv.py b/gnn_matlang_b200/libs/spect_conv.py
--- a/gnn_matlang_b200/libs/spect_conv.py
+++ b/gnn_matlang_b200/libs/spect_conv.py
@@ -385,6 +385,27 @@
         return (dx, dea, dws[0], dws[1], dws[2], dws[3], dwc, dbc, dw11, db11, dw12, db12, None, None, None, None)
 
 
+class _EdgeMLPLayersFn(torch.autograd.Function):
+
+    @staticmethod
+    def forward(ctx, ea_s, *ws):
+        four = [ws[i:i + 4] for i in range(0, len(ws), 4)]
+        ctx.save_for_backward(ea_s, *ws)
+        return tuple(ops.edge_mlp_fwd_layers(ea_s, four))
+
+    @staticmethod
+    def backward(ctx, *gouts):
+        ea_s, *ws = ctx.saved_tensors
+        four = [ws[i:i + 4] for i in range(0, len(ws), 4)]
+        dws = ops.edge_mlp_bwd_layers(ea_s, gouts, four)
+        return (None,) + tuple(d for ds in dws for d in ds)
+
+
+def edge_mlp_layers(ea_s, layers):
+    ws = [w for m in layers for w in (m.fc1_1.weight, m.fc1_2.weight, m.fc1_3.weight, m.fc1_4.weight)]
+    return _EdgeMLPLayersFn.apply(ea_s.contiguous(), *ws)
+
+
 def _needs_save(*tensors):
     return torch.is_grad_enabled() and any(t is not None and t.requires_grad for t in tensors)
 
@@ -577,6 +598,13 @@
         g = (self.fc11.weight, self.fc11.bias, self.fc12.weight, self.fc12.bias) if self.nout2 > 0 else (None,) * 4
         return _ML3LayerFn.apply(x, ea, *w, c.weight, c.bias, *g, plan, fused_edge, prec, _needs_save(x, ea, *w, c.weight, c.bias, *g))
 
+    def _forward_edge_done(self, x, plan, ea2):
+        _check_inputs(x, plan.col, ea2)
+        c = self.conv1
+        g = (self.fc11.weight, self.fc11.bias, self.fc12.weight, self.fc12.bias) if self.nout2 > 0 else (None,) * 4
+        return _ML3LayerFn.apply(x, ea2, None, None, None, None, c.weight, c.bias, *g, plan, False, _PRECISIONS[self.precision],
+                                 _needs_save(x, ea2, c.weight, c.bias, *g))
+
 
 ML1_PATH_COUNTS = {"fused": 0, "composed": 0}
 
diff --git a/gnn_matlang_b200/models.py b/gnn_matlang_b200/models.py
--- a/gnn_matlang_b200/models.py
+++ b/gnn_matlang_b200/models.py
@@ -1,7 +1,9 @@
 import torch
 import torch.nn as nn
 
-from .libs.spect_conv import ML3Layer, SpectConv, _LinearFn, _PRECISIONS, _check_precision, ml1_layer
+from . import ops
+from .graph import get_plan, sorted_edge_attr
+from .libs.spect_conv import ML3Layer, SpectConv, _LinearFn, _PRECISIONS, _check_precision, edge_mlp_layers, ml1_layer
 import torch.nn.functional as F
 
 from .pool import global_add_pool, global_max_pool, global_mean_pool
@@ -47,10 +49,20 @@
         edge_index = data.edge_index2
         edge_attr = data.edge_attr2
         c = self.cfg
+        convs = [getattr(self, "conv%d" % (l + 1)) for l in range(c["nlayer"])]
+        ea2s = None
+        if (edge_attr.is_cuda and edge_attr.dim() == 2 and not edge_attr.requires_grad
+                and all(m.learnedge and m.fc1_1.in_features == edge_attr.size(1)
+                        and ops.edge_mlp_supported(m.fc1_1.in_features, m.fc1_4.out_features) for m in convs)):
+            plan = get_plan(edge_index, x.size(0))
+            ea2s = edge_mlp_layers(sorted_edge_attr(edge_attr, plan), convs)
         for l in range(c["nlayer"]):
             if c.get("dropout"):
                 x = F.dropout(x, p=c["dropout"], training=self.training)
-            x = getattr(self, "conv%d" % (l + 1))(x, edge_index, edge_attr)
+            if ea2s is not None:
+                x = convs[l]._forward_edge_done(x, plan, ea2s[l])
+            else:
+                x = convs[l](x, edge_index, edge_attr)
             if c.get("bn") == "layers":
                 x = getattr(self, "bn%d" % (l + 1))(x)
         B = getattr(data, "num_graphs", None)
diff --git a/gnn_matlang_b200/ops.py b/gnn_matlang_b200/ops.py
--- a/gnn_matlang_b200/ops.py
+++ b/gnn_matlang_b200/ops.py
@@ -290,6 +290,49 @@
                                            _lib.ptr(dw[2]), _lib.ptr(dw[3]), _lib.ptr(ws), ws.numel(), _lib.stream_ptr()),
                    "gnnml3_edge_mlp_bwd")
     return dea, dw
+
+
+def _ptr_array(ts):
+    import ctypes
+    return (ctypes.c_void_p * len(ts))(*[_lib.ptr(t) for t in ts])
+
+
+def _addr(arr):
+    import ctypes
+    return ctypes.addressof(arr)
+
+
+def edge_mlp_fwd_layers(ea, ws):
+    lib = _lib.load()
+    ea = _f32c(ea, "edge_attr")
+    ws = [tuple(_f32c(w, "w") for w in four) for four in ws]
+    E, K = ea.shape
+    Kout = ws[0][3].size(0)
+    out = [torch.empty(E, Kout, dtype=torch.float32, device=ea.device) for _ in ws]
+    arrs = [_ptr_array([four[i] for four in ws]) for i in range(4)] + [_ptr_array(out)]
+    with _on(ea.device):
+        _lib.check(lib.gnnml3_edge_mlp_fwd_layers(_lib.ptr(ea), None, *(_addr(a) for a in arrs[:4]), len(ws), E, K, Kout,
+                                                  _addr(arrs[4]), _lib.stream_ptr()), "gnnml3_edge_mlp_fwd_layers")
+    return out
+
+
+def edge_mlp_bwd_layers(ea, gouts, ws):
+    lib = _lib.load()
+    ea = _f32c(ea, "edge_attr")
+    gouts = [_f32c(g, "gout") for g in gouts]
+    ws = [tuple(_f32c(w, "w") for w in four) for four in ws]
+    E, K = ea.shape
+    Kout = ws[0][3].size(0)
+    L = len(ws)
+    dws = [tuple(torch.empty_like(w) for w in four) for four in ws]
+    ws_buf = _ws(ea.device, lib.gnnml3_edge_mlp_bwd_layers_workspace_bytes(E, K, L))
+    arrs = ([_ptr_array(gouts)] + [_ptr_array([four[i] for four in ws]) for i in range(4)]
+            + [_ptr_array([four[i] for four in dws]) for i in range(4)])
+    with _on(ea.device):
+        _lib.check(lib.gnnml3_edge_mlp_bwd_layers(_lib.ptr(ea), None, *(_addr(a) for a in arrs[:5]), L, E, K, Kout,
+                                                  *(_addr(a) for a in arrs[5:]), _lib.ptr(ws_buf), ws_buf.numel(),
+                                                  _lib.stream_ptr()), "gnnml3_edge_mlp_bwd_layers")
+    return dws
 
 
 def ml3_act_fwd(pre, Fo, G):
@@ -721,6 +764,6 @@
 
 
 for _n in ("csr_build", "gather_rows", "scatter_rows", "spmm_k", "spmm_projected", "sddmm_k", "gemm_nn_tc", "gemm_nn", "gemm_tn", "colsum", "edge_mlp_fwd",
-           "edge_mlp_bwd", "ml3_act_fwd", "ml3_act_bwd", "ml3_act_bwd_y", "fused_agg_proj", "fused_sddmm", "ml3layer_forward", "ml3layer_backward", "segment_pool_fwd",
+           "edge_mlp_bwd", "edge_mlp_fwd_layers", "edge_mlp_bwd_layers", "ml3_act_fwd", "ml3_act_bwd", "ml3_act_bwd_y", "fused_agg_proj", "fused_sddmm", "ml3layer_forward", "ml3layer_backward", "segment_pool_fwd",
            "segment_pool_bwd"):
     globals()[_n] = _instrument(_n, globals()[_n])
diff --git a/include/gnnml3_b200.h b/include/gnnml3_b200.h
--- a/include/gnnml3_b200.h
+++ b/include/gnnml3_b200.h
@@ -69,6 +69,14 @@
 GNNML3_API int gnnml3_edge_mlp_bwd(const float* ea, const int32_t* eperm, const float* gout, const float* w1, const float* w2,
                         const float* w3, const float* w4, int64_t E, int K, int Kout, float* dea, float* dw1,
                         float* dw2, float* dw3, float* dw4, void* workspace, size_t workspace_bytes, void* stream);
+GNNML3_API int gnnml3_edge_mlp_fwd_layers(const float* ea, const int32_t* eperm, const float* const* w1, const float* const* w2,
+                        const float* const* w3, const float* const* w4, int L, int64_t E, int K, int Kout, float* const* out,
+                        void* stream);
+GNNML3_API size_t gnnml3_edge_mlp_bwd_layers_workspace_bytes(int64_t E, int K, int L);
+GNNML3_API int gnnml3_edge_mlp_bwd_layers(const float* ea, const int32_t* eperm, const float* const* gout, const float* const* w1,
+                        const float* const* w2, const float* const* w3, const float* const* w4, int L, int64_t E, int K,
+                        int Kout, float* const* dw1, float* const* dw2, float* const* dw3, float* const* dw4, void* workspace,
+                        size_t workspace_bytes, void* stream);
 
 GNNML3_API int gnnml3_ml3_act_fwd(const float* pre, int64_t ldp, int64_t N, int Fo, int G, float* y, int64_t ldy, void* stream);
 GNNML3_API size_t gnnml3_ml3_act_bwd_workspace_bytes(int64_t N, int Fo, int G);
```

Measured after the change: 3.704 million (median of 6 runs). +1.5%, better.
